# JayKickliter/Multirate.jl

Measured on AMD Instinct MI355X. Metric: Msamples/s in (Float32, 147//160, 24*147 taps) + achieved HBM GB/s vs roofline, higher is better.
Workload: dtype f32

## Files before the change

include/multirate_hip.h:

```cpp
#ifndef MULTIRATE_HIP_H
#define MULTIRATE_HIP_H

#include <stddef.h>
#include <stdint.h>

#ifdef __cplusplus
extern "C" {
#endif

#define MRHIP_ABI_VERSION 1

typedef enum {
    MRHIP_OK = 0,
    MRHIP_ERR_INVALID_ARG = 1,
    MRHIP_ERR_BUFFER_TOO_SMALL = 2,
    MRHIP_ERR_HIP = 3,
    MRHIP_ERR_NO_DEVICE = 4,
    MRHIP_ERR_UNSUPPORTED = 5
} mrhip_status;

typedef enum { MRHIP_F32 = 0, MRHIP_F64 = 1, MRHIP_C64 = 2, MRHIP_C128 = 3 } mrhip_dtype;

typedef enum {
    MRHIP_FIR_STANDARD = 0,
// ... 1 lines not shown
    MRHIP_FIR_INTERPOLATOR = 2,
    MRHIP_FIR_RATIONAL = 3,
    MRHIP_FIR_ARBITRARY = 4,
    MRHIP_FIR_FARROW = 5
} mrhip_kind;

typedef enum { MRHIP_NUMERICS_STRICT = 0, MRHIP_NUMERICS_FUSED = 1 } mrhip_numerics;

typedef struct mrhip_filter mrhip_filter;

typedef struct {
    int32_t kind;
    int32_t tap_dtype;
    int32_t sample_dtype;
    int32_t output_dtype;
    int64_t nchannels;
    int64_t hLen;
    int64_t interpolation;
    int64_t decimation;
    int64_t Nphi;
    int64_t tapsPerPhi;
    int64_t historyLen;
    int64_t phiIdx;
    int64_t inputDeficit;
    int64_t xIdx;
    double rate;
    double phiAccumulator;
    double alpha;
    double delta;
} mrhip_state;

int mrhip_abi_version(void);
const char *mrhip_last_error(void);
int mrhip_device_count(void);

int64_t mrhip_taps2pfb(const void *h, int64_t hLen, int tap_dtype, int64_t Nphi, void *pfb);
int64_t mrhip_nextphase(int64_t currentphase, int64_t interpolation, int64_t decimation);
int64_t mrhip_outputlength_ratio(int64_t inputlength, int64_t interpolation, int64_t decimation,
                                 int64_t initialPhi);
int64_t mrhip_inputlength_ratio(int64_t outputlength, int64_t interpolation, int64_t decimation,
                                int64_t initialPhi);
int mrhip_polyfit(const double *y, int64_t n, int64_t polyorder, double *coef);
int mrhip_output_dtype(int tap_dtype, int sample_dtype);

typedef enum { MRHIP_LOWPASS = 0, MRHIP_BANDPASS = 1, MRHIP_HIGHPASS = 2, MRHIP_BANDSTOP = 3 } mrhip_fir_response;
int mrhip_kaiserlength(double transition, double attenuation, double samplerate, int64_t *numtaps, double *beta);
int mrhip_kaiser(int64_t n, double beta, double *out);
int64_t mrhip_firprototype(int64_t numtaps, const double *F, int nF, int response, double *out);
int64_t mrhip_firdes(int64_t numtaps, const double *cutoff, int ncutoff, int response, double samplerate, double beta,
                     const double *window, double *out);
int64_t mrhip_firdes_kaiser(const double *cutoff, int ncutoff, double transitionwidth, double stopbandAttenuation, int response,
                            double samplerate, double *out);

int mrhip_create_rational(const void *h, int64_t hLen, int tap_dtype, int64_t num, int64_t den,
                          int sample_dtype, int64_t nchannels, int device, mrhip_filter **out);
int mrhip_create_rational_bank(const void *h, int64_t hLen, int tap_dtype, int64_t num, int64_t den,
                               int sample_dtype, int64_t nchannels, int device, mrhip_filter **out);
int mrhip_create_rational_bank_ctaps(const void *h, int64_t hLen, int tap_dtype, int64_t num, int64_t den,
                                     int sample_dtype, int64_t nchannels, int device, mrhip_filter **out);
int mrhip_create_arbitrary(const void *h, int64_t hLen, int tap_dtype, double rate, int64_t Nphi,
                           int sample_dtype, int64_t nchannels, int device, mrhip_filter **out);
int mrhip_create_arbitrary_ctaps(const void *h, int64_t hLen, int tap_dtype, double rate, int64_t Nphi,
                                 int sample_dtype, int64_t nchannels, int device, mrhip_filter **out);
int mrhip_create_farrow(const void *h, int64_t hLen, int tap_dtype, double rate, int64_t Nphi, int64_t polyorder,
                        int sample_dtype, int64_t nchannels, int device, mrhip_filter **out);
int mrhip_create_farrow_pnfb(const double *pnfb, int64_t hLen, int tap_dtype, double rate, int64_t Nphi,
                             int64_t polyorder, int sample_dtype, int64_t nchannels, int device, mrhip_filter **out);
int mrhip_create_farrow_ctaps(const void *h, int64_t hLen, int tap_dtype, double rate, int64_t Nphi, int64_t polyorder,
                              int sample_dtype, int64_t nchannels, int device, mrhip_filter **out);
int mrhip_create_farrow_pnfb_ctaps(const double *pnfb, int64_t hLen, int tap_dtype, double rate, int64_t Nphi,
                                   int64_t polyorder, int sample_dtype, int64_t nchannels, int device, mrhip_filter **out);
int mrhip_get_pnfb(const mrhip_filter *f, double *host_out);
int mrhip_farrow_tapsforphase(const mrhip_filter *f, double phase, void *host_out);
int mrhip_arbitrary_tapsforphase(const mrhip_filter *f, double phase, void *host_out);
void mrhip_destroy(mrhip_filter *f);

int64_t mrhip_outputlength(const mrhip_filter *f, int64_t inputlength);
int64_t mrhip_next_output_count(const mrhip_filter *f, int64_t inputlength);
int64_t mrhip_advance_state(mrhip_filter *f, int64_t inputlength);
int64_t mrhip_inputlength(const mrhip_filter *f, int64_t outputlength);
int mrhip_get_state(const mrhip_filter *f, mrhip_state *st);
int mrhip_set_state(mrhip_filter *f, int64_t phiIdx, int64_t inputDeficit, double phiAccumulator);
int mrhip_get_history(mrhip_filter *f, void *host_out);
int mrhip_set_history(mrhip_filter *f, const void *host_in);
int mrhip_set_history_device(mrhip_filter *f, const void *device_in, void *stream);
int mrhip_reset(mrhip_filter *f);
int mrhip_set_numerics(mrhip_filter *f, int numerics);
int mrhip_set_mod_form(mrhip_filter *f, int form);
int mrhip_get_taps(mrhip_filter *f, int which, void *host_out);

int mrhip_filt_device(mrhip_filter *f, const void *x, int64_t x_len, int64_t x_stride, void *y,
                      int64_t y_capacity, int64_t y_stride, int64_t *n_written, void *stream);
int mrhip_filt_device_async(mrhip_filter *f, const void *x, int64_t x_len, int64_t x_stride, void *y,
                            int64_t y_capacity, int64_t y_stride, int64_t *count_out, void *stream);
int mrhip_filt_device_chained(mrhip_filter *f, const mrhip_filter *prev, const void *x, int64_t x_len_bound, int64_t x_stride,
                              void *y, int64_t y_capacity, int64_t y_stride, int64_t *count_out, void *stream);
int mrhip_filt_device_multi(mrhip_filter *const *filters, int n, const void *const *x, const int64_t *x_len, void *const *y,
                            const int64_t *y_capacity, int64_t *n_written, void *stream);
int64_t mrhip_outputlength_bound(const mrhip_filter *f, int64_t inputlength);
int mrhip_sync_state(mrhip_filter *f, int64_t *last_n_written);
int mrhip_filt_device_chunked(mrhip_filter *f, const void *x, int64_t x_len, int64_t x_stride, int64_t chunk, void *y,
                              int64_t y_capacity, int64_t y_stride, int64_t *n_written, void *stream);
int mrhip_filt_host(mrhip_filter *f, const void *x, int64_t x_len, int64_t x_stride, void *y,
                    int64_t y_capacity, int64_t y_stride, int64_t *n_written);
int mrhip_synchronize(mrhip_filter *f, void *stream);

typedef struct mrhip_cascade mrhip_cascade;
int mrhip_cascade_create(mrhip_filter *const *stages, int nstages, mrhip_cascade **out);
void mrhip_cascade_destroy(mrhip_cascade *c);
int64_t mrhip_cascade_outputlength(const mrhip_cascade *c, int64_t inputlength);
int64_t mrhip_cascade_next_output_count(const mrhip_cascade *c, int64_t inputlength);
int mrhip_cascade_filt_device(mrhip_cascade *c, const void *x, int64_t x_len, int64_t x_stride, void *y, int64_t y_capacity,
                              int64_t y_stride, int64_t *n_written, void *stream);
int mrhip_cascade_filt_device_async(mrhip_cascade *c, const void *x, int64_t x_len, int64_t x_stride, void *y, int64_t y_capacity,
                                    int64_t y_stride, int64_t *count_out, void *stream);
int mrhip_cascade_reset(mrhip_cascade *c);

typedef struct mrhip_ring mrhip_ring;
int mrhip_ring_open(mrhip_filter *f, mrhip_ring **out);
int mrhip_ring_push(mrhip_ring *r, const void *x, int64_t x_len, int64_t x_stride, void *y, int64_t y_capacity, int64_t y_stride,
                    int64_t *n_written, uint64_t *seq);
int mrhip_ring_push_chunks(mrhip_ring *r, const void *x, int64_t x_len, int64_t x_stride, int64_t chunk, void *y, int64_t y_capacity,
                           int64_t y_stride, int64_t *n_written, uint64_t *last_seq);
int mrhip_ring_wait(mrhip_ring *r, uint64_t seq);
int mrhip_ring_drain(mrhip_ring *r);
int mrhip_ring_close(mrhip_ring *r);
int mrhip_ring_info(const mrhip_ring *r, int64_t *info, int n);

typedef struct mrhip_sharded mrhip_sharded;
int mrhip_sharded_create(int ctor, const void *h, int64_t hLen, int tap_dtype, int64_t num, int64_t den, double rate, int64_t Nphi,
                         int64_t polyorder, int sample_dtype, int64_t nchannels, const int *devices, int ndevices, mrhip_sharded **out);
void mrhip_sharded_destroy(mrhip_sharded *s);
int mrhip_sharded_nshards(const mrhip_sharded *s);
int mrhip_sharded_shard(const mrhip_sharded *s, int i, int64_t *start, int64_t *count, int *device, mrhip_filter **filter);
int64_t mrhip_sharded_outputlength(const mrhip_sharded *s, int64_t inputlength);
int64_t mrhip_sharded_next_output_count(const mrhip_sharded *s, int64_t inputlength);
int mrhip_sharded_reset(mrhip_sharded *s);
int mrhip_sharded_filt_device(mrhip_sharded *s, const void *const *x, int64_t x_len, const int64_t *x_stride, void *const *y, int64_t y_capacity,
                              const int64_t *y_stride, int64_t *n_written);
int mrhip_sharded_filt_host(mrhip_sharded *s, const void *x, int64_t x_len, int64_t x_stride, void *y, int64_t y_capacity, int64_t y_stride,
                            int64_t *n_written);
int mrhip_sharded_gather(mrhip_sharded *s, const void *const *y, int64_t n_out, const int64_t *y_stride, void *dst, int64_t dst_stride, int dst_device);
int mrhip_sharded_wait_stream(mrhip_sharded *s, int shard, void *stream);
int mrhip_sharded_signal_stream(mrhip_sharded *s, int shard, void *stream);
int mrhip_sharded_synchronize(mrhip_sharded *s);

int mrhip_filt_once(const void *h, int64_t hLen, int tap_dtype, int64_t num, int64_t den, double rate,
                    int64_t Nphi, const void *x, int64_t x_len, int sample_dtype, void *y,
                    int64_t y_capacity, int64_t *n_written, int device);

int mrhip_set_timing(mrhip_filter *f, int enabled);
int mrhip_timing_read(mrhip_filter *f, int64_t *n_launches, double *total_ms);
const char *mrhip_last_kernel_name(const mrhip_filter *f);
int mrhip_schedule_info(const mrhip_filter *f, int64_t *info, int n);

#ifdef __cplusplus
}
#endif
#endif
```

multirate.jl_amd/csrc/api.hip:

```cpp
#include <algorithm>
#include <cmath>
#include <chrono>
#include <cstdlib>
#include <cstring>
#include <mutex>
#include <numeric>
#include <unordered_map>

#include "mrhip_filter.h"

namespace mrhip {

bool plan_farrow_wave(const FarrowArgs &a);
hipError_t launch_farrow_wave(const TypeKey &tk, bool fused, const FarrowArgs &a, hipStream_t s, const char **kname, int num_cus);

thread_local LaunchEvents g_launch_events;
static thread_local std::string g_last_error;

void set_error(const std::string &msg) { g_last_error = msg; }

namespace {
struct OccKey { const void *fn; int dev; bool operator==(const OccKey &o) const { return fn == o.fn && dev == o.dev; } };
struct OccKeyHash { size_t operator()(const OccKey &k) const { return std::hash<const void *>()(k.fn) ^ (static_cast<size_t>(k.dev) * 0x9e3779b97f4a7c15ull); } };
struct OccEntry { unsigned block = 0; size_t lds = ~static_cast<size_t>(0), attr = 0; int per_cu = 0; };
// ... 137 lines not shown
        } else {
            (void)hipGetLastError();
            MRHIP_CHECK_HIP(device_sync_relaxed());
        }
    }
    f->last_stream = stream;
    f->last_stream_valid = true;
    return MRHIP_OK;
}

int drain_filter(mrhip_filter *f)
{
    if (f->last_stream_valid && hipStreamSynchronize(f->last_stream) != hipSuccess) {
        (void)hipGetLastError();
        MRHIP_CHECK_HIP(device_sync_relaxed());
    }
    return MRHIP_OK;
}

int check_create_args(const void *h, int64_t hLen, int th, int tx, int64_t nch, int device, mrhip_filter **out, bool complex_taps_ok = false)
{
    if (!out) return fail(MRHIP_ERR_INVALID_ARG, "out is NULL");
    *out = nullptr;
    if (!h || hLen < 1) return fail(MRHIP_ERR_INVALID_ARG, "h must hold at least one tap");
    if (th < MRHIP_F32 || th > MRHIP_C128) return fail(MRHIP_ERR_INVALID_ARG, "bad tap dtype");
    if (dtype_is_complex(th) && !complex_taps_ok)
        return fail(MRHIP_ERR_UNSUPPORTED, "complex taps are supported by the rational family only (mrhip_create_rational: FIRStandard, FIRDecimator, "
                                           "FIRInterpolator, FIRRational); FIRArbitrary and FIRFarrow take Float32 or Float64 taps");
    if (tx < MRHIP_F32 || tx > MRHIP_C128) return fail(MRHIP_ERR_INVALID_ARG, "bad sample dtype");
    if (nch < 1) return fail(MRHIP_ERR_INVALID_ARG, "nchannels must be >= 1");
    int ndev = 0;
    if (hipGetDeviceCount(&ndev) != hipSuccess || ndev == 0)
        return fail(MRHIP_ERR_NO_DEVICE, "no HIP device visible; libmultirate_hip has no CPU fallback");
    if (device < 0 || device >= ndev) return fail(MRHIP_ERR_INVALID_ARG, "device ordinal out of range");
    if (!device_is_gfx950(device))
        return fail(MRHIP_ERR_NO_DEVICE, "device is not gfx950 (MI355X); kernels are built for gfx950 only");
    return MRHIP_OK;
}

int multi_staging(mrhip_filter *f, size_t bytes)
{
    if (bytes > f->multi_cap) {
        if (f->multi_in_flight) { MRHIP_CHECK_HIP(hipEventSynchronize(f->multi_ev)); f->multi_in_flight = false; }
        if (int rc = drain_filter(f)) return rc;
        if (f->multi_pin) (void)hipHostFree(f->multi_pin);
        if (f->multi_dev) (void)hipFree(f->multi_dev);
        f->multi_pin = f->multi_dev = nullptr; f->multi_cap = 0;
        MRHIP_CHECK_HIP(hipHostMalloc(&f->multi_pin, bytes * 2, hipHostMallocDefault));
        MRHIP_CHECK_HIP(hipMalloc(&f->multi_dev, bytes * 2));
        f->multi_cap = bytes * 2;
        if (!f->multi_ev) MRHIP_CHECK_HIP(hipEventCreateWithFlags(&f->multi_ev, hipEventDisableTiming));
    }
    if (f->multi_in_flight) { MRHIP_CHECK_HIP(hipEventSynchronize(f->multi_ev)); f->multi_in_flight = false; }
    return MRHIP_OK;
}

hipError_t launch_opair_blocks(mrhip_filter *f, const TypeKey &tk, bool fused, const PolyArgs &a, hipStream_t s, const char **kname, bool *launched)
{
    *launched = false;
    PairArgs pa;
    dim3 block;
    size_t lds = 0;
    int nblocks = 0;
    if (!plan_rational_opair_blocks(tk, fused, a, f->num_cus, &pa, &block, &lds, &nblocks)) return hipSuccess;
    const size_t bytes = static_cast<size_t>(nblocks) * sizeof(MultiDesc);
    if (multi_staging(f, bytes) != MRHIP_OK) return hipErrorOutOfMemory;
    MultiDesc *d = static_cast<MultiDesc *>(f->multi_pin);
    const size_t osz = dtype_scalar_size(f->ty) * static_cast<size_t>(f->nc);
    unsigned steps_max = 0;
    for (int b = 0; b < nblocks; ++b) {
        MultiDesc &m = d[b];
        const long long first = static_cast<long long>(b) * pa.P;
        const long long Pb = std::min<long long>(pa.P, static_cast<long long>(pa.Sout) - first);
        const long long n_rel = a.n_out - first;
        const long long spc = n_rel > 0 ? (n_rel + pa.Sout - 1) / pa.Sout : 0;
        const long long u0b = a.u0 + first * a.M;
        m.x = a.x; m.y = static_cast<unsigned char *>(a.y) + static_cast<size_t>(first) * osz;
        m.hist = a.hist; m.hist_new = a.hist_new; m.taps = a.taps; m.rec = b == 0 ? a.rec : nullptr;
        m.x_stride = a.x_stride; m.y_stride = a.y_stride; m.x_len = a.x_len; m.n_out = std::max<long long>(n_rel, 0);
        m.u0 = u0b; m.d0 = a.d0; m.phi_end = a.phi_end; m.d_end = a.d_end;
        m.steps_per_channel = static_cast<unsigned>(std::max<long long>(spc, 1));
        m.total_steps = static_cast<unsigned>(spc * a.nch);
        m.spc_magic = step_magic(spc);
        m.nch = b == 0 ? a.nch : 0;
        m.P_blk = static_cast<int>(Pb);
        m.q0 = static_cast<int>((u0b / a.L) & ~1LL);
        steps_max = std::max(steps_max, m.total_steps);
    }
    hipError_t e = hipMemcpyAsync(f->multi_dev, f->multi_pin, bytes, hipMemcpyHostToDevice, s);
    if (e != hipSuccess) return e;
    e = hipEventRecord(f->multi_ev, s);
    if (e != hipSuccess) return e;
    f->multi_in_flight = true;
    PolyArgs am = a;
    am.multi = static_cast<const MultiDesc *>(f->multi_dev); am.multi_n = nblocks;
    pa.total_steps = steps_max;
    e = launch_rational_opair(fused, am, pa, block, lds, s, kname, f->num_cus, f->d_counters);
    *launched = e == hipSuccess;
    return e;
}

}
bool try_launch_interp_lane(const TypeKey &tk, bool fused, const PolyArgs &a, unsigned *counters, hipStream_t s, const char **kname, int num_cus, hipError_t *err);
namespace {

hipError_t launch_poly(const mrhip_filter *f, const TypeKey &tk, bool fused, const PolyArgs &a, hipStream_t s,
                       const char **kname, bool *did_shiftin, unsigned *counters, bool *rec_written)
{
    *did_shiftin = false;
    *rec_written = false;
    if (tk.bank && tk.complex_h) {
        *rec_written = true;
        ArbTileArgs bt;
        size_t bl = 0;
        if (!f->force_generic && plan_bank_ctaps_tiled(tk, a, f->num_cus, &bt, &bl))
            return launch_poly_bank_ctaps_tiled(tk, a, bt, bl, s, kname, f->num_cus);
        return launch_poly_bank_ctaps_generic(tk, a, s, kname);
    }
    if (tk.bank) {
        *rec_written = true;
        ArbTileArgs bt;
        size_t bl = 0;
        if (!f->force_generic && plan_bank_tiled(tk, a, f->num_cus, &bt, &bl))
            return launch_poly_bank_tiled(tk, fused, a, bt, bl, s, kname, f->num_cus);
        return launch_poly_bank_generic(tk, fused, a, s, kname);
    }
    if (tk.complex_h) {
        *rec_written = true;
        ArbTileArgs ct;
        size_t cl = 0;
        if (!f->force_generic && plan_ctaps_tiled(tk, a, f->num_cus, &ct, &cl))
            return launch_poly_ctaps_tiled(tk, a, ct, cl, s, kname, f->num_cus);
        return launch_poly_ctaps_generic(tk, a, s, kname);
    }
    if (!f->force_generic) {
        if (a.L == 1) {
            PairArgs spa;
            dim3 sblock;
            size_t slds = 0;
            if (plan_fir_stream(tk, a, f->num_cus, &spa, &sblock, &slds)) {
                *rec_written = true;
                *did_shiftin = a.H > 0;
                return launch_fir_stream(fused, a, spa, sblock, slds, s, kname, f->num_cus, counters);
            }
        }
        {
            hipError_t el = hipSuccess;
            if (try_launch_interp_lane(tk, fused, a, counters, s, kname, f->num_cus, &el)) return el;
        }
        {
            PairArgs pa;
            dim3 block;
            size_t lds = 0;
            if (plan_rational_opair(tk, fused, a, f->num_cus, &pa, &block, &lds)) {
                *rec_written = true;
                *did_shiftin = a.H > 0;
                return launch_rational_opair(fused, a, pa, block, lds, s, kname, f->num_cus, counters);
            }
            bool launched = false;
            const hipError_t eb = launch_opair_blocks(const_cast<mrhip_filter *>(f), tk, fused, a, s, kname, &launched);
            if (eb != hipSuccess) return eb;
            if (launched) { *rec_written = true; *did_shiftin = a.H > 0; return hipSuccess; }
        }
        TileArgs ta;
        dim3 grid, block;
        size_t lds = 0;
        if (plan_phase_stationary(tk, a, f->num_cus, &ta, &grid, &block, &lds))
            return launch_poly_phase_stationary(tk, fused, a, ta, grid, block, lds, s, kname, f->num_cus);
        {
            ArbTileArgs tt;
            size_t tl = 0;
            if (plan_poly_tiled(tk, a, f->num_cus, &tt, &tl))
                return launch_poly_tiled(tk, fused, a, tt, tl, s, kname, f->num_cus);
        }
    }
    *rec_written = true;
    return launch_poly_generic(tk, fused, a, s, kname);
}

}

bool any_capture_active() { return any_capture_active_impl(); }
}

using namespace mrhip;

extern "C" {

int mrhip_abi_version(void) { return MRHIP_ABI_VERSION; }
const char *mrhip_last_error(void) { return g_last_error.c_str(); }

int mrhip_device_count(void)
{
    int n = 0;
    if (hipGetDeviceCount(&n) != hipSuccess) return 0;
    int ok = 0;
    for (int d = 0; d < n; ++d) ok += device_is_gfx950(d) ? 1 : 0;
    return ok;
}

int64_t mrhip_taps2pfb(const void *h, int64_t hLen, int tap_dtype, int64_t Nphi, void *pfb)
{
    if (!h || hLen < 1 || Nphi < 1) return -1;
    return taps2pfb(h, hLen, tap_dtype, Nphi, pfb);
}
int64_t mrhip_nextphase(int64_t p, int64_t L, int64_t M) { return nextphase(p, L, M); }
int64_t mrhip_outputlength_ratio(int64_t n, int64_t L, int64_t M, int64_t phi) { return outputlength_ratio(n, L, M, phi); }
int64_t mrhip_inputlength_ratio(int64_t n, int64_t L, int64_t M, int64_t phi) { return inputlength_ratio(n, L, M, phi); }

int mrhip_output_dtype(int th, int tx)
{
    const bool f64 = dtype_is_f64(th) || dtype_is_f64(tx);
    if (dtype_is_complex(tx) || dtype_is_complex(th)) return f64 ? MRHIP_C128 : MRHIP_C64;
    return f64 ? MRHIP_F64 : MRHIP_F32;
}

static int create_rational_common(const void *h, int64_t hLen, int th, int64_t num, int64_t den, int tx, int64_t nch,
                                  int device, bool bank, mrhip_filter **out)
{
    if (num < 1 || den < 1) return fail(MRHIP_ERR_INVALID_ARG, "ratio must be positive");
    const int64_t g = std::gcd(num, den);
    const int64_t L = num / g, M = den / g;
    if (L > 0x7fffffff || M > 0x7fffffff || hLen > 0x7fffffff)
        return fail(MRHIP_ERR_INVALID_ARG, "L, M and hLen must fit in 31 bits");

    DeviceGuard guard(device);
    if (!guard.ok) return fail(MRHIP_ERR_HIP, "hipSetDevice failed");
    auto *f = new mrhip_filter();
    f->th = th; f->tx = tx; f->ty = mrhip_output_dtype(th, tx);
    f->nc = dtype_is_complex(tx) ? 2 : 1;
    f->r_f64 = dtype_is_f64(f->ty);
    f->nch = nch; f->hLen = hLen; f->L = L; f->M = M; f->device = device;
    f->bank = bank;
    const size_t es = dtype_size(th);
    const size_t rows = bank ? static_cast<size_t>(nch) : 1;

    if (L == 1) {
        f->kind = M == 1 ? MRHIP_FIR_STANDARD : MRHIP_FIR_DECIMATOR;
        f->Nphi = 1; f->T = hLen; f->H = hLen - 1;
    } else {
        f->kind = M == 1 ? MRHIP_FIR_INTERPOLATOR : MRHIP_FIR_RATIONAL;
        f->Nphi = L;
        f->T = taps2pfb(h, hLen, th, L, nullptr);
        f->H = f->T - 1;
    }
    {
        const size_t bank_bytes = static_cast<size_t>(f->T) * static_cast<size_t>(f->Nphi) * es;
        f->h_taps.resize(bank_bytes * rows);
        for (size_t r = 0; r < rows; ++r)
            taps2pfb(static_cast<const unsigned char *>(h) + r * static_cast<size_t>(hLen) * es, hLen, th, f->Nphi, f->h_taps.data() + r * bank_bytes);
    }
    int rc = upload_taps(f, f->h_taps, &f->d_taps, &f->d_taps_alloc);
    if (!rc) rc = alloc_common(f);
    if (rc) { mrhip_destroy(f); return rc; }
    *out = f;
    return MRHIP_OK;
}

int mrhip_create_rational(const void *h, int64_t hLen, int th, int64_t num, int64_t den, int tx, int64_t nch,
                          int device, mrhip_filter **out)
{
    if (int rc = check_create_args(h, hLen, th, tx, nch, device, out, true)) return rc;
    return create_rational_common(h, hLen, th, num, den, tx, nch, device, false, out);
}

int mrhip_create_rational_bank(const void *h, int64_t hLen, int th, int64_t num, int64_t den, int tx, int64_t nch,
                               int device, mrhip_filter **out)
{
    if (out) *out = nullptr;
    if (th == MRHIP_C64 || th == MRHIP_C128)
        return fail(MRHIP_ERR_UNSUPPORTED, "mrhip_create_rational_bank takes Float32 / Float64 taps (complex taps in a bank are not supported)");
    if (int rc = check_create_args(h, hLen, th, tx, nch, device, out)) return rc;
    return create_rational_common(h, hLen, th, num, den, tx, nch, device, true, out);
}

int mrhip_create_rational_bank_ctaps(const void *h, int64_t hLen, int th, int64_t num, int64_t den, int tx, int64_t nch,
                                     int device, mrhip_filter **out)
{
    if (out) *out = nullptr;
    if (th == MRHIP_F32 || th == MRHIP_F64)
        return fail(MRHIP_ERR_INVALID_ARG, "mrhip_create_rational_bank_ctaps takes Complex64 / Complex128 taps; real taps: mrhip_create_rational_bank");
    if (int rc = check_create_args(h, hLen, th, tx, nch, device, out, true)) return rc;
    return create_rational_common(h, hLen, th, num, den, tx, nch, device, true, out);
}

static int create_arbitrary_common(const void *h, int64_t hLen, int th, double rate, int64_t Nphi, int tx, int64_t nch,
                                   int device, mrhip_filter **out)
{
    if (!(rate > 0.0)) return fail(MRHIP_ERR_INVALID_ARG, "rate must be greater than 0");
    if (Nphi < 1 || Nphi > 0x7fffffff || hLen > 0x7fffffff) return fail(MRHIP_ERR_INVALID_ARG, "bad Nphi");

    DeviceGuard guard(device);
    if (!guard.ok) return fail(MRHIP_ERR_HIP, "hipSetDevice failed");
    auto *f = new mrhip_filter();
    f->kind = MRHIP_FIR_ARBITRARY;
    f->th = th; f->tx = tx; f->ty = mrhip_output_dtype(th, tx);
    f->nc = dtype_is_complex(tx) ? 2 : 1;
    f->r_f64 = dtype_is_f64(f->ty);
    f->nch = nch; f->hLen = hLen; f->L = Nphi; f->M = 1; f->Nphi = Nphi; f->device = device;
    f->rate = rate;
    f->delta = static_cast<double>(Nphi) / rate;
    const size_t es = dtype_size(th);

    std::vector<unsigned char> dh(static_cast<size_t>(hLen) * es, 0);
    arbitrary_dh(h, hLen, th, dh.data());
    f->T = taps2pfb(h, hLen, th, Nphi, nullptr);
    f->H = f->T - 1;
// ... 1383 lines not shown
        if (f->d_xbuf[slot]) (void)hipFree(f->d_xbuf[slot]);
        f->d_xbuf[slot] = nullptr; f->d_xcap[slot] = 0;
        MRHIP_CHECK_HIP(hipMalloc(&f->d_xbuf[slot], xbytes));
        f->d_xcap[slot] = xbytes;
    }
    if (ybytes > f->d_ycap[slot]) {
        if (f->d_ybuf[slot]) (void)hipFree(f->d_ybuf[slot]);
        f->d_ybuf[slot] = nullptr; f->d_ycap[slot] = 0;
        MRHIP_CHECK_HIP(hipMalloc(&f->d_ybuf[slot], ybytes));
        f->d_ycap[slot] = ybytes;
    }
    return MRHIP_OK;
}

int mrhip_filt_host(mrhip_filter *f, const void *x, int64_t x_len, int64_t x_stride, void *y, int64_t y_capacity,
                    int64_t y_stride, int64_t *n_written)
{
    if (!f) return fail(MRHIP_ERR_INVALID_ARG, "NULL filter");
    if (n_written) *n_written = 0;
    if (x_len < 0 || y_capacity < 0) return fail(MRHIP_ERR_INVALID_ARG, "negative length");
    if (x_len == 0) return MRHIP_OK;
    if (!x) return fail(MRHIP_ERR_INVALID_ARG, "x is NULL");
    if (f->nch > 1 && x_stride < x_len) return fail(MRHIP_ERR_INVALID_ARG, "x_stride < x_len");
    const int64_t count = mrhip_next_output_count(f, x_len);
    if (count > y_capacity) return fail(MRHIP_ERR_BUFFER_TOO_SMALL, "buffer is too small");
    if (count > 0 && !y) return fail(MRHIP_ERR_INVALID_ARG, "y is NULL");
    if (f->nch > 1 && y_stride < count) return fail(MRHIP_ERR_INVALID_ARG, "y_stride < output count");

    DeviceGuard guard(f->device);
    if (!guard.ok) return fail(MRHIP_ERR_HIP, "hipSetDevice failed");
    const size_t xe = x_elt(f), ye = y_elt(f);
    const int64_t env_kb = MRHIP_ENV_INT("MRHIP_HOST_PIECE_KB", 0);
    const int64_t piece_kb = env_kb > 0 ? env_kb : 64 * 1024;
    int64_t piece = (piece_kb << 10) / static_cast<int64_t>(xe * static_cast<size_t>(f->nch));
    piece = std::max<int64_t>(piece, 256);
    const bool pipelined = x_len > piece + piece / 2;
    if (!pipelined) piece = x_len;
    if (!f->s_in) {
        MRHIP_CHECK_HIP(hipStreamCreateWithFlags(&f->s_in, hipStreamNonBlocking));
        MRHIP_CHECK_HIP(hipStreamCreateWithFlags(&f->s_out, hipStreamNonBlocking));
        for (int i = 0; i < 2; ++i) {
            MRHIP_CHECK_HIP(hipEventCreateWithFlags(&f->ev_in[i], hipEventDisableTiming));
            MRHIP_CHECK_HIP(hipEventCreateWithFlags(&f->ev_k[i], hipEventDisableTiming));
            MRHIP_CHECK_HIP(hipEventCreateWithFlags(&f->ev_out[i], hipEventDisableTiming));
        }
    }
    hipStream_t sk = f->own_stream;
    const int64_t y_piece_cap = pipelined ? std::max<int64_t>(mrhip_outputlength(f, piece), 0) + 8 + 2 * (f->L / std::max<int64_t>(f->M, 1) + 1) : count;
    const int nslots = pipelined ? 2 : 1;
    for (int sl = 0; sl < nslots; ++sl)
        if (int rc = ensure_staging(f, sl, std::max<size_t>(static_cast<size_t>(piece) * xe * f->nch, 16),
                                    std::max<size_t>(static_cast<size_t>(y_piece_cap) * ye * f->nch, 16))) return rc;
    const size_t x_pitch = static_cast<size_t>(f->nch > 1 ? x_stride : x_len) * xe;
    const size_t y_pitch = static_cast<size_t>(f->nch > 1 ? y_stride : count) * ye;
    int64_t k = 0;
    int it = 0;
    bool used[2] = {false, false};
    auto bail = [&](int rc) -> int {
        (void)hipStreamSynchronize(f->s_in); (void)hipStreamSynchronize(sk); (void)hipStreamSynchronize(f->s_out);
        (void)hipGetLastError();
        if (n_written) *n_written = k;
        return rc;
    };
#define MRHIP_HOSTPATH_HIP(expr)                                                                          \
    do {                                                                                                    \
        hipError_t e_ = (expr);                                                                             \
        if (e_ != hipSuccess) return bail(fail(MRHIP_ERR_HIP, std::string(#expr) + ": " + hipGetErrorString(e_))); \
    } while (0)
    for (int64_t a = 0; a < x_len; a += piece, ++it) {
        const int sl = it & 1;
        const int64_t len = std::min<int64_t>(piece, x_len - a);
        const size_t xrow = static_cast<size_t>(len) * xe;
        if (used[sl]) MRHIP_HOSTPATH_HIP(hipStreamWaitEvent(f->s_in, f->ev_k[sl], 0));
        MRHIP_HOSTPATH_HIP(hipMemcpy2DAsync(f->d_xbuf[sl], xrow, static_cast<const unsigned char *>(x) + static_cast<size_t>(a) * xe, x_pitch, xrow,
                                         static_cast<size_t>(f->nch), hipMemcpyHostToDevice, f->s_in));
        MRHIP_HOSTPATH_HIP(hipEventRecord(f->ev_in[sl], f->s_in));
        MRHIP_HOSTPATH_HIP(hipStreamWaitEvent(sk, f->ev_in[sl], 0));
        if (used[sl]) MRHIP_HOSTPATH_HIP(hipStreamWaitEvent(sk, f->ev_out[sl], 0));
        const int64_t cap = std::min<int64_t>(y_piece_cap, count - k);
        int64_t nw = 0;
        if (int rc = filt_device_one(f, f->d_xbuf[sl], len, len, f->d_ybuf[sl], cap, std::max<int64_t>(cap, 1), &nw, sk, a > 0)) {
            return bail(rc);
        }
        MRHIP_HOSTPATH_HIP(hipEventRecord(f->ev_k[sl], sk));
        if (nw > 0) {
            MRHIP_HOSTPATH_HIP(hipStreamWaitEvent(f->s_out, f->ev_k[sl], 0));
            const size_t yrow = static_cast<size_t>(nw) * ye;
            MRHIP_HOSTPATH_HIP(hipMemcpy2DAsync(static_cast<unsigned char *>(y) + static_cast<size_t>(k) * ye, y_pitch, f->d_ybuf[sl],
                                             static_cast<size_t>(std::max<int64_t>(cap, 1)) * ye, yrow, static_cast<size_t>(f->nch), hipMemcpyDeviceToHost, f->s_out));
        }
        MRHIP_HOSTPATH_HIP(hipEventRecord(f->ev_out[sl], f->s_out));
        used[sl] = true;
        k += nw;
    }
#undef MRHIP_HOSTPATH_HIP
    MRHIP_CHECK_HIP(hipStreamSynchronize(f->s_out));
    MRHIP_CHECK_HIP(hipStreamSynchronize(sk));
    if (n_written) *n_written = k;
    return MRHIP_OK;
}

int mrhip_synchronize(mrhip_filter *f, void *stream)
{
    if (!f) return fail(MRHIP_ERR_INVALID_ARG, "NULL filter");
    DeviceGuard guard(f->device);
    MRHIP_CHECK_HIP(hipStreamSynchronize(static_cast<hipStream_t>(stream)));
    return MRHIP_OK;
}

int mrhip_filt_once(const void *h, int64_t hLen, int th, int64_t num, int64_t den, double rate, int64_t Nphi,
                    const void *x, int64_t x_len, int tx, void *y, int64_t y_capacity, int64_t *n_written, int device)
{
    mrhip_filter *f = nullptr;
    int rc = rate > 0.0 ? mrhip_create_arbitrary(h, hLen, th, rate, Nphi, tx, 1, device, &f)
                        : mrhip_create_rational(h, hLen, th, num, den, tx, 1, device, &f);
    if (rc) return rc;
    rc = mrhip_filt_host(f, x, x_len, x_len, y, y_capacity, y_capacity, n_written);
    mrhip_destroy(f);
    return rc;
}

int mrhip_set_timing(mrhip_filter *f, int enabled)
{
    if (!f) return fail(MRHIP_ERR_INVALID_ARG, "NULL filter");
    f->timing = enabled != 0;
    f->timing_stride = enabled > 1 ? enabled : 1;
    f->timing_group = enabled < -1 ? -enabled : 1;
    f->timing_launch = 0; f->timing_open = false; f->ev_skip = false;
    f->ev_used = 0;
    return MRHIP_OK;
}

int mrhip_timing_read(mrhip_filter *f, int64_t *n_launches, double *total_ms)
{
    if (!f || !n_launches || !total_ms) return fail(MRHIP_ERR_INVALID_ARG, "NULL argument");
    DeviceGuard guard(f->device);
    *n_launches = 0;
    *total_ms = 0.0;
    const size_t pairs = f->ev_used / 2;
    for (size_t i = 0; i < pairs; ++i) {
        float ms = 0.f;
        MRHIP_CHECK_HIP(hipEventSynchronize(f->ev_pool[2 * i + 1]));
        MRHIP_CHECK_HIP(hipEventElapsedTime(&ms, f->ev_pool[2 * i], f->ev_pool[2 * i + 1]));
        *total_ms += ms;
    }
    *n_launches = static_cast<int64_t>(pairs) * f->timing_group;
    f->ev_used = 0;
    f->timing_launch = 0; f->timing_open = false;
    return MRHIP_OK;
}

const char *mrhip_last_kernel_name(const mrhip_filter *f) { return f ? f->last_kernel : ""; }

int mrhip_schedule_info(const mrhip_filter *f, int64_t *info, int n)
{
    if (!f || !info || n < 0) return fail(MRHIP_ERR_INVALID_ARG, "NULL argument");
    if (f->kind != MRHIP_FIR_ARBITRARY && f->kind != MRHIP_FIR_FARROW) return fail(MRHIP_ERR_INVALID_ARG, "not a FIRArbitrary / FIRFarrow filter");
    const int64_t v[9] = {f->splan.ok, f->splan.ncand, f->splan.nwin, f->per_valid ? f->per_Q : 0,
                          f->stat_host_steps, f->stat_periodic_steps, f->stat_device_pieces, f->stat_fallback_pieces, f->stat_memo_hits};
    for (int i = 0; i < n && i < 9; ++i) info[i] = v[i];
    return MRHIP_OK;
}

}

#include "ring_api.inc"
```

multirate.jl_amd/csrc/kernels_rational_opair.hip:

```cpp
#include <algorithm>
#include <cstdio>
#include <cstdlib>
#include <vector>

#include "mrhip_internal.h"

namespace mrhip {

hipError_t launch_opair_f32_s0r(bool fused, int T, dim3 block, size_t lds, hipStream_t s, const PolyArgs &a, const PairArgs &pa, int num_cus);
hipError_t launch_opair_f32_s0c(bool fused, int T, dim3 block, size_t lds, hipStream_t s, const PolyArgs &a, const PairArgs &pa, int num_cus);
hipError_t launch_opair_f32_s1r(bool fused, int T, dim3 block, size_t lds, hipStream_t s, const PolyArgs &a, const PairArgs &pa, int num_cus);
hipError_t launch_opair_f32_s1c(bool fused, int T, dim3 block, size_t lds, hipStream_t s, const PolyArgs &a, const PairArgs &pa, int num_cus);
hipError_t launch_opair_f32_s0_long(int nc, bool fused, int T, dim3 block, size_t lds, hipStream_t s, const PolyArgs &a, const PairArgs &pa, int num_cus);
hipError_t launch_opair_f32_s1_long(int nc, bool fused, int T, dim3 block, size_t lds, hipStream_t s, const PolyArgs &a, const PairArgs &pa, int num_cus);
hipError_t launch_opair_f32_s2(int nc, bool fused, int T, dim3 block, size_t lds, hipStream_t s, const PolyArgs &a, const PairArgs &pa, int num_cus);
hipError_t launch_opair_f32_s3(int nc, bool fused, int T, dim3 block, size_t lds, hipStream_t s, const PolyArgs &a, const PairArgs &pa, int num_cus);
hipError_t launch_opair_f32_s4(int nc, bool fused, int T, dim3 block, size_t lds, hipStream_t s, const PolyArgs &a, const PairArgs &pa, int num_cus);
hipError_t launch_opair_f32_s5(int nc, bool fused, int T, dim3 block, size_t lds, hipStream_t s, const PolyArgs &a, const PairArgs &pa, int num_cus);
hipError_t launch_opair_wide_s0(bool x_f64, bool fused, int T, dim3 block, size_t lds, hipStream_t s, const PolyArgs &a, const PairArgs &pa, int num_cus);
hipError_t launch_opair_wide_s1(bool x_f64, bool fused, int T, dim3 block, size_t lds, hipStream_t s, const PolyArgs &a, const PairArgs &pa, int num_cus);
hipError_t launch_opair_cmix_s0(bool x_f64, bool fused, int T, dim3 block, size_t lds, hipStream_t s, const PolyArgs &a, const PairArgs &pa, int num_cus);
hipError_t launch_opair_cmix_s1(bool x_f64, bool fused, int T, dim3 block, size_t lds, hipStream_t s, const PolyArgs &a, const PairArgs &pa, int num_cus);

namespace {
constexpr int kOMaxThreads = 512;
}

bool plan_rational_opair(const TypeKey &tk, bool fused, const PolyArgs &a, int num_cus, PairArgs *out, dim3 *block, size_t *lds, int force_wgpc)
{
    if (!MRHIP_ENV_INT("MRHIP_OPAIR", 1)) return false;
    if (tk.x_f64 && !tk.r_f64) return false;
    const int nc = tk.complex_x ? 2 : 1;
    const long long es = (tk.x_f64 ? 8 : 4) * nc;
#ifdef MRHIP_PS_FAST_BUILD
    if (a.T != 24 && !((a.T == 36 || a.T == 48) && !tk.complex_x) && !(!tk.r_f64 && (a.T == 36 || a.T == 48 || a.T == 56 || a.T == 64))) return false;
#endif
    if (a.T < 1 || a.T > (tk.r_f64 ? (tk.complex_x ? 32 : 48) : 64)) return false;
    if (a.L < 2 || a.M < 1 || a.zero_start_below > 0) return false;
    const int smin = static_cast<int>(a.M / a.L);
    if (smin > 5) return false;
    if (!opair_instantiated(fused, smin, a.T)) return false;
    if (smin >= 2 && (tk.r_f64 || a.T > 32)) return false;
    const int env_c = MRHIP_ENV_INT("MRHIP_OPAIR_C", 0), env_j = MRHIP_ENV_INT("MRHIP_OPAIR_J", 0), env_ns = MRHIP_ENV_INT("MRHIP_OPAIR_NS", 0);
    int best_c = 0;
    double best = -1.0;
    for (int pass = 0; pass < 2 && !best_c; ++pass)
        for (int c = 2; static_cast<long long>(c) * a.L / 2 <= kOMaxThreads && static_cast<long long>(c) * a.L <= 1024; c += 2) {
            const int lanes = static_cast<int>(static_cast<long long>(c) * a.L / 2);
            const int padded = (lanes + 63) / 64 * 64;
            if (pass == 0 && (padded < 192 || padded > 448)) continue;
            const double score = static_cast<double>(lanes) / padded * (padded < 192 ? 0.5 + 0.5 * padded / 192.0 : 1.0);
            if (score > best + 1e-9) { best = score; best_c = c; }
        }
    if (a.n_out * a.nch < (1LL << 22))
        for (int c = 2; static_cast<long long>(c) * a.L / 2 <= kOMaxThreads && static_cast<long long>(c) * a.L <= 1024; c += 2)
            if (static_cast<long long>(c) * a.L / 2 >= 128) { best_c = c; break; }
    if (env_c > 0 && env_c % 2 == 0 && static_cast<long long>(env_c) * a.L / 2 <= kOMaxThreads && static_cast<long long>(env_c) * a.L <= 1024) best_c = env_c;
    if (!best_c) return false;
    if (tk.r_f64 && a.T > 32 && (static_cast<long long>(best_c) * a.L / 2 + 63) / 64 > 7) return false;
    const int c = best_c;
    const long long cM = static_cast<long long>(c) * a.M, cL = static_cast<long long>(c) * a.L;
    const int lanes = static_cast<int>(cL / 2);
    const int padded = (lanes + 63) / 64 * 64;
    const int nwaves = padded / 64;
    const int tail = a.T + smin + 4;
    const int vgpr_est = (2 * a.T + (nc == 2 ? 36 : 30) + 7) / 8 * 8;
    const int waves_per_cu = tk.r_f64 ? 12 : 4 * std::min(8, 512 / vgpr_est);
    int wg_per_cu = std::max(1, std::min(4, waves_per_cu / (nwaves + 1)));
    if (nwaves + 1 == 6 && !tk.r_f64) wg_per_cu = 3;
    if (nwaves + 1 == 6 && tk.r_f64) wg_per_cu = 1;
    if (force_wgpc > 0) wg_per_cu = force_wgpc;
    if (const int env_w = MRHIP_ENV_INT("MRHIP_OPAIR_WGPC", 0); env_w > 0) wg_per_cu = env_w;
    int ns = env_ns >= 2 && env_ns <= 8 ? env_ns : (wg_per_cu == 1 ? 3 : 2);
    auto j_for = [&](int stages) -> long long {
        const long long budget_kib = ((wg_per_cu <= 3 ? 150 : 160) * 1024 / wg_per_cu - 64) / stages / 1024;
        const long long j = ((budget_kib > 1 ? budget_kib : 1) * 1024 / es - tail) / cM;
        return j < 1 ? 1 : j;
    };
    long long J = j_for(ns);
    if (env_j > 0) J = env_j;
    if (J > 64) J = 64;
    if (env_j <= 0) {
        const long long want_tiles = 4LL * num_cus;
        while (J > 2 && ((a.n_out + J * cL - 1) / (J * cL)) * a.nch < want_tiles) J = (J + 1) / 2;
    }
    const long long max_slots = 60 / (ns > 2 ? ns - 2 : 1);
    auto slots_for = [&](long long j) { return (((j * cM + tail + 3) / 4 * 4) * es / 16 + 63) / 64; };
    while (J > 1 && slots_for(J) > max_slots) --J;
    long long tile_len = (J * cM + tail + 3) / 4 * 4;
    const long long nslots = slots_for(J);
    const size_t stage_bytes = static_cast<size_t>(nslots) * 1024;
    if (nslots > max_slots || ns * stage_bytes > 156 * 1024) return false;
    PairArgs pa{};
    pa.c = c; pa.P = static_cast<int>(cL); pa.cM = static_cast<int>(cM);
    pa.Sout = pa.P; pa.lds_step = pa.cM; pa.run_chunks = 0; pa.q0 = 0; pa.run_magic = 0;
    pa.J = static_cast<int>(J);
    pa.tile_len = static_cast<int>(tile_len);
    pa.tail = tail;
    pa.dma_rounds = static_cast<int>(nslots);
    pa.stage_bytes = static_cast<int>(stage_bytes);
    pa.ns = ns;
    pa.nc = nc;
    pa.x_f64 = tk.x_f64 ? 1 : 0; pa.r_f64 = tk.r_f64 ? 1 : 0;
    pa.o0 = a.d0 - a.T;
    pa.tile_in = J * cM;
    pa.tile_out = J * cL;
    pa.tiles_per_channel = (a.n_out + pa.tile_out - 1) / pa.tile_out;
    pa.total_tiles = pa.tiles_per_channel * a.nch;
    if (a.n_out >= (1LL << 31) - pa.tile_out || pa.total_tiles >= (1LL << 31) - 65536) return false;
    const long long spc = (a.n_out + cL - 1) / cL;
    if (spc * a.nch >= (1LL << 31)) return false;
    pa.steps_per_channel = static_cast<unsigned>(spc);
    pa.total_steps = static_cast<unsigned>(spc * a.nch);
    pa.spc_magic = step_magic(spc);
    pa.flags_off = static_cast<int>(ns * stage_bytes);
    {
        const long long pt = (a.T + 4) | 1;
        const bool fits = static_cast<size_t>(a.L * pt * (tk.r_f64 ? 8 : 4)) <= stage_bytes;
        pa.bank_off = (fits && MRHIP_ENV_INT("MRHIP_OPAIR_BANK", 1)) ? static_cast<int>((ns - 1) * stage_bytes) : -1;
    }
    *out = pa;
    *block = dim3(static_cast<unsigned>(padded + 64));
    *lds = ns * stage_bytes + 8 * ns;
    return true;
}

bool plan_rational_opair_blocks(const TypeKey &tk, bool fused, const PolyArgs &a, int num_cus, PairArgs *out, dim3 *block, size_t *lds, int *nblocks_out)
{
    if (!MRHIP_ENV_INT("MRHIP_OPAIR", 1) || !MRHIP_ENV_INT("MRHIP_OPAIR_BLOCKS", 1)) return false;
    if (tk.x_f64 && !tk.r_f64) return false;
    if (a.L <= 512 || a.L > 4096 || a.M < 1 || a.zero_start_below > 0 || a.dyn || a.multi) return false;
    const int smin = static_cast<int>(a.M / a.L);
    if (smin > 1 || !opair_instantiated(fused, smin, a.T)) return false;
    if (a.T < 1 || a.T > (tk.r_f64 ? (tk.complex_x ? 32 : 48) : 64)) return false;
#ifdef MRHIP_PS_FAST_BUILD
    if (a.T != 24) return false;
#endif
    const int nc = tk.complex_x ? 2 : 1;
    const long long es = (tk.x_f64 ? 8 : 4) * nc;
    const int epc = static_cast<int>(16 / es) > 0 ? static_cast<int>(16 / es) : 1;
    const long long Sout = 2LL * a.L, Sin = 2LL * a.M;
    int max_lanes = MRHIP_ENV_INT("MRHIP_OPAIR_BLK_LANES", 0);
    if (max_lanes < 64 || max_lanes > 448) max_lanes = tk.r_f64 ? 320 : 448;
    int nblocks = static_cast<int>((Sout / 2 + max_lanes - 1) / max_lanes);
    if (nblocks < 2) nblocks = 2;
    long long P = (Sout + nblocks - 1) / nblocks;
    P = (P + 1) / 2 * 2;
    nblocks = static_cast<int>((Sout + P - 1) / P);
    const int lanes = static_cast<int>(P / 2), padded = (lanes + 63) / 64 * 64, nwaves = padded / 64;
    if (tk.r_f64 && a.T > 32 && nwaves > 7) return false;
    long long span = ((P - 2) * a.M + a.L - 1) / a.L + 1 + a.T + smin + 2 + 2;
    const long long rc = (span + epc - 1) / epc;
    long long lds_step = rc * epc;
    const int vgpr_est = (2 * a.T + (nc == 2 ? 36 : 30) + 7) / 8 * 8;
    const int waves_per_cu = tk.r_f64 ? 12 : 4 * std::min(8, 512 / vgpr_est);
    int wg_per_cu = std::max(1, std::min(4, waves_per_cu / (nwaves + 1)));
    if (nwaves + 1 == 6 && !tk.r_f64) wg_per_cu = 3;
    const int ns = wg_per_cu == 1 ? 3 : 2;
    const long long budget = ((wg_per_cu <= 3 ? 150 : 160) * 1024 / wg_per_cu - 64) / ns;
    long long J = budget / (lds_step * es);
    if (const int env_j = MRHIP_ENV_INT("MRHIP_OPAIR_J", 0); env_j > 0) J = env_j;
    if (J > 64) J = 64;
    if (J < 1) return false;
    const long long max_slots = 60 / (ns > 2 ? ns - 2 : 1);
    auto slots_for = [&](long long j) { return (j * rc + 63) / 64; };
    while (J > 1 && slots_for(J) > max_slots) --J;
    {
        const long long want_tiles = 4LL * num_cus;
        const long long spc0 = (a.n_out + Sout - 1) / Sout;
        while (J > 2 && ((spc0 + J - 1) / J) * a.nch * nblocks < want_tiles) J = (J + 1) / 2;
    }
    const long long nslots = slots_for(J);
    const size_t stage_bytes = static_cast<size_t>(nslots) * 1024;
    if (nslots > max_slots || ns * stage_bytes > 156 * 1024) return false;
    const long long spc = (a.n_out + Sout - 1) / Sout;
    if (spc * a.nch >= (1LL << 31) || a.n_out >= (1LL << 31) - Sout * J) return false;
    if ((a.u0 + Sout * a.M) >= (1LL << 31)) return false;
    PairArgs pa{};
    pa.c = 2; pa.P = static_cast<int>(P); pa.cM = static_cast<int>(Sin);
    pa.Sout = static_cast<int>(Sout); pa.lds_step = static_cast<int>(lds_step); pa.run_chunks = static_cast<int>(rc); pa.q0 = 0;
    pa.run_magic = static_cast<unsigned>(0xffffffffu / static_cast<unsigned>(rc) + 1u);
    pa.J = static_cast<int>(J);
    pa.tile_len = static_cast<int>(J * lds_step);
    pa.tail = a.T + smin + 4;
    pa.dma_rounds = static_cast<int>(nslots);
    pa.stage_bytes = static_cast<int>(stage_bytes);
    pa.ns = ns; pa.nc = nc;
    pa.x_f64 = tk.x_f64 ? 1 : 0; pa.r_f64 = tk.r_f64 ? 1 : 0;
    pa.o0 = a.d0 - a.T;
    pa.tile_in = J * Sin; pa.tile_out = J * Sout;
    pa.tiles_per_channel = (a.n_out + pa.tile_out - 1) / pa.tile_out;
    pa.total_tiles = pa.tiles_per_channel * a.nch * nblocks;
    pa.steps_per_channel = static_cast<unsigned>(spc);
    pa.total_steps = static_cast<unsigned>(spc * a.nch);
    pa.spc_magic = step_magic(spc);
    pa.flags_off = static_cast<int>(ns * stage_bytes);
    pa.bank_off = -1;
    *out = pa;
    *block = dim3(static_cast<unsigned>(padded + 64));
    *lds = ns * stage_bytes + 8 * ns;
    *nblocks_out = nblocks;
    return true;
}

bool opair_ring_available(const TypeKey &tk, bool fused, const PolyArgs &a)
{
    if (fused || a.L < 2 || a.M < 1 || a.M / a.L > 1) return false;
    if (tk.x_f64 && !tk.r_f64) return false;
#ifdef MRHIP_PS_FAST_BUILD
    return a.T == 24;
#else
    return a.T == 24 || a.T == 32;
#endif
}

#ifdef MRHIP_OPAIR_PROBE
static unsigned long long *opair_probe_buf(long long g)
{
    static unsigned long long *buf = nullptr;
    static long long cap = 0;
    if (!std::getenv("MRHIP_PROBE_OUT")) return nullptr;
    if (g > cap) { if (buf) (void)hipFree(buf); (void)hipMalloc(&buf, static_cast<size_t>(g) * 8 * 4 * 8); cap = g; }
    (void)hipMemset(buf, 0, static_cast<size_t>(g) * 8 * 4 * 8);
    (void)hipDeviceSynchronize();
    return buf;
}
static void opair_probe_dump(unsigned long long *buf, long long g, hipStream_t s)
{
    if (!buf) return;
    (void)hipStreamSynchronize(s);
    std::vector<unsigned long long> h(static_cast<size_t>(g) * 8 * 4);
    (void)hipMemcpy(h.data(), buf, h.size() * 8, hipMemcpyDeviceToHost);
    if (FILE *f = std::fopen(std::getenv("MRHIP_PROBE_OUT"), "wb")) { std::fwrite(h.data(), 8, h.size(), f); std::fclose(f); }
}
#define MRHIP_PROBE_PRE(g) pa.probe = opair_probe_buf(g);
#define MRHIP_PROBE_POST(g) opair_probe_dump(pa.probe, g, s);
#else
#define MRHIP_PROBE_PRE(g)
#define MRHIP_PROBE_POST(g)
#endif

hipError_t launch_opair_kernel(PairKernelFn kfn, const void *key, dim3 block, size_t lds, hipStream_t s, const PolyArgs &a, PairArgs pa, int num_cus)
{
    if (!kfn) return hipErrorNotSupported;
    int per_cu = 0;
    hipError_t eo = occupancy_cached(reinterpret_cast<const void *>(kfn), block.x, lds, &per_cu);
    if (eo != hipSuccess) return eo;
    per_cu = opair_six_wave_cap(per_cu, num_cus, pa.total_steps, pa.J, block.x);
    if (const int bpc = MRHIP_ENV_INT("MRHIP_OPAIR_BPC", 0); bpc > 0) per_cu = bpc;
    const PairGrid pg = pair_grid(per_cu, num_cus, pa.total_steps, pa.J, kPairGroups, a.multi ? a.multi_n : 0, a.ring_dev != nullptr, pa.grid_cap);
    pa.ngroups = pg.ngroups;
    if (!a.ring_dev) pa.steps_per_group = pg.steps_per_group;
    pa.static_grabs = pg.static_grabs;
    const long long g = pg.grid;
    if (int regs; debug_first_launch(key, reinterpret_cast<const void *>(kfn), &regs))
        std::fprintf(stderr, "[mrhip] rational_opair T=%d smin=%d in=%zuB arith=%zuB grid=%lld block=%u lds=%zu occ/CU=%d regs=%d c=%d P=%d cM=%d J=%d ns=%d\n",
                     a.T, static_cast<int>(a.M / a.L), static_cast<size_t>(pa.x_f64 ? 8 : 4) * pa.nc, static_cast<size_t>(pa.r_f64 ? 8 : 4), g, block.x, lds, per_cu,
                     regs, pa.c, pa.P, pa.cM, pa.J, pa.ns);
    MRHIP_PROBE_PRE(g)
    launch_kernel(kfn, dim3(static_cast<unsigned>(g)), block, lds, s, a, pa);
    MRHIP_PROBE_POST(g)
    return hipGetLastError();
}

hipError_t launch_rational_opair(bool fused, const PolyArgs &a, const PairArgs &pa_in, dim3 block, size_t lds, hipStream_t s,
                                 const char **kname, int num_cus, unsigned *counters)
{
    if (!counters) return hipErrorInvalidValue;
    PairArgs pa = pa_in;
    pa.counters = counters;
    *kname = "rational_opair_kernel";
    const int smin = static_cast<int>(a.M / a.L);
    if (pa.r_f64 && pa.nc == 2)
        return smin == 0 ? launch_opair_cmix_s0(pa.x_f64 != 0, fused, a.T, block, lds, s, a, pa, num_cus)
                         : launch_opair_cmix_s1(pa.x_f64 != 0, fused, a.T, block, lds, s, a, pa, num_cus);
    if (pa.r_f64)
        return smin == 0 ? launch_opair_wide_s0(pa.x_f64 != 0, fused, a.T, block, lds, s, a, pa, num_cus)
                         : launch_opair_wide_s1(pa.x_f64 != 0, fused, a.T, block, lds, s, a, pa, num_cus);
    if (a.T > 48)
        return smin == 0 ? launch_opair_f32_s0_long(pa.nc, fused, a.T, block, lds, s, a, pa, num_cus) : launch_opair_f32_s1_long(pa.nc, fused, a.T, block, lds, s, a, pa, num_cus);
    switch (smin) {
    case 0: return pa.nc == 2 ? launch_opair_f32_s0c(fused, a.T, block, lds, s, a, pa, num_cus) : launch_opair_f32_s0r(fused, a.T, block, lds, s, a, pa, num_cus);
    case 1: return pa.nc == 2 ? launch_opair_f32_s1c(fused, a.T, block, lds, s, a, pa, num_cus) : launch_opair_f32_s1r(fused, a.T, block, lds, s, a, pa, num_cus);
    case 2: return launch_opair_f32_s2(pa.nc, fused, a.T, block, lds, s, a, pa, num_cus);
    case 3: return launch_opair_f32_s3(pa.nc, fused, a.T, block, lds, s, a, pa, num_cus);
    case 4: return launch_opair_f32_s4(pa.nc, fused, a.T, block, lds, s, a, pa, num_cus);
    case 5: return launch_opair_f32_s5(pa.nc, fused, a.T, block, lds, s, a, pa, num_cus);
    default: return hipErrorInvalidValue;
    }
}

}
```

multirate.jl_amd/csrc/mrhip_internal.h:

```cpp
#pragma once

#include <hip/hip_runtime.h>
#include <hip/hip_ext.h>

#include <cstdint>
#include <cstdlib>
#include <string>
#include <vector>

#include "multirate_hip.h"

namespace mrhip {

void set_error(const std::string &msg);
int fail(int code, const std::string &msg);

#define MRHIP_CHECK_HIP(expr)                                                                  \
    do {                                                                                       \
        hipError_t _e = (expr);                                                                \
        if (_e != hipSuccess)                                                                  \
            return ::mrhip::fail(MRHIP_ERR_HIP, std::string(#expr) + ": " + hipGetErrorString(_e)); \
    } while (0)

inline bool dtype_is_complex(int dt) { return dt == MRHIP_C64 || dt == MRHIP_C128; }
// ... 203 lines not shown
    unsigned steps_per_channel, total_steps, spc_magic;
    int nch;
    int P_blk, q0;
};

constexpr int kRingDepth = 64;
constexpr int kRingTraceRows = 512, kRingTraceTiles = 32;
constexpr int kRingShards = 32;
struct RingDesc {
    unsigned long long x, y;
    long long x_stride, y_stride, x_len, n_out;
    long long u0, d0;
    unsigned long long tile_base;
    unsigned ngrabs, seq_lo;
    unsigned steps_per_channel, total_steps;
    unsigned spc_magic, flags;
    unsigned long long seq;
    unsigned long long pad[3];
};
static_assert(sizeof(RingDesc) == 128, "RingDesc is 16 quad-words");
constexpr int kRingKeyQword = 8;
struct RingHost {
    unsigned long long head;
    unsigned long long close;
    unsigned long long stopped;
    unsigned long long arrived, grid;
    unsigned long long pad[3];
    unsigned long long done[kRingDepth];
    RingDesc desc[kRingDepth];
};
struct RingDev {
    unsigned long long head;
    unsigned long long closed;
    unsigned long long idle_ticks;
    unsigned long long opts;
    unsigned long long pad[4];
    unsigned long long hist_seq[kRingDepth];
    unsigned chunk_done[kRingDepth];
    unsigned shard_done[kRingDepth][kRingShards][32];
    unsigned long long stats[24];
    unsigned long long arrived;
    unsigned long long grid;
    unsigned long long flush_req;
    unsigned long long flush_pub;
    unsigned long long flush_pad[12];
    unsigned long long flush_ent[kRingDepth][2];
    unsigned long long flush_claim[8][16];
    unsigned long long flush_done[8][16];
    unsigned long long next_ticket[8][16];
    __attribute__((aligned(128))) RingDesc desc[kRingDepth];
    unsigned long long trace[kRingTraceRows][3 * kRingTraceTiles];
};

struct ShiftFold {
    void *hist_new;
    unsigned *done;
};

struct ArbArgs {
    const void *x;
    void *y;
    const void *hist;
    const void *taps;
    const void *dtaps;
    const int *n_idx;
    const double *acc;
    long long x_stride, y_stride;
    long long x_len;
    long long n_out;
    int T, H, Nphi;
    int nch;
    const DevCall *dyn;
    ShiftFold fold;
};

struct FarrowArgs {
    const void *x;
    void *y;
    const void *hist;
    const double *pnfb;
    const int *n_idx;
    const double *acc;
    long long x_stride, y_stride;
    long long x_len;
    long long n_out;
    int T, H, polyorder;
    int tap_f32;
    int nch;
    int seam_below;
    const DevCall *dyn;
    ShiftFold fold;
};

struct HistArgs {
    const void *x;
    const void *hist_old;
    void *hist_new;
    long long x_stride;
    long long x_len;
    int H;
    int nch;
    const DevCall *dyn;
};

struct TileArgs {
    int c;
    int P;
    int J;
    int tile_len;
    int copyB_offset_bytes;
    int stage_bytes;
    int dma_rounds;
    int ablate;
    int x_aligned16;
    int by_position;
    long long tiles_per_channel;
    long long total_tiles;
};

struct PairArgs {
    int c;
    int P;
    int cM;
    int J;
    int tile_len;
    int tail;
    int dma_rounds;
    int stage_bytes;
    int ns;
    int nc;
    int x_f64, r_f64;
    int ablate;
    unsigned steps_per_channel;
    unsigned total_steps;
    unsigned steps_per_group;
    int ngroups;
    int grid_cap;
    int flags_off;
    int pad_every;
    int bank_off;
    int static_grabs;
    int rt;
    int rt_rd;
    unsigned *counters;
    unsigned spc_magic;
    int Sout, lds_step, run_chunks, q0;
    unsigned run_magic;
    long long o0;
    long long tile_in;
    long long tile_out;
    long long tiles_per_channel;
    long long total_tiles;
    unsigned long long *probe;
};

constexpr size_t kCounterBytes = 33 * 256;

struct ArbTileArgs {
    int cpl;
    int tap_pitch;
    int bank_elems;
    int x_offset_bytes;
    int max_span;
    int prefetch;
    int copyb_pad;
    int pipe;
    int row_pitch;
    int dma_slots;
    long long tile_out;
    long long tiles_per_channel;
    long long total_tiles;
    unsigned *counters;
    int run_tiles;
};

__device__ __forceinline__ void tiles_take_dyn(long long &n_out, ArbTileArgs &ta, long long &ngroups, const DevCall *dyn)
{
    ngroups = ta.tiles_per_channel > 0 ? ta.total_tiles / ta.tiles_per_channel : 1;
    if (dyn) {
        n_out = dyn->n_out;
        ta.tiles_per_channel = (n_out + ta.tile_out - 1) / ta.tile_out;
        ta.total_tiles = ta.tiles_per_channel * ngroups;
    }
}

struct LaunchEvents { hipEvent_t start = nullptr, stop = nullptr; };
extern thread_local LaunchEvents g_launch_events;

template <typename F, typename... Args>
inline void launch_kernel(F kfn, dim3 grid, dim3 block, size_t lds, hipStream_t s, Args... args)
{
    const LaunchEvents ev = g_launch_events;
    g_launch_events = LaunchEvents{};
    if (ev.start && ev.stop)
        hipExtLaunchKernelGGL(kfn, grid, block, static_cast<std::uint32_t>(lds), s, ev.start, ev.stop, 0u, args...);
    else
        hipLaunchKernelGGL(kfn, grid, block, lds, s, args...);
}

hipError_t occupancy_cached(const void *kfn, unsigned block, size_t lds, int *per_cu);

inline int env_int_read(const char *name, int dflt)
{
    const char *v = std::getenv(name);
    return v && *v ? std::atoi(v) : dflt;
}
inline bool env_dynamic()
{
    static const bool d = env_int_read("MRHIP_ENV_DYNAMIC", 0) != 0;
    return d;
}
#define MRHIP_ENV_INT(name, dflt) ([]() -> int { static const int v_ = ::mrhip::env_int_read(name, dflt); \
                                                 return ::mrhip::env_dynamic() ? ::mrhip::env_int_read(name, dflt) : v_; }())

struct PersistentGrid { hipError_t err; long long grid; int per_cu; };
inline PersistentGrid persistent_grid(const void *kfn, unsigned threads, size_t lds, int num_cus, long long total_tiles, int bpc = 0,
                                      bool bpc_replaces = false)
{
    PersistentGrid g{hipSuccess, 1, 0};
    g.err = occupancy_cached(kfn, threads, lds, &g.per_cu);
    if (g.err == hipSuccess) g.grid = persistent_grid_size(&g.per_cu, num_cus, total_tiles, bpc, bpc_replaces);
    return g;
}

bool debug_first_launch(const void *key, const void *kfn, int *regs);

struct TypeKey {
    bool x_f64;
    bool r_f64;
    bool complex_x;
    bool complex_h = false;
    bool bank = false;
};

hipError_t launch_poly_generic(const TypeKey &tk, bool fused, const PolyArgs &a, hipStream_t s, const char **kname);
hipError_t launch_arb_generic(const TypeKey &tk, bool fused, const ArbArgs &a, hipStream_t s, const char **kname);
hipError_t launch_farrow(const TypeKey &tk, bool fused, const FarrowArgs &a, hipStream_t s, const char **kname);
bool plan_farrow_tiled(const TypeKey &tk, const FarrowArgs &a, const int32_t *n_idx_host, const int *spans, int num_cus, ArbTileArgs *out, size_t *lds);
hipError_t launch_farrow_tiled(const TypeKey &tk, bool fused, const FarrowArgs &a, const ArbTileArgs &ta, size_t lds, hipStream_t s,
                               const char **kname, int num_cus);
hipError_t launch_shiftin(const TypeKey &tk, const HistArgs &a, hipStream_t s);
bool polyfit_rows(const double *y, int64_t n, int polyorder, double *coef);
bool plan_rational_opair(const TypeKey &tk, bool fused, const PolyArgs &a, int num_cus, PairArgs *out, dim3 *block, size_t *lds, int force_wgpc = 0);
bool plan_rational_opair_blocks(const TypeKey &tk, bool fused, const PolyArgs &a, int num_cus, PairArgs *out, dim3 *block, size_t *lds, int *nblocks);
hipError_t launch_rational_opair(bool fused, const PolyArgs &a, const PairArgs &pa, dim3 block, size_t lds, hipStream_t s,
                                 const char **kname, int num_cus, unsigned *counters);
constexpr bool opair_instantiated(bool fused, int smin, int T) { return !fused || (smin <= 1 && T % 4 == 0); }
using PairKernelFn = void (*)(PolyArgs, PairArgs);
hipError_t launch_opair_kernel(PairKernelFn kfn, const void *key, dim3 block, size_t lds, hipStream_t s, const PolyArgs &a, PairArgs pa, int num_cus);
hipError_t launch_stream_kernel(PairKernelFn kfn, const void *key, dim3 block, size_t lds, hipStream_t s, const PolyArgs &a, PairArgs pa, int num_cus);
bool plan_fir_stream(const TypeKey &tk, const PolyArgs &a, int num_cus, PairArgs *out, dim3 *block, size_t *lds);
hipError_t launch_fir_stream(bool fused, const PolyArgs &a, const PairArgs &pa, dim3 block, size_t lds, hipStream_t s,
                             const char **kname, int num_cus, unsigned *counters);
bool plan_arb_tiled(const TypeKey &tk, const ArbArgs &a, const int32_t *n_idx_host, const int *spans, int num_cus, ArbTileArgs *out, size_t *lds);
bool plan_arb_pipe(const TypeKey &tk, const ArbArgs &a, long long span256, ArbTileArgs *out, size_t *lds);
hipError_t launch_arb_pipe(const TypeKey &tk, bool fused, const ArbArgs &a, const ArbTileArgs &ta, size_t lds, hipStream_t s,
                           const char **kname, int num_cus);
struct ArbLaneArgs {
    int ring;
    int pitch8;
    int stretch;
    int chunk_max;
    int ngroups;
    int y16;
    unsigned *counters;
};
bool arb_lane_eligible(const TypeKey &tk, int T, int H, int64_t nch, double rate, int64_t x_len, int64_t x_stride, int64_t y_stride);
bool plan_arb_lane(const TypeKey &tk, const ArbArgs &a, double rate, ArbLaneArgs *out, size_t *lds);
hipError_t launch_arb_lane(bool fused, const ArbArgs &a, const ArbLaneArgs &la, size_t lds, hipStream_t s, const char **kname, int num_cus);
hipError_t launch_arb_tiled(const TypeKey &tk, bool fused, const ArbArgs &a, const ArbTileArgs &ta, size_t lds, hipStream_t s,
                            const char **kname, int num_cus);
bool plan_poly_tiled(const TypeKey &tk, const PolyArgs &a, int num_cus, ArbTileArgs *out, size_t *lds);
hipError_t launch_poly_tiled(const TypeKey &tk, bool fused, const PolyArgs &a, const ArbTileArgs &ta, size_t lds, hipStream_t s,
                             const char **kname, int num_cus);
hipError_t launch_poly_ctaps_generic(const TypeKey &tk, const PolyArgs &a, hipStream_t s, const char **kname);
bool plan_ctaps_tiled(const TypeKey &tk, const PolyArgs &a, int num_cus, ArbTileArgs *out, size_t *lds);
hipError_t launch_poly_ctaps_tiled(const TypeKey &tk, const PolyArgs &a, const ArbTileArgs &ta, size_t lds, hipStream_t s,
                                   const char **kname, int num_cus);
hipError_t launch_poly_bank_generic(const TypeKey &tk, bool fused, const PolyArgs &a, hipStream_t s, const char **kname);
bool plan_bank_tiled(const TypeKey &tk, const PolyArgs &a, int num_cus, ArbTileArgs *out, size_t *lds);
hipError_t launch_poly_bank_tiled(const TypeKey &tk, bool fused, const PolyArgs &a, const ArbTileArgs &ta, size_t lds, hipStream_t s,
                                  const char **kname, int num_cus);
hipError_t launch_poly_bank_ctaps_generic(const TypeKey &tk, const PolyArgs &a, hipStream_t s, const char **kname);
bool plan_bank_ctaps_tiled(const TypeKey &tk, const PolyArgs &a, int num_cus, ArbTileArgs *out, size_t *lds);
hipError_t launch_poly_bank_ctaps_tiled(const TypeKey &tk, const PolyArgs &a, const ArbTileArgs &ta, size_t lds, hipStream_t s,
                                        const char **kname, int num_cus);
hipError_t launch_arb_ctaps_generic(const TypeKey &tk, const ArbArgs &a, hipStream_t s, const char **kname);
bool plan_ctaps_arb_tiled(const TypeKey &tk, const ArbArgs &a, double rate, int num_cus, ArbTileArgs *out, size_t *lds);
hipError_t launch_arb_ctaps_tiled(const TypeKey &tk, const ArbArgs &a, const ArbTileArgs &ta, size_t lds, hipStream_t s,
                                  const char **kname, int num_cus);
hipError_t launch_farrow_ctaps_generic(const TypeKey &tk, const FarrowArgs &a, hipStream_t s, const char **kname);
bool plan_ctaps_farrow_tiled(const TypeKey &tk, const FarrowArgs &a, double rate, int num_cus, ArbTileArgs *out, size_t *lds);
hipError_t launch_farrow_ctaps_tiled(const TypeKey &tk, const FarrowArgs &a, const ArbTileArgs &ta, size_t lds, hipStream_t s,
                                     const char **kname, int num_cus);
void arbitrary_dh(const void *h, int64_t hLen, int th, void *dh);
bool plan_phase_stationary(const TypeKey &tk, const PolyArgs &a, int num_cus, TileArgs *out, dim3 *grid, dim3 *block,
                           size_t *lds);
hipError_t launch_poly_phase_stationary(const TypeKey &tk, bool fused, const PolyArgs &a, const TileArgs &ta, dim3 grid,
                                        dim3 block, size_t lds, hipStream_t s, const char **kname, int num_cus);

}
```

multirate.jl_amd/csrc/opair_kernel.inc:

```
#include <algorithm>
#include <cstdio>
#include <cstdlib>
#include <type_traits>
#include <vector>

#include "mrhip_internal.h"
#include "pair_device.h"
#include "pair_loader.h"

#pragma clang fp contract(off)

#ifndef MRHIP_OPAIR_WIDE_LONG
#define MRHIP_OPAIR_WIDE_LONG 1
#endif

namespace mrhip {
namespace {

constexpr int kOMaxThreads = 512;

using namespace dev;

__device__ __forceinline__ float fma_r(float a, float b, float c) { return __builtin_fmaf(a, b, c); }
__device__ __forceinline__ double fma_r(double a, double b, double c) { return __builtin_fma(a, b, c); }

template <bool FUSED, bool FIRST, bool COND, typename R>
__device__ __forceinline__ R slot_mac(R tap, R w, R acc, bool used)
{
    if constexpr (FIRST) {
        const R p = tap * w;
        if constexpr (COND) return used ? p : static_cast<R>(-0.0);
        else return p;
    } else if constexpr (FUSED) {
        const R r = fma_r(tap, w, acc);
        if constexpr (COND) return used ? r : acc;
        else return r;
    } else {
        R p = tap * w;
        if constexpr (COND) p = used ? p : static_cast<R>(-0.0);
        return acc + p;
    }
}

template <int T, bool FUSED, int NC, int SMIN, typename TXS, typename R, int MODE = 0>
#ifndef MRHIP_OPAIR_WIDE_WAVES
#define MRHIP_OPAIR_WIDE_WAVES 3
#endif
#ifndef MRHIP_RING_WAVES
#define MRHIP_RING_WAVES 4
#endif
__global__ __launch_bounds__(sizeof(R) == 8 && T > 32 ? kOMaxThreads : kOMaxThreads + 64, sizeof(R) == 8 ? (T > 32 ? 2 : MRHIP_OPAIR_WIDE_WAVES) : (MODE == 2 ? MRHIP_RING_WAVES : 3))
void rational_opair_kernel(PolyArgs a, PairArgs pa)
{
    constexpr unsigned ES = static_cast<unsigned>(sizeof(TXS)) * NC;
    constexpr unsigned OS = static_cast<unsigned>(sizeof(R)) * NC;
    constexpr int NW = static_cast<int>(ES / 4);
    static_assert(NW == 1 || NW == 2 || NW == 4, "sample size");
    using pair_t = std::conditional_t<NW == 1, v2u_t, v4u_t>;
    constexpr int SPRD = NW == 4 ? 1 : 2;
    constexpr int W = T + SMIN + 2;
    constexpr int NPR = (W + SPRD - 1) / SPRD;
    constexpr int NA = T + 1, NB = T + 2;
    constexpr bool TAILM = T >= 3;
    constexpr bool HEADM = T >= 3 && !FUSED;

    extern __shared__ __attribute__((aligned(16))) unsigned char smem[];
    const unsigned lds_base = static_cast<unsigned>(reinterpret_cast<uintptr_t>(smem));
    const int tid = threadIdx.x;
    const int wave = __builtin_amdgcn_readfirstlane(tid >> 6), lane = tid & 63;
    const int ncw = (blockDim.x >> 6) - 1;
    constexpr bool RING = MODE == 2;
    if constexpr (MODE == 0) pair_take_dyn(a, pa);

    if (wave == ncw) {
        if constexpr (RING) pair_ring_loader_wave<NW, static_cast<int>(OS)>(a, pa, smem, lane);
        else pair_loader_wave<NW, MODE != 1>(a, pa, smem, lane);
        return;
    }
    if constexpr (RING) { if (blockIdx.x == 0) return; }
    volatile unsigned *const tile_flag = reinterpret_cast<volatile unsigned *>(smem + pa.flags_off);

    const int Li = static_cast<int>(a.L), Mi = static_cast<int>(a.M);
    int u0 = static_cast<int>(a.u0);
    const bool act = 2 * tid + 1 < pa.P;
    int uA = u0 + (act ? 2 * tid : 0) * Mi, uB = uA + Mi;
    int qA = uA / Li, phA = uA - qA * Li;
    int qB = uB / Li, phB = uB - qB * Li;
    int run0 = qA & ~1;
    int offA = qA - run0;
    int dB = qB - run0 - SMIN;
    R tapA[NA], tapB[NB];
    auto gather_taps = [&]() {
        const R *__restrict__ ca = static_cast<const R *>(a.taps) + static_cast<long long>(phA) * T;
        const R *__restrict__ cb = static_cast<const R *>(a.taps) + static_cast<long long>(phB) * T;
        R colA[T], colB[T];
#pragma unroll
        for (int i = 0; i < T; ++i) { colA[i] = ca[i]; colB[i] = cb[i]; }
#pragma unroll
        for (int j = NA - 1; j >= 0; --j) {
            const R t0 = j < T ? colA[j] : R(0), t1 = j >= 1 ? colA[j - 1] : R(0);
            tapA[j] = act ? (offA == 0 ? t0 : t1) : R(0);
            pin(tapA[j]);
        }
#pragma unroll
        for (int j = NB - 1; j >= 0; --j) {
            const R t0 = j < T ? colB[j] : R(0), t1 = (j >= 1 && j - 1 < T) ? colB[j - 1] : R(0), t2 = j >= 2 ? colB[j - 2] : R(0);
            tapB[j] = act ? (dB == 0 ? t0 : dB == 1 ? t1 : t2) : R(0);
            pin(tapB[j]);
        }
    };
    if constexpr (RING) {
#pragma unroll
        for (int j = 0; j < NA; ++j) tapA[j] = R(0);
#pragma unroll
        for (int j = 0; j < NB; ++j) tapB[j] = R(0);
        u0 = -1;
    } else if (pa.bank_off >= 0) {
        constexpr int PT = (T + 4) | 1;
        R *const bank = reinterpret_cast<R *>(smem + pa.bank_off);
        const R *__restrict__ tg = static_cast<const R *>(a.taps);
        const int ntaps = Li * T;
        for (int idx = tid; idx < ntaps; idx += ncw * 64) {
            const int col = idx / T, i = idx - col * T;
            bank[col * PT + 2 + i] = tg[idx];
        }
        asm volatile("s_waitcnt vmcnt(0) lgkmcnt(0)" ::: "memory");
        __builtin_amdgcn_s_barrier();
        const R *ba = bank + (act ? phA : 0) * PT + 2 - offA;
        const R *bb = bank + (act ? phB : 0) * PT + 2 - (act ? dB : 0);
#pragma unroll
        for (int j = 0; j < NA; ++j) tapA[j] = ba[j];
#pragma unroll
        for (int j = 0; j < NB; ++j) tapB[j] = bb[j];
#pragma unroll
        for (int j = 0; j < NA; ++j) pin(tapA[j]);
#pragma unroll
        for (int j = 0; j < NB; ++j) pin(tapB[j]);
    } else gather_taps();
    bool useA0 = offA == 0, useAT = offA == 1;
    bool useB0 = dB == 0, useB1 = dB <= 1, useBT = dB >= 1, useBT1 = dB == 2;
    auto lanes_of = [](bool b) { return static_cast<unsigned long long>(__builtin_amdgcn_ballot_w64(b)); };
    unsigned long long mA0 = lanes_of(useA0), mAT = lanes_of(useAT);
    unsigned long long mB0 = lanes_of(useB0), mB1 = lanes_of(useB1), mBT = lanes_of(useBT), mBT1 = lanes_of(useBT1);

    const int n_out = static_cast<int>(a.n_out);
#ifdef MRHIP_OPAIR_PROBE
    unsigned long long pr_wait = 0, pr_tiles = 0;
    const unsigned long long pr_t0 = clock64(), pr_w0 = wall_clock64();
#endif
    unsigned ring_opts = 0;
    if constexpr (RING) ring_opts = static_cast<unsigned>(__builtin_amdgcn_readfirstlane(static_cast<int>(ld_sc1(&a.ring_dev->opts))));
    unsigned long long rs_bar = 0, rs_drain = 0;
    const unsigned long long rs_t0 = RING ? wall_clock64() : 0ull;
    bool pend = false;
    int p_stage = 0;
    unsigned p_slot = 0, p_shard = 0, p_cnt = 0, p_nshards = 0, p_seq_lo = 0, p_seq_hi = 0;
    for (int s = 0;; s = (s + 1 == pa.ns ? 0 : s + 1)) {
#ifdef MRHIP_OPAIR_PROBE
        const unsigned long long pr_a = clock64();
#endif
        unsigned long long rs_b0 = 0;
        if constexpr (RING) { if (ring_opts & 256u) rs_b0 = wall_clock64(); }
        __builtin_amdgcn_s_barrier();
        asm volatile("" ::: "memory");
        if constexpr (RING) { if (ring_opts & 256u) rs_bar += wall_clock64() - rs_b0; }
#ifdef MRHIP_OPAIR_PROBE
        pr_wait += clock64() - pr_a;
        ++pr_tiles;
#endif
        int J, remaining;
        R *__restrict__ yc;
        unsigned ring_flags = 0, ring_slot = 0, ring_shard = 0, ring_cnt = 0, ring_nshards = 0, ring_seq_lo = 0, ring_seq_hi = 0;
        if constexpr (RING) {
            auto word = [&](int w) -> unsigned { return static_cast<unsigned>(__builtin_amdgcn_readfirstlane(static_cast<int>(tile_flag[kRingTileWords * s + w]))); };
            const unsigned tj = word(0);
            ring_flags = word(1);
            if (pend) {
                pend = false;
                const unsigned long long rs_d0 = (ring_opts & 256u) ? wall_clock64() : 0ull;
                if (!(ring_opts & 16u)) vm_drain();
                if (ring_opts & 256u) rs_drain += wall_clock64() - rs_d0;
                if (lane == 0) {
                    unsigned *const wg_done = reinterpret_cast<unsigned *>(smem + pa.flags_off) + kRingTileWords * pa.ns;
                    const unsigned prev = __hip_atomic_fetch_add(wg_done + p_stage, 1u, __ATOMIC_RELAXED, __HIP_MEMORY_SCOPE_WORKGROUP);
                    if (prev + 1u == static_cast<unsigned>(ncw)) {
                        __hip_atomic_store(wg_done + p_stage, 0u, __ATOMIC_RELAXED, __HIP_MEMORY_SCOPE_WORKGROUP);
                        ring_grab_done(a.ring_dev, a.ring_host, p_slot, (static_cast<unsigned long long>(p_seq_hi) << 32) | p_seq_lo, p_shard, p_cnt, p_nshards);
                    }
                }
            }
            if (tj == 0u) break;
            if (ring_flags & 2u) continue;
            J = static_cast<int>(tj);
            yc = reinterpret_cast<R *>((static_cast<unsigned long long>(word(3)) << 32) | word(2));
            remaining = static_cast<int>(word(4));
            const int u0_t = static_cast<int>(word(5));
            ring_slot = word(6); ring_shard = word(7); ring_seq_lo = word(8); ring_seq_hi = word(9); ring_cnt = word(10); ring_nshards = word(11);
            if (u0_t != u0) {
                u0 = u0_t;
                uA = u0 + (act ? 2 * tid : 0) * Mi; uB = uA + Mi;
                qA = uA / Li; phA = uA - qA * Li;
                qB = uB / Li; phB = uB - qB * Li;
                run0 = qA & ~1; offA = qA - run0; dB = qB - run0 - SMIN;
                gather_taps();
                useA0 = offA == 0; useAT = offA == 1;
                useB0 = dB == 0; useB1 = dB <= 1; useBT = dB >= 1; useBT1 = dB == 2;
                mA0 = lanes_of(useA0); mAT = lanes_of(useAT);
                mB0 = lanes_of(useB0); mB1 = lanes_of(useB1); mBT = lanes_of(useBT); mBT1 = lanes_of(useBT1);
            }
        } else {
            const unsigned tg = static_cast<unsigned>(__builtin_amdgcn_readfirstlane(static_cast<int>(tile_flag[2 * s])));
            const unsigned tj = static_cast<unsigned>(__builtin_amdgcn_readfirstlane(static_cast<int>(tile_flag[2 * s + 1])));
            if (tj == 0u) break;
            const TileAt ta = pair_tile_at(pa, tg, tj);
            J = ta.jt;
            yc = static_cast<R *>(a.y) + (static_cast<long long>(ta.ch) * a.y_stride + static_cast<long long>(ta.st) * pa.Sout) * NC;
            remaining = n_out - ta.st * pa.Sout;
        }
        const bool full = remaining >= (J - 1) * pa.Sout + pa.P;
        unsigned lane_t;
        asm volatile("v_mbcnt_lo_u32_b32 %0, -1, 0\n\tv_mbcnt_hi_u32_b32 %0, -1, %0" : "=v"(lane_t));
        const unsigned tid_t = static_cast<unsigned>(wave) * 64u + lane_t;
        const unsigned my_out = 2u * tid_t;
        const unsigned uA_t = static_cast<unsigned>(u0) + (2u * tid_t < static_cast<unsigned>(pa.P) ? 2u * tid_t : 0u) * static_cast<unsigned>(Mi);
        const unsigned R_t = (uA_t / static_cast<unsigned>(Li)) & ~1u;
        const unsigned wbase = lds_base + static_cast<unsigned>(s) * pa.stage_bytes + (R_t - static_cast<unsigned>(pa.q0)) * ES;

        auto run_steps = [&](auto full_tag) {
            constexpr bool FULL = decltype(full_tag)::value;
            constexpr int KP = NPR < (NW == 1 ? 5 : 3) ? NPR : (NW == 1 ? 5 : 3);
            constexpr int NPRV = (NPR + KP - 1) / KP * KP;
            constexpr bool PAIRED_WAITS = KP >= 5;
            pair_t pring[KP];
            char *const ybytes = reinterpret_cast<char *>(yc);
            auto read_pair = [&](auto off_tag, unsigned addr) -> pair_t {
                constexpr int OFFP = decltype(off_tag)::value;
                if constexpr (NW == 1) return lds_read_b64<OFFP * 8>(addr);
                else return lds_read_b128<OFFP * 16>(addr);
            };
            static_for<0, KP>([&](auto I) { pring[decltype(I)::value] = read_pair(I, wbase); });
#pragma unroll 1
            for (int j = 0; j < J; ++j) {
                const int jn = j + 1 < J ? j + 1 : j;
                const unsigned wcur = wbase + static_cast<unsigned>(j) * pa.lds_step * ES;
                const unsigned wnext = wbase + static_cast<unsigned>(jn) * pa.lds_step * ES;
                R accA[NC] = {}, accB[NC] = {};
                R headA[NC], headB[NC], sumB[NC];
                static_for<0, NPRV>([&](auto I) {
                    constexpr int r = decltype(I)::value;
                    constexpr int slot = r % KP;
                    if constexpr (r < NPR) {
                        if constexpr (!PAIRED_WAITS) lgkm_wait<ring_younger(r, NPR, KP, 0)>(pring[slot]);
                        else if constexpr (r % 2 == 0) {
                            if constexpr (r + 1 < NPR) lgkm_wait2<ring_younger_pair(r, NPR, KP, 0)>(pring[slot], pring[(r + 1) % KP]);
                            else lgkm_wait<ring_younger(r, NPR, KP, 0)>(pring[slot]);
                        }
                        R wv[2][NC];
                        if constexpr (NW == 4) {
                            wv[0][0] = __hiloint2double(static_cast<int>(pring[slot].y), static_cast<int>(pring[slot].x));
                            wv[0][1] = __hiloint2double(static_cast<int>(pring[slot].w), static_cast<int>(pring[slot].z));
                        } else if constexpr (sizeof(TXS) == 8) {
                            wv[0][0] = __hiloint2double(static_cast<int>(pring[slot].y), static_cast<int>(pring[slot].x));
                            wv[1][0] = __hiloint2double(static_cast<int>(pring[slot].w), static_cast<int>(pring[slot].z));
                        } else if constexpr (NC == 1) {
                            wv[0][0] = static_cast<R>(__uint_as_float(pring[slot].x)); wv[1][0] = static_cast<R>(__uint_as_float(pring[slot].y));
                        } else {
                            wv[0][0] = static_cast<R>(__uint_as_float(pring[slot].x)); wv[0][1] = static_cast<R>(__uint_as_float(pring[slot].y));
                            wv[1][0] = static_cast<R>(__uint_as_float(pring[slot].z)); wv[1][1] = static_cast<R>(__uint_as_float(pring[slot].w));
                        }
                        static_for<0, SPRD>([&](auto H) {
                            constexpr int js = SPRD * r + decltype(H)::value;
                            constexpr int jb = js - SMIN;
                            constexpr bool a_lo = js < 1, a_hi = js > T - 1;
                            constexpr bool b_lo = jb < 2, b_hi = jb > T - 1;
                            constexpr int h = decltype(H)::value;
                            if constexpr (js < NA) {
                                if constexpr (HEADM && js == 0) {
                                    if constexpr (SPRD == 1) masked_mul(headA, tapA[0], wv[h], mA0);
                                } else if constexpr (HEADM && js == 1) {
#pragma unroll
                                    for (int cc = 0; cc < NC; ++cc) accA[cc] = tapA[1] * wv[h][cc];
                                    if constexpr (SPRD == 1) masked_add(accA, headA, mA0);
                                    else masked_mul_add(accA, tapA[0], wv[0], mA0);
                                } else if constexpr (TAILM && a_hi) masked_mac<FUSED>(accA, tapA[js], wv[h], mAT);
                                else {
                                    const bool used = (a_lo ? useA0 : true) && (a_hi ? useAT : true);
#pragma unroll
                                    for (int cc = 0; cc < NC; ++cc) accA[cc] = slot_mac<FUSED, js == 0, a_lo || a_hi, R>(tapA[js], wv[h][cc], accA[cc], used);
                                }
                            }
                            if constexpr (jb >= 0 && jb < NB) {
                                if constexpr (HEADM && jb == 0) masked_mul(headB, tapB[0], wv[h], mB0);
                                else if constexpr (HEADM && jb == 1) masked_mul_then_add(sumB, headB, tapB[1], wv[h], mB1, mB0);
                                else if constexpr (HEADM && jb == 2) {
#pragma unroll
                                    for (int cc = 0; cc < NC; ++cc) accB[cc] = tapB[2] * wv[h][cc];
                                    masked_add(accB, sumB, mB1);
                                } else if constexpr (TAILM && b_hi) masked_mac<FUSED>(accB, tapB[jb], wv[h], jb == T ? mBT : mBT1);
                                else {
                                    const bool used = (b_lo ? (jb == 0 ? useB0 : useB1) : true) && (b_hi ? (jb == T ? useBT : useBT1) : true);
#pragma unroll
                                    for (int cc = 0; cc < NC; ++cc) accB[cc] = slot_mac<FUSED, jb == 0, b_lo || b_hi, R>(tapB[jb], wv[h][cc], accB[cc], used);
                                }
                            }
                        });
                        constexpr int js_l = SPRD * r + SPRD - 1, jb_l = js_l - SMIN;
#pragma unroll
                        for (int cc = 0; cc < NC; ++cc) {
                            if constexpr (HEADM && js_l == 0) pin(headA[cc]); else pin(accA[cc]);
                            if constexpr (HEADM && jb_l == 0) pin(headB[cc]);
                            else if constexpr (HEADM && jb_l == 1) pin(sumB[cc]);
                            else if constexpr (!HEADM || jb_l >= 2) pin(accB[cc]);
                        }
                    }
                    if constexpr (r + KP < NPR) pring[slot] = read_pair(std::integral_constant<int, r + KP>{}, wcur);
                    else if constexpr (r + KP >= NPRV) pring[slot] = read_pair(std::integral_constant<int, r + KP - NPRV>{}, wnext);
                });
                {
                    const unsigned kj = static_cast<unsigned>(j) * static_cast<unsigned>(pa.Sout);
                    char *const dst = ybytes + (kj + my_out) * OS;
                    R v[2 * NC];
#pragma unroll
                    for (int cc = 0; cc < NC; ++cc) { v[cc] = accA[cc]; v[NC + cc] = accB[cc]; }
                    auto put2 = [&]() { if constexpr (RING) { if (ring_nshards >> 31) { store_wt<2 * OS>(dst, v); return; } } __builtin_memcpy(dst, v, 2 * OS); };
                    auto put1 = [&]() { if constexpr (RING) { if (ring_nshards >> 31) { store_wt<OS>(dst, v); return; } } __builtin_memcpy(dst, v, OS); };
                    bool covered = false;
                    if constexpr (RING && 2 * OS == 8) {
                        if (!(ring_nshards >> 31)) {
                            covered = true;
                            const unsigned lim_x = FULL ? static_cast<unsigned>(pa.P) : (static_cast<unsigned>(remaining) > kj ? umin(static_cast<unsigned>(remaining) - kj, static_cast<unsigned>(pa.P)) : 0u);
                            if (my_out + 1 < lim_x) __builtin_memcpy(dst, v, 2 * OS);
                            else if (my_out < lim_x) __builtin_memcpy(dst, v, OS);
                        } else if (ring_opts & 8u) {
                            unsigned q[4];
                            q[0] = __float_as_uint(v[0]); q[1] = __float_as_uint(v[1]);
                            q[2] = static_cast<unsigned>(__builtin_amdgcn_mov_dpp(static_cast<int>(q[0]), 0xF5, 0xF, 0xF, false));
                            q[3] = static_cast<unsigned>(__builtin_amdgcn_mov_dpp(static_cast<int>(q[1]), 0xF5, 0xF, 0xF, false));
                            const unsigned lim_x = FULL ? static_cast<unsigned>(pa.P) : (static_cast<unsigned>(remaining) > kj ? umin(static_cast<unsigned>(remaining) - kj, static_cast<unsigned>(pa.P)) : 0u);
                            const bool even = (lane_t & 1u) == 0u;
                            if (even && my_out + 3 < lim_x) {
                                if (ring_opts & 2048u) {
                                    v4u_t qq; __builtin_memcpy(&qq, q, 16);
                                    asm volatile("global_store_dwordx4 %0, %1, off sc0 sc1" ::"v"(dst), "v"(qq) : "memory");
                                } else store_wt<16>(dst, q);
                                covered = true;
                            }
                            else if (!even && my_out + 1 < lim_x) covered = true;
                        }
                    }
                    if (!covered) {
                    if constexpr (FULL) {
                        if (my_out + 1 < static_cast<unsigned>(pa.P)) put2();
                    } else {
                        const unsigned rem_j = static_cast<unsigned>(remaining) > kj ? static_cast<unsigned>(remaining) - kj : 0u;
                        const unsigned lim = rem_j < static_cast<unsigned>(pa.P) ? rem_j : static_cast<unsigned>(pa.P);
                        if (my_out + 1 < lim) put2();
                        else if (my_out < lim) put1();
                    }
                    }
                }
            }
            lgkm_wait<0>(pring[0]);
            static_for<0, KP>([&](auto I) { pin(pring[decltype(I)::value]); });
        };
        if (full) run_steps(std::true_type{});
        else run_steps(std::false_type{});
        if constexpr (RING) {
            if (ring_flags & 1u) {
                pend = true; p_stage = s;
                p_slot = ring_slot; p_shard = ring_shard; p_cnt = ring_cnt; p_nshards = ring_nshards; p_seq_lo = ring_seq_lo; p_seq_hi = ring_seq_hi;
                if (ring_opts & 2u) {
                    pend = false;
                    vm_drain();
                    if (lane == 0) {
                        unsigned *const wg_done = reinterpret_cast<unsigned *>(smem + pa.flags_off) + kRingTileWords * pa.ns;
                        const unsigned prev = __hip_atomic_fetch_add(wg_done + p_stage, 1u, __ATOMIC_RELAXED, __HIP_MEMORY_SCOPE_WORKGROUP);
                        if (prev + 1u == static_cast<unsigned>(ncw)) {
                            __hip_atomic_store(wg_done + p_stage, 0u, __ATOMIC_RELAXED, __HIP_MEMORY_SCOPE_WORKGROUP);
                            ring_grab_done(a.ring_dev, a.ring_host, p_slot, (static_cast<unsigned long long>(p_seq_hi) << 32) | p_seq_lo, p_shard, p_cnt, p_nshards);
                        }
                    }
                }
            }
        }
    }
    if constexpr (RING) {
        if ((ring_opts & 256u) && lane == 0) {
            atomicAdd(&a.ring_dev->stats[0], wall_clock64() - rs_t0);
            atomicAdd(&a.ring_dev->stats[1], rs_bar);
            atomicAdd(&a.ring_dev->stats[2], rs_drain);
            atomicAdd(&a.ring_dev->stats[3], 1ull);
        }
    }
#ifdef MRHIP_OPAIR_PROBE
    if (pa.probe && lane == 0) {
        unsigned long long *r = pa.probe + (static_cast<unsigned long long>(blockIdx.x) * 8u + static_cast<unsigned>(wave)) * 4u;
        const unsigned hw = __builtin_amdgcn_s_getreg(0xF804), xcc = __builtin_amdgcn_s_getreg(0xF814);
        r[0] = hw | (static_cast<unsigned long long>(xcc) << 32);
        r[1] = clock64() - pr_t0; r[2] = pr_wait; r[3] = pr_tiles | ((wall_clock64() - pr_w0) << 32);
    }
#endif
}

template <typename TXS, typename R>
constexpr bool opair_plain_instantiated(bool fused, int nc, int smin, int T)
{
    return !fused && smin <= 1 && (T == 24 || T == 32) && (nc >= 1) && sizeof(TXS) >= 4 && sizeof(R) >= 4;
}
template <int T, bool FUSED, int NC, int SMIN, typename TXS, typename R>
PairKernelFn opair_select(int mode)
{
    if constexpr (opair_plain_instantiated<TXS, R>(FUSED, NC, SMIN, T)) {
        if (mode == 1) return rational_opair_kernel<T, FUSED, NC, SMIN, TXS, R, 1>;
        if (mode == 2) return rational_opair_kernel<T, FUSED, NC, SMIN, TXS, R, 2>;
        if (mode == 3) return rational_opair_kernel<T, FUSED, NC, SMIN, TXS, R, 3>;
    } else if (mode == 2) return nullptr;
    return rational_opair_kernel<T, FUSED, NC, SMIN, TXS, R>;
}
template <bool FUSED, int NC, int SMIN, typename TXS, typename R>
hipError_t launch_opair_T(int T, dim3 block, size_t lds, hipStream_t s, const PolyArgs &a, PairArgs pa, int num_cus)
{
    const bool plain = !a.ring_dev && !a.dyn && !a.multi && MRHIP_ENV_INT("MRHIP_OPAIR_PLAIN", 1);
    const int mode = a.ring_dev ? 2 : !plain ? 0 : a.n_out * a.nch >= (1LL << 22) ? 1 : 3;
#define MRHIP_CASE(TT) \
    case TT: if constexpr (opair_instantiated(FUSED, SMIN, TT)) return launch_opair_kernel(opair_select<TT, FUSED, NC, SMIN, TXS, R>(mode), \
        reinterpret_cast<const void *>(rational_opair_kernel<TT, FUSED, NC, SMIN, TXS, R>), block, lds, s, a, pa, num_cus); else break;
#ifdef MRHIP_OPAIR_LONG
    switch (T) {
#ifdef MRHIP_PS_FAST_BUILD
        MRHIP_CASE(56) MRHIP_CASE(64)
#else
        MRHIP_CASE(49) MRHIP_CASE(50) MRHIP_CASE(51) MRHIP_CASE(52) MRHIP_CASE(53) MRHIP_CASE(54) MRHIP_CASE(55) MRHIP_CASE(56)
        MRHIP_CASE(57) MRHIP_CASE(58) MRHIP_CASE(59) MRHIP_CASE(60) MRHIP_CASE(61) MRHIP_CASE(62) MRHIP_CASE(63) MRHIP_CASE(64)
#endif
    default: break;
    }
#else
    switch (T) {
#ifdef MRHIP_PS_FAST_BUILD
        MRHIP_CASE(24)
#else
        MRHIP_CASE(1) MRHIP_CASE(2) MRHIP_CASE(3) MRHIP_CASE(4) MRHIP_CASE(5) MRHIP_CASE(6) MRHIP_CASE(7) MRHIP_CASE(8)
        MRHIP_CASE(9) MRHIP_CASE(10) MRHIP_CASE(11) MRHIP_CASE(12) MRHIP_CASE(13) MRHIP_CASE(14) MRHIP_CASE(15) MRHIP_CASE(16)
        MRHIP_CASE(17) MRHIP_CASE(18) MRHIP_CASE(19) MRHIP_CASE(20) MRHIP_CASE(21) MRHIP_CASE(22) MRHIP_CASE(23) MRHIP_CASE(24)
        MRHIP_CASE(25) MRHIP_CASE(26) MRHIP_CASE(27) MRHIP_CASE(28) MRHIP_CASE(29) MRHIP_CASE(30) MRHIP_CASE(31) MRHIP_CASE(32)
#endif
    default: break;
    }
    if constexpr ((sizeof(R) == 4 || (NC == 1 && MRHIP_OPAIR_WIDE_LONG)) && SMIN <= 1) {
        switch (T) {
#ifndef MRHIP_PS_FAST_BUILD
        MRHIP_CASE(33) MRHIP_CASE(34) MRHIP_CASE(35) MRHIP_CASE(36) MRHIP_CASE(37) MRHIP_CASE(38) MRHIP_CASE(39) MRHIP_CASE(40)
        MRHIP_CASE(41) MRHIP_CASE(42) MRHIP_CASE(43) MRHIP_CASE(44) MRHIP_CASE(45) MRHIP_CASE(46) MRHIP_CASE(47) MRHIP_CASE(48)
#else
        MRHIP_CASE(36) MRHIP_CASE(48)
#endif
        default: break;
        }
    }
#endif
    return hipErrorInvalidValue;
#undef MRHIP_CASE
}

}
}
```

multirate.jl_amd/csrc/pair_device.h:

```cpp
#ifndef MRHIP_PAIR_DEVICE_H
#define MRHIP_PAIR_DEVICE_H

#include <hip/hip_runtime.h>
#include <type_traits>

#pragma clang fp contract(off)

namespace mrhip {
namespace dev {

typedef unsigned v2u_t __attribute__((ext_vector_type(2)));

template <int I, int N, typename F>
__device__ __forceinline__ void static_for(F &&f)
{
    if constexpr (I < N) {
        f(std::integral_constant<int, I>{});
        static_for<I + 1, N>(f);
    }
}

template <int OFF>
__device__ __forceinline__ v2u_t lds_read_b64(unsigned byte_addr)
{
    v2u_t v;
    asm volatile("ds_read_b64 %0, %1 offset:%2" : "=v"(v) : "v"(byte_addr), "n"(OFF));
    return v;
}
typedef unsigned v4u_t __attribute__((ext_vector_type(4)));
template <int P0>
__device__ __forceinline__ v4u_t lds_read2_b64(unsigned byte_addr)
{
    v4u_t v;
    asm volatile("ds_read2_b64 %0, %1 offset0:%2 offset1:%3" : "=v"(v) : "v"(byte_addr), "n"(P0), "n"(P0 + 1));
    return v;
}
template <int OFF>
__device__ __forceinline__ v4u_t lds_read_b128(unsigned byte_addr)
{
    v4u_t v;
    asm volatile("ds_read_b128 %0, %1 offset:%2" : "=v"(v) : "v"(byte_addr), "n"(OFF));
    return v;
}
template <int N, typename V>
__device__ __forceinline__ void lgkm_wait(V &reg)
{
    asm volatile("s_waitcnt lgkmcnt(%1)" : "+v"(reg) : "n"(N < 15 ? N : 15));
}

template <int N, typename V>
__device__ __forceinline__ void lgkm_wait2(V &reg_a, V &reg_b)
{
    asm volatile("s_waitcnt lgkmcnt(%2)" : "+v"(reg_a), "+v"(reg_b) : "n"(N < 15 ? N : 15));
}

__device__ __forceinline__ unsigned umin(unsigned a, unsigned b) { return a < b ? a : b; }
template <typename V>
__device__ __forceinline__ void pin(V &reg)
{
    asm volatile("" : "+v"(reg));
}
__device__ __forceinline__ void lds_write_b32(unsigned byte_addr, float v)
{
    asm volatile("ds_write_b32 %0, %1" ::"v"(byte_addr), "v"(v));
}
typedef float v2f_t __attribute__((ext_vector_type(2)));
__device__ __forceinline__ void lds_write_b64(unsigned byte_addr, v2f_t v)
{
    asm volatile("ds_write_b64 %0, %1" ::"v"(byte_addr), "v"(v));
}

__device__ __forceinline__ void dma16(const void *gsrc, void *lds_wave_base)
{
    __builtin_amdgcn_global_load_lds((const __attribute__((address_space(1))) void *)gsrc,
                                     (__attribute__((address_space(3))) void *)lds_wave_base, 16, 0, 0);
}

__device__ __forceinline__ void dma16_sc1(const void *gsrc, void *lds_wave_base)
{
    __builtin_amdgcn_global_load_lds((const __attribute__((address_space(1))) void *)gsrc,
                                     (__attribute__((address_space(3))) void *)lds_wave_base, 16, 0, 16);
}

__device__ __forceinline__ void dma16_nt(const void *gsrc, void *lds_wave_base)
{
    __builtin_amdgcn_global_load_lds((const __attribute__((address_space(1))) void *)gsrc,
                                     (__attribute__((address_space(3))) void *)lds_wave_base, 16, 0, 2);
}

template <typename TX, int NC>
__device__ __forceinline__ void shiftin_by_last_workgroup(const ShiftFold &sf, const void *x, const void *hist, long long x_stride, long long x_len, int H, int nch)
{
    if (!sf.hist_new) return;
    __shared__ int s_last;
    if (!sf.done) {
        if (blockIdx.x + 1u != gridDim.x || blockIdx.y != 0u || blockIdx.z != 0u) return;
        s_last = 1;
    } else {
    __syncthreads();
    if (threadIdx.x == 0) {
        const unsigned total = gridDim.x * gridDim.y * gridDim.z;
        const bool last = __hip_atomic_fetch_add(sf.done, 1u, __ATOMIC_RELAXED, __HIP_MEMORY_SCOPE_AGENT) == total - 1u;
        if (last) __hip_atomic_store(sf.done, 0u, __ATOMIC_RELAXED, __HIP_MEMORY_SCOPE_AGENT);
        s_last = last ? 1 : 0;
    }
    __syncthreads();
    }
    if (!s_last) return;
    const long long total = static_cast<long long>(nch) * H;
    for (long long t = threadIdx.x; t < total; t += blockDim.x) {
        const long long ch = t / H, i = t - ch * H;
        const long long e = i + x_len;
        const TX *src = e < H ? static_cast<const TX *>(hist) + (ch * H + e) * NC : static_cast<const TX *>(x) + (ch * x_stride + (e - H)) * NC;
        TX *dst = static_cast<TX *>(sf.hist_new) + t * NC;
#pragma unroll
        for (int c = 0; c < NC; ++c) dst[c] = src[c];
    }
}

__device__ __forceinline__ v4u_t lds_read16_now(unsigned byte_addr)
{
    v4u_t v;
    asm volatile("ds_read_b128 %0, %1\n\ts_waitcnt lgkmcnt(0)" : "=&v"(v) : "v"(byte_addr) : "memory");
    return v;
}

__device__ __forceinline__ unsigned long long ld_sc1(const unsigned long long *p) { return __hip_atomic_load(p, __ATOMIC_RELAXED, __HIP_MEMORY_SCOPE_AGENT); }
__device__ __forceinline__ unsigned ld_sc1(const unsigned *p) { return __hip_atomic_load(p, __ATOMIC_RELAXED, __HIP_MEMORY_SCOPE_AGENT); }
__device__ __forceinline__ float ld_sc1(const float *p) { return __uint_as_float(__hip_atomic_load(reinterpret_cast<const unsigned *>(p), __ATOMIC_RELAXED, __HIP_MEMORY_SCOPE_AGENT)); }
__device__ __forceinline__ void st_sc1(unsigned long long *p, unsigned long long v) { __hip_atomic_store(p, v, __ATOMIC_RELAXED, __HIP_MEMORY_SCOPE_AGENT); }
__device__ __forceinline__ void st_sc1(unsigned *p, unsigned v) { __hip_atomic_store(p, v, __ATOMIC_RELAXED, __HIP_MEMORY_SCOPE_AGENT); }
__device__ __forceinline__ void st_sc1(float *p, float v) { __hip_atomic_store(reinterpret_cast<unsigned *>(p), __float_as_uint(v), __ATOMIC_RELAXED, __HIP_MEMORY_SCOPE_AGENT); }
__device__ __forceinline__ unsigned long long ld_sys(const unsigned long long *p) { return __hip_atomic_load(p, __ATOMIC_RELAXED, __HIP_MEMORY_SCOPE_SYSTEM); }
__device__ __forceinline__ void st_sys(unsigned long long *p, unsigned long long v) { __hip_atomic_store(p, v, __ATOMIC_RELAXED, __HIP_MEMORY_SCOPE_SYSTEM); }
__device__ __forceinline__ void vm_drain() { asm volatile("s_waitcnt vmcnt(0)" ::: "memory"); }
__device__ __forceinline__ void ld96_sc1(const void *p, v4u_t (&d)[6])
{
    asm volatile("global_load_dwordx4 %0, %6, off sc1\n\t"
                 "global_load_dwordx4 %1, %6, off offset:16 sc1\n\t"
                 "global_load_dwordx4 %2, %6, off offset:32 sc1\n\t"
                 "global_load_dwordx4 %3, %6, off offset:48 sc1\n\t"
                 "global_load_dwordx4 %4, %6, off offset:64 sc1\n\t"
                 "global_load_dwordx4 %5, %6, off offset:80 sc1\n\t"
                 "s_waitcnt vmcnt(0)"
                 : "=&v"(d[0]), "=&v"(d[1]), "=&v"(d[2]), "=&v"(d[3]), "=&v"(d[4]), "=&v"(d[5])
                 : "v"(p)
                 : "memory");
}
__device__ __forceinline__ void ld32_sys(const void *p0, const void *p1, v4u_t &d0, v4u_t &d1)
{
    asm volatile("global_load_dwordx4 %0, %2, off sc0 sc1\n\t"
                 "global_load_dwordx4 %1, %3, off sc0 sc1\n\t"
                 "s_waitcnt vmcnt(0)"
                 : "=&v"(d0), "=&v"(d1)
                 : "v"(p0), "v"(p1)
                 : "memory");
}
template <int N>
__device__ __forceinline__ void store_wt(void *dst, const void *regs)
{
    if constexpr (N == 4) {
        unsigned v; __builtin_memcpy(&v, regs, 4);
        asm volatile("global_store_dword %0, %1, off sc1" ::"v"(dst), "v"(v) : "memory");
    } else if constexpr (N == 8) {
        v2u_t v; __builtin_memcpy(&v, regs, 8);
        asm volatile("global_store_dwordx2 %0, %1, off sc1" ::"v"(dst), "v"(v) : "memory");
    } else if constexpr (N == 16) {
        v4u_t v; __builtin_memcpy(&v, regs, 16);
        asm volatile("global_store_dwordx4 %0, %1, off sc1" ::"v"(dst), "v"(v) : "memory");
    } else {
        static_assert(N == 32, "store_wt");
        v4u_t v0, v1; __builtin_memcpy(&v0, regs, 16); __builtin_memcpy(&v1, static_cast<const char *>(regs) + 16, 16);
        asm volatile("global_store_dwordx4 %0, %1, off sc1\n\tglobal_store_dwordx4 %0, %2, off offset:16 sc1" ::"v"(dst), "v"(v0), "v"(v1) : "memory");
    }
}

__device__ __forceinline__ void wait_vmcnt_le(int n)
{
    switch (n) {
#define MRHIP_W(K) case K: asm volatile("s_waitcnt vmcnt(" #K ")" ::: "memory"); break;
        MRHIP_W(0) MRHIP_W(1) MRHIP_W(2) MRHIP_W(3) MRHIP_W(4) MRHIP_W(5) MRHIP_W(6) MRHIP_W(7) MRHIP_W(8) MRHIP_W(9)
        MRHIP_W(10) MRHIP_W(11) MRHIP_W(12) MRHIP_W(13) MRHIP_W(14) MRHIP_W(15) MRHIP_W(16) MRHIP_W(17) MRHIP_W(18) MRHIP_W(19)
        MRHIP_W(20) MRHIP_W(21) MRHIP_W(22) MRHIP_W(23) MRHIP_W(24) MRHIP_W(25) MRHIP_W(26) MRHIP_W(27) MRHIP_W(28) MRHIP_W(29)
        MRHIP_W(30) MRHIP_W(31) MRHIP_W(32) MRHIP_W(33) MRHIP_W(34) MRHIP_W(35) MRHIP_W(36) MRHIP_W(37) MRHIP_W(38) MRHIP_W(39)
        MRHIP_W(40) MRHIP_W(41) MRHIP_W(42) MRHIP_W(43) MRHIP_W(44) MRHIP_W(45) MRHIP_W(46) MRHIP_W(47) MRHIP_W(48) MRHIP_W(49)
        MRHIP_W(50) MRHIP_W(51) MRHIP_W(52) MRHIP_W(53) MRHIP_W(54) MRHIP_W(55) MRHIP_W(56) MRHIP_W(57) MRHIP_W(58) MRHIP_W(59)
        MRHIP_W(60)
#undef MRHIP_W
    default: asm volatile("s_waitcnt vmcnt(0)" ::: "memory"); break;
    }
}

template <bool FUSED>
__device__ __forceinline__ float macf(float t, float x, float acc)
{
    if constexpr (FUSED) return __builtin_fmaf(t, x, acc);
    else { const float p = t * x; return acc + p; }
}

#define MRHIP_MASKED_SLOT_OPS(R, SFX)                                                                                                     \
                                                                                       \
    template <bool FUSED>                                                                                                                 \
    __device__ __forceinline__ void masked_mac(R (&acc)[1], R tap, const R (&w)[1], unsigned long long m)                                 \
    {                                                                                                                                     \
        unsigned long long sv;                                                                                                            \
        if constexpr (FUSED)                                                                                                              \
            asm("s_and_saveexec_b64 %[sv], %[m]\n\tv_fma_" SFX " %[a0], %[t], %[w0], %[a0]\n\ts_mov_b64 exec, %[sv]"                      \
                : [a0] "+v"(acc[0]), [sv] "=&s"(sv) : [t] "v"(tap), [w0] "v"(w[0]), [m] "s"(m) : "scc");                                  \
        else {                                                                                                                            \
            R p0;                                                                                                                         \
            asm("s_and_saveexec_b64 %[sv], %[m]\n\tv_mul_" SFX " %[p0], %[t], %[w0]\n\tv_add_" SFX " %[a0], %[a0], %[p0]\n\t"             \
                "s_mov_b64 exec, %[sv]"                                                                                                   \
                : [a0] "+v"(acc[0]), [p0] "=&v"(p0), [sv] "=&s"(sv) : [t] "v"(tap), [w0] "v"(w[0]), [m] "s"(m) : "scc");                  \
        }                                                                                                                                 \
    }                                                                                                                                     \
    template <bool FUSED>                                                                                                                 \
    __device__ __forceinline__ void masked_mac(R (&acc)[2], R tap, const R (&w)[2], unsigned long long m)                                 \
    {                                                                                                                                     \
        unsigned long long sv;                                                                                                            \
        if constexpr (FUSED)                                                                                                              \
            asm("s_and_saveexec_b64 %[sv], %[m]\n\tv_fma_" SFX " %[a0], %[t], %[w0], %[a0]\n\tv_fma_" SFX " %[a1], %[t], %[w1], %[a1]\n\t" \
                "s_mov_b64 exec, %[sv]"                                                                                                   \
                : [a0] "+v"(acc[0]), [a1] "+v"(acc[1]), [sv] "=&s"(sv) : [t] "v"(tap), [w0] "v"(w[0]), [w1] "v"(w[1]), [m] "s"(m) : "scc"); \
        else {                                                                                                                            \
            R p0, p1;                                                                                                                     \
            asm("s_and_saveexec_b64 %[sv], %[m]\n\tv_mul_" SFX " %[p0], %[t], %[w0]\n\tv_mul_" SFX " %[p1], %[t], %[w1]\n\t"              \
                "v_add_" SFX " %[a0], %[a0], %[p0]\n\tv_add_" SFX " %[a1], %[a1], %[p1]\n\ts_mov_b64 exec, %[sv]"                         \
                : [a0] "+v"(acc[0]), [a1] "+v"(acc[1]), [p0] "=&v"(p0), [p1] "=&v"(p1), [sv] "=&s"(sv)                                    \
                : [t] "v"(tap), [w0] "v"(w[0]), [w1] "v"(w[1]), [m] "s"(m) : "scc");                                                      \
        }                                                                                                                                 \
    }                                                                                                                                     \
                                                       \
    __device__ __forceinline__ void masked_mul_add(R (&acc)[1], R tap, const R (&w)[1], unsigned long long m)                             \
    {                                                                                                                                     \
        unsigned long long sv;                                                                                                            \
        R p0;                                                                                                                             \
        asm("s_and_saveexec_b64 %[sv], %[m]\n\tv_mul_" SFX " %[p0], %[t], %[w0]\n\tv_add_" SFX " %[a0], %[p0], %[a0]\n\t"                 \
            "s_mov_b64 exec, %[sv]"                                                                                                       \
            : [a0] "+v"(acc[0]), [p0] "=&v"(p0), [sv] "=&s"(sv) : [t] "v"(tap), [w0] "v"(w[0]), [m] "s"(m) : "scc");                      \
    }                                                                                                                                     \
    __device__ __forceinline__ void masked_mul_add(R (&acc)[2], R tap, const R (&w)[2], unsigned long long m)                             \
    {                                                                                                                                     \
        unsigned long long sv;                                                                                                            \
        R p0, p1;                                                                                                                         \
        asm("s_and_saveexec_b64 %[sv], %[m]\n\tv_mul_" SFX " %[p0], %[t], %[w0]\n\tv_mul_" SFX " %[p1], %[t], %[w1]\n\t"                  \
            "v_add_" SFX " %[a0], %[p0], %[a0]\n\tv_add_" SFX " %[a1], %[p1], %[a1]\n\ts_mov_b64 exec, %[sv]"                             \
            : [a0] "+v"(acc[0]), [a1] "+v"(acc[1]), [p0] "=&v"(p0), [p1] "=&v"(p1), [sv] "=&s"(sv)                                        \
            : [t] "v"(tap), [w0] "v"(w[0]), [w1] "v"(w[1]), [m] "s"(m) : "scc");                                                          \
    }                                                                                                                                     \
                                       \
    __device__ __forceinline__ void masked_mul(R (&s)[1], R tap, const R (&w)[1], unsigned long long m)                                   \
    {                                                                                                                                     \
        unsigned long long sv;                                                                                                            \
        asm("s_and_saveexec_b64 %[sv], %[m]\n\tv_mul_" SFX " %[s0], %[t], %[w0]\n\ts_mov_b64 exec, %[sv]"                                 \
            : [s0] "=&v"(s[0]), [sv] "=&s"(sv) : [t] "v"(tap), [w0] "v"(w[0]), [m] "s"(m) : "scc");                                       \
    }                                                                                                                                     \
    __device__ __forceinline__ void masked_mul(R (&s)[2], R tap, const R (&w)[2], unsigned long long m)                                   \
    {                                                                                                                                     \
        unsigned long long sv;                                                                                                            \
        asm("s_and_saveexec_b64 %[sv], %[m]\n\tv_mul_" SFX " %[s0], %[t], %[w0]\n\tv_mul_" SFX " %[s1], %[t], %[w1]\n\t"                  \
            "s_mov_b64 exec, %[sv]"                                                                                                       \
            : [s0] "=&v"(s[0]), [s1] "=&v"(s[1]), [sv] "=&s"(sv) : [t] "v"(tap), [w0] "v"(w[0]), [w1] "v"(w[1]), [m] "s"(m) : "scc");     \
    }                                                                                                                                     \
                                                                                                                       \
    __device__ __forceinline__ void masked_add(R (&acc)[1], const R (&s)[1], unsigned long long m)                                        \
    {                                                                                                                                     \
        unsigned long long sv;                                                                                                            \
        asm("s_and_saveexec_b64 %[sv], %[m]\n\tv_add_" SFX " %[a0], %[s0], %[a0]\n\ts_mov_b64 exec, %[sv]"                                \
            : [a0] "+v"(acc[0]), [sv] "=&s"(sv) : [s0] "v"(s[0]), [m] "s"(m) : "scc");                                                    \
    }                                                                                                                                     \
    __device__ __forceinline__ void masked_add(R (&acc)[2], const R (&s)[2], unsigned long long m)                                        \
    {                                                                                                                                     \
        unsigned long long sv;                                                                                                            \
        asm("s_and_saveexec_b64 %[sv], %[m]\n\tv_add_" SFX " %[a0], %[s0], %[a0]\n\tv_add_" SFX " %[a1], %[s1], %[a1]\n\t"                \
            "s_mov_b64 exec, %[sv]"                                                                                                       \
            : [a0] "+v"(acc[0]), [a1] "+v"(acc[1]), [sv] "=&s"(sv) : [s0] "v"(s[0]), [s1] "v"(s[1]), [m] "s"(m) : "scc");                 \
    }                                                                                                                                     \
// ... 66 lines not shown
```

multirate.jl_amd/csrc/pair_loader.h:

```cpp
#ifndef MRHIP_PAIR_LOADER_H
#define MRHIP_PAIR_LOADER_H

#include "mrhip_internal.h"
#include "pair_device.h"

namespace mrhip {
namespace dev {

struct TileAt { int ch, st, jt; };

__device__ __forceinline__ TileAt pair_tile_at(const PairArgs &pa, unsigned g, unsigned jt)
{
    const unsigned spc = pa.steps_per_channel;
    unsigned q = __umulhi(g, pa.spc_magic);
    unsigned r = g - q * spc;
    if (r >= spc) { ++q; r -= spc; }
    if (r >= spc) { ++q; r -= spc; }
    return TileAt{static_cast<int>(q), static_cast<int>(r), static_cast<int>(umin(jt, spc - r))};
}

__device__ __forceinline__ void pair_take_dyn(PolyArgs &a, PairArgs &pa)
{
#ifdef MRHIP_NO_TAKE_DYN
    return;
#endif
    if (a.multi) {
        const MultiDesc *__restrict__ d = a.multi + (blockIdx.x % static_cast<unsigned>(a.multi_n));
        a.x = d->x; a.y = d->y; a.hist = d->hist; a.hist_new = d->hist_new; a.taps = d->taps; a.rec = d->rec;
        a.x_stride = d->x_stride; a.y_stride = d->y_stride; a.x_len = d->x_len; a.n_out = d->n_out;
        a.u0 = d->u0; a.d0 = d->d0; a.phi_end = d->phi_end; a.d_end = d->d_end; a.nch = d->nch;
        pa.o0 = d->d0 - a.T;
        if (d->P_blk > 0) { pa.P = d->P_blk; pa.q0 = d->q0; pa.o0 += d->q0; }
        pa.steps_per_channel = d->steps_per_channel;
        pa.total_steps = d->total_steps;
        pa.spc_magic = d->spc_magic;
        pa.steps_per_group = d->total_steps;
    }
    if (a.dyn) {
        const DevCall *__restrict__ d = a.dyn;
        a.n_out = d->n_out; a.u0 = d->u0; a.d0 = d->d0;
        a.x_len = d->x_len;
        pa.o0 = d->d0 - a.T;
        pa.steps_per_channel = d->steps_per_channel;
        pa.total_steps = d->total_steps;
        pa.spc_magic = d->spc_magic;
        pa.steps_per_group = (pa.total_steps + static_cast<unsigned>(pa.ngroups) - 1u) / static_cast<unsigned>(pa.ngroups);
    }
}

template <int NC, bool FAST_SEAM = true>
__device__ __forceinline__ void pair_loader_wave(const PolyArgs &a, const PairArgs &pa, unsigned char *smem, int lane)
{
    volatile unsigned *const tile_flag = reinterpret_cast<volatile unsigned *>(smem + pa.flags_off);
    auto tile_at = [&](unsigned g, unsigned jt) -> TileAt { return pair_tile_at(pa, g, jt); };
    const unsigned pad_magic = pa.pad_every > 0 ? 0xffffffffu / static_cast<unsigned>(pa.pad_every + 1) + 1u : 0u;
    auto stage_tile = [&](const TileAt &ta, int stage) -> int {
        const int sch = ta.ch;
        constexpr int EPC = 4 / NC;
        const int rc = pa.run_chunks;
        const int tlen = rc > 0 ? ta.jt * rc * EPC : (ta.jt * pa.cM + pa.tail + EPC - 1) / EPC * EPC;
        const int nchunks = tlen / EPC;
        const int cd = pa.pad_every;
        const int nlds = cd > 0 ? (nchunks + cd - 1) / cd * (cd + 1) : nchunks;
        const int nslots = (nlds + 63) >> 6;
        const float *__restrict__ xc = static_cast<const float *>(a.x) + static_cast<long long>(sch) * a.x_stride * NC;
        const long long o = pa.o0 + static_cast<long long>(ta.st) * pa.cM;
        unsigned char *st = smem + static_cast<size_t>(stage) * pa.stage_bytes;
        const long long o_end = rc > 0 ? o + static_cast<long long>(ta.jt - 1) * pa.cM + rc * EPC : o + tlen;
        const bool interior = o >= 0 && o_end <= a.x_len;
        auto chunk_sample = [&](int c) -> long long {
            if (rc <= 0) return static_cast<long long>(EPC) * c;
            unsigned j = __umulhi(static_cast<unsigned>(c), pa.run_magic);
            int w = c - static_cast<int>(j) * rc;
            if (w < 0) { --j; w += rc; }
            return static_cast<long long>(j) * pa.cM + static_cast<long long>(EPC) * w;
        };
        if (interior) {
            const unsigned char *src = reinterpret_cast<const unsigned char *>(xc + o * NC);
            if (rc > 0) {
                for (int slot = 0; slot < nslots; ++slot) {
                    const int ci = slot * 64 + lane;
                    const int cis = ci < nchunks ? ci : 0;
                    dma16(src + static_cast<size_t>(chunk_sample(cis)) * (NC * 4u), st + static_cast<size_t>(slot) * 1024);
                }
                return nslots;
            }
            for (int slot = 0; slot < nslots; ++slot) {
                const int ci = slot * 64 + lane;
                int d = ci;
                if (cd > 0) { const int g = static_cast<int>(__umulhi(static_cast<unsigned>(ci), pad_magic)), r = ci - g * (cd + 1); d = r == cd ? 0 : g * cd + r; }
                const int cis = d < nchunks ? d : 0;
                dma16(src + static_cast<size_t>(cis) * 16, st + static_cast<size_t>(slot) * 1024);
            }
            return nslots;
        }
        if constexpr (FAST_SEAM) {
            const unsigned char *src = reinterpret_cast<const unsigned char *>(xc + o * NC);
            const unsigned char *dummy = static_cast<const unsigned char *>(a.taps);
            for (int slot = 0; slot < nslots; ++slot) {
                const int ci = slot * 64 + lane;
                int d = ci;
                bool data = ci < nlds;
                if (cd > 0) { const int g = static_cast<int>(__umulhi(static_cast<unsigned>(ci), pad_magic)), r = ci - g * (cd + 1); data = data && r != cd; d = g * cd + r; }
                data = data && d < nchunks;
                const long long smp = data ? chunk_sample(d) : 0;
                const bool inside = data && o + smp >= 0 && o + smp + EPC <= a.x_len;
                dma16(inside ? src + smp * (NC * 4) : dummy, st + static_cast<size_t>(slot) * 1024);
            }
            asm volatile("s_waitcnt vmcnt(0)" ::: "memory");
        }
        const float *__restrict__ hc = static_cast<const float *>(a.hist) + static_cast<long long>(sch) * a.H * NC;
        float *l = reinterpret_cast<float *>(st);
        for (int ci = lane; ci < nchunks; ci += 64) {
            const long long g0 = o + chunk_sample(ci);
            if constexpr (FAST_SEAM) { if (g0 >= 0 && g0 + EPC <= a.x_len) continue; }
            float4 v;
            float *pv = reinterpret_cast<float *>(&v);
#pragma unroll
            for (int e = 0; e < EPC; ++e) {
                const long long gi = g0 + e;
#pragma unroll
                for (int cc = 0; cc < NC; ++cc) {
                    float val = 0.f;
                    if (gi >= 0) { if (gi < a.x_len) val = xc[gi * NC + cc]; }
                    else if (gi >= -static_cast<long long>(a.H)) val = hc[(a.H + gi) * NC + cc];
                    pv[e * NC + cc] = val;
                }
            }
            *reinterpret_cast<float4 *>(l + (cd > 0 ? ci + ci / cd : ci) * 4) = v;
        }
        asm volatile("s_waitcnt vmcnt(0) lgkmcnt(0)" ::: "memory");
        return 0;
    };
    const unsigned grp = blockIdx.x % static_cast<unsigned>(pa.ngroups);
    const unsigned grp_lo = a.multi ? 0u : umin(grp * pa.steps_per_group, pa.total_steps);
    const unsigned grp_hi = umin(grp_lo + pa.steps_per_group, pa.total_steps);
    unsigned *const ctr = pa.counters + grp * 64u;
    unsigned pend = 0;
    unsigned static_next = blockIdx.x / static_cast<unsigned>(pa.ngroups);
    const unsigned static_stride = (gridDim.x + static_cast<unsigned>(pa.ngroups) - 1u - grp) / static_cast<unsigned>(pa.ngroups);
    auto grab_issue = [&]() {
        if (pa.static_grabs) { pend = static_next; static_next += static_stride; }
        else if (lane == 0) pend = atomicAdd(ctr, 1u);
    };
    unsigned ra = 0, rb = 0;
    bool more = true;
    auto grab_take = [&]() {
        const unsigned t = static_cast<unsigned>(__builtin_amdgcn_readfirstlane(static_cast<int>(pend)));
        const unsigned long long lo = static_cast<unsigned long long>(grp_lo) + static_cast<unsigned long long>(t) * pa.J;
        if (lo < grp_hi) { ra = static_cast<unsigned>(lo); rb = umin(ra + pa.J, grp_hi); grab_issue(); }
        else { more = false; ra = rb = 0; }
    };
    unsigned long long hist = 0;
    auto newest_ops = [&](int ntiles) -> int {
        int n = 0;
        for (int k = 0; k < ntiles; ++k) n += static_cast<int>((hist >> (6 * k)) & 63u);
        return n < 60 ? n : 60;
    };
    auto produce = [&](int stage) -> bool {
        if (ra >= rb && more) grab_take();
        if (ra >= rb) {
            if (lane == 0) { tile_flag[2 * stage] = 0u; tile_flag[2 * stage + 1] = 0u; }
            hist <<= 6;
            return false;
        }
        const TileAt ta = tile_at(ra, rb - ra);
        if (lane == 0) { tile_flag[2 * stage] = ra; tile_flag[2 * stage + 1] = static_cast<unsigned>(ta.jt); }
        hist = (hist << 6) | static_cast<unsigned>((pa.ablate & 1) ? 0 : stage_tile(ta, stage));
        ra += static_cast<unsigned>(ta.jt);
        return true;
    };
    grab_issue();
    unsigned pipeline = 0;
    for (int k = 0; k < pa.ns - 1; ++k)
        if (produce(k)) pipeline |= 1u << k;
    if (pa.bank_off >= 0) __builtin_amdgcn_s_barrier();
    wait_vmcnt_le(newest_ops(pa.ns - 2));
    int pstage = pa.ns - 1;
#ifdef MRHIP_OPAIR_PROBE
    unsigned long long pr_bar = 0, pr_vm = 0;
    const unsigned long long pr_t0 = clock64();
#endif
    for (;;) {
        asm volatile("s_waitcnt lgkmcnt(0)" ::: "memory");
#ifdef MRHIP_OPAIR_PROBE
        const unsigned long long pr_a = clock64();
#endif
        __builtin_amdgcn_s_barrier();
#ifdef MRHIP_OPAIR_PROBE
        pr_bar += clock64() - pr_a;
#endif
        if (!(pipeline & 1u)) break;
        pipeline >>= 1;
        if (produce(pstage)) pipeline |= 1u << (pa.ns - 2);
        pstage = pstage + 1 == pa.ns ? 0 : pstage + 1;
#ifdef MRHIP_OPAIR_PROBE
        const unsigned long long pr_b = clock64();
#endif
        wait_vmcnt_le(newest_ops(pa.ns - 2));
#ifdef MRHIP_OPAIR_PROBE
        pr_vm += clock64() - pr_b;
#endif
    }
#ifdef MRHIP_OPAIR_PROBE
    if (pa.probe && lane == 0) {
        unsigned long long *r = pa.probe + (static_cast<unsigned long long>(blockIdx.x) * 8u + 7u) * 4u;
        const unsigned hw = __builtin_amdgcn_s_getreg(0xF804), xcc = __builtin_amdgcn_s_getreg(0xF814);
        r[0] = hw | (static_cast<unsigned long long>(xcc) << 32) | (1ULL << 63);
        r[1] = clock64() - pr_t0; r[2] = pr_bar; r[3] = pr_vm;
    }
#endif
    if (lane == 0 && !pa.static_grabs) {
        unsigned *const done = pa.counters + static_cast<unsigned>(pa.ngroups) * 64u;
        if (atomicAdd(done, 1u) == gridDim.x - 1) {
            for (int k = 0; k < pa.ngroups; ++k) pa.counters[k * 64] = 0u;
            *done = 0u;
        }
    }
    const unsigned wg_in_grp = blockIdx.x / static_cast<unsigned>(pa.ngroups);
    if ((a.multi ? wg_in_grp == 0u : blockIdx.x == 0) && lane == 0 && a.rec && !a.dyn) {
        a.rec->phiIdx = a.phi_end;
        a.rec->inputDeficit = a.d_end;
        a.rec->n_written = a.n_out;
        a.rec->calls += 1;
    }
    if (a.H > 0) {
        const float *__restrict__ xin = static_cast<const float *>(a.x);
        const float *__restrict__ hold = static_cast<const float *>(a.hist);
        float *__restrict__ hnew = static_cast<float *>(a.hist_new);
        const int c_first = a.multi ? static_cast<int>(wg_in_grp) : static_cast<int>(blockIdx.x);
        const int c_step = a.multi ? static_cast<int>(static_stride) : static_cast<int>(gridDim.x);
        for (int c2 = c_first; c2 < a.nch; c2 += c_step)
            for (int i = lane; i < a.H; i += 64) {
                const long long e = static_cast<long long>(i) + a.x_len;
#pragma unroll
                for (int cc = 0; cc < NC; ++cc)
                    hnew[(static_cast<long long>(c2) * a.H + i) * NC + cc] =
                        e < a.H ? hold[(static_cast<long long>(c2) * a.H + e) * NC + cc]
                                : xin[(static_cast<long long>(c2) * a.x_stride + (e - a.H)) * NC + cc];
            }
    }
}


constexpr unsigned kRingTileWords = 16;

__device__ __forceinline__ void ring_grab_done(RingDev *rd, RingHost *rh, unsigned slot, unsigned long long seq, unsigned shard, unsigned cnt, unsigned nshards_wt)
{
    const bool wt = (nshards_wt >> 31) != 0u;
    const unsigned nshards = nshards_wt & 0x7fffffffu;
    const unsigned prev = __hip_atomic_fetch_add(&rd->shard_done[slot][shard][0], 1u, __ATOMIC_RELAXED, __HIP_MEMORY_SCOPE_AGENT);
    if (prev + 1u == cnt) {
        st_sc1(&rd->shard_done[slot][shard][0], 0u);
        vm_drain();
        const unsigned top = __hip_atomic_fetch_add(&rd->chunk_done[slot], 1u, __ATOMIC_RELAXED, __HIP_MEMORY_SCOPE_AGENT);
        if (top + 1u == nshards) {
            st_sc1(&rd->chunk_done[slot], 0u);
            vm_drain();
            if (wt) st_sys(&rh->done[slot], seq + 1ull);
            else {
                const unsigned long long r = __hip_atomic_fetch_add(&rd->flush_req, 1ull, __ATOMIC_RELAXED, __HIP_MEMORY_SCOPE_AGENT) + 1ull;
                const unsigned long long ent[2] = {r, seq};
                store_wt<16>(&rd->flush_ent[r % kRingDepth][0], ent);
                vm_drain();
            }
        }
    }
}
__device__ __forceinline__ unsigned ring_shard_count(unsigned long long tb, unsigned n, unsigned s)
{
    const unsigned long long S = kRingShards;
    auto below = [&](unsigned long long e) -> unsigned long long { return e > s ? (e - s + S - 1ull) / S : 0ull; };
    return static_cast<unsigned>(below(tb + n) - below(tb));
}

__device__ __forceinline__ void ring_feeder(RingDev *rd, RingHost *rh, int lane)
{
    unsigned long long last = 0, t0 = wall_clock64(), code = 0;
    unsigned long long fb = 0, ft = 0, fd = 0;
    const unsigned long long idle = ld_sc1(&rd->idle_ticks);
    const int du = lane & 7, dk = lane >> 3;
    constexpr int KU = kRingKeyQword / 2;
    bool whole = false;
    for (;;) {
        if (!whole) {
            const unsigned long long arr = ld_sc1(&rd->arrived);
            if (lane == 0) { st_sys(&rh->grid, static_cast<unsigned long long>(gridDim.x)); st_sys(&rh->arrived, arr); }
            whole = arr >= gridDim.x;
        }
        const unsigned long long h = ld_sys(&rh->head);
        const unsigned long long tseen = wall_clock64();
        if (h > last) {
            const unsigned nb = h - last < 16ull ? static_cast<unsigned>(h - last) : 16u;
            const unsigned k0 = static_cast<unsigned>(dk), k1 = static_cast<unsigned>(dk) + 8u;
            const bool on0 = k0 < nb && du < 6, on1 = k1 < nb && du < 6;
            const unsigned char *h0 = reinterpret_cast<const unsigned char *>(&rh->desc[(last + (on0 ? k0 : 0u)) % kRingDepth]) + 16 * (du < 6 ? du : 0);
            const unsigned char *h1 = reinterpret_cast<const unsigned char *>(&rh->desc[(last + (on1 ? k1 : 0u)) % kRingDepth]) + 16 * (du < 6 ? du : 0);
            v4u_t u0, u1;
            ld32_sys(h0, h1, u0, u1);
            unsigned char *d0 = reinterpret_cast<unsigned char *>(&rd->desc[(last + k0) % kRingDepth]) + 16 * du;
            unsigned char *d1 = reinterpret_cast<unsigned char *>(&rd->desc[(last + k1) % kRingDepth]) + 16 * du;
            if (on0 && du != KU) store_wt<16>(d0, &u0);
            if (on1 && du != KU) store_wt<16>(d1, &u1);
            vm_drain();
            if (on0 && du == KU) { u0.w = static_cast<unsigned>((last + k0) & 0xffffffffull); store_wt<16>(d0, &u0); }
            if (on1 && du == KU) { u1.w = static_cast<unsigned>((last + k1) & 0xffffffffull); store_wt<16>(d1, &u1); }
            vm_drain();
            last += nb;
            if (lane == 0) st_sc1(&rd->head, last);
            {
                const unsigned long long t1 = wall_clock64();
                if (lane == 0) {
                    if (fb < static_cast<unsigned long long>(kRingTraceTiles)) { rd->trace[0][3 * fb] = tseen; rd->trace[0][3 * fb + 1] = t1; rd->trace[0][3 * fb + 2] = last; }
                    fb += 1; ft += t1 - tseen; fd += nb;
                }
                t0 = t1;
            }
            continue;
        }
        if (ld_sc1(&rd->closed) != 0ull) { code = 3; break; }
        if (ld_sys(&rh->close) != 0ull) {
            if (ld_sys(&rh->head) == last) { code = 1; break; }
            continue;
        }
        if (wall_clock64() - t0 > idle) { code = 2; break; }
        __builtin_amdgcn_s_sleep(8);
    }
    vm_drain();
    if (lane == 0) {
        atomicAdd(&rd->stats[13], fb); atomicAdd(&rd->stats[14], ft); atomicAdd(&rd->stats[15], fd);
        if (code != 3) st_sc1(&rd->closed, code);
        vm_drain();
        st_sys(&rh->stopped, code);
    }
    vm_drain();
}

__device__ __attribute__((noinline)) void ring_flush_duty(RingDev *rd, RingHost *rh, unsigned xcc, unsigned long long req, int lane)
{
    unsigned long long won = 0;
    if (lane == 0) won = __hip_atomic_fetch_max(&rd->flush_claim[xcc][0], req, __ATOMIC_RELAXED, __HIP_MEMORY_SCOPE_AGENT) < req ? 1ull : 0ull;
    if (!__builtin_amdgcn_readfirstlane(static_cast<int>(won))) return;
    __builtin_amdgcn_fence(__ATOMIC_RELEASE, "agent");
    asm volatile("s_waitcnt vmcnt(0)" ::: "memory");
    if (lane != 0) return;
    (void)__hip_atomic_fetch_max(&rd->flush_done[xcc][0], req, __ATOMIC_RELAXED, __HIP_MEMORY_SCOPE_AGENT);
    unsigned long long F = ~0ull;
    for (int x = 0; x < 8; ++x) {
        const unsigned long long d = __hip_atomic_fetch_max(&rd->flush_done[x][0], 0ull, __ATOMIC_RELAXED, __HIP_MEMORY_SCOPE_AGENT);
        F = d < F ? d : F;
    }
    const unsigned long long P = __hip_atomic_fetch_max(&rd->flush_pub, F, __ATOMIC_RELAXED, __HIP_MEMORY_SCOPE_AGENT);
    for (unsigned long long r = P + 1ull; r <= F; ++r) {
        unsigned long long seq;
        for (;;) {
            v4u_t e;
            asm volatile("global_load_dwordx4 %0, %1, off sc1\n\ts_waitcnt vmcnt(0)" : "=&v"(e) : "v"(&rd->flush_ent[r % kRingDepth][0]) : "memory");
            if (((static_cast<unsigned long long>(e.y) << 32) | e.x) == r) { seq = (static_cast<unsigned long long>(e.w) << 32) | e.z; break; }
            __builtin_amdgcn_s_sleep(1);
        }
        st_sys(&rh->done[seq % kRingDepth], seq + 1ull);
    }
}

template <int NC>
__device__ __attribute__((noinline)) void ring_stage_seam(const float *xc, long long o, long long xlen, const float *hc, int H, int nchunks, int cd,
                                                          unsigned char *st, const unsigned char *dummy, int nslots, int lane)
{
    constexpr int EPC = 4 / NC;
    {
        const unsigned char *src = reinterpret_cast<const unsigned char *>(xc + o * NC);
        for (int slot = 0; slot < nslots; ++slot) {
            const int ci = slot * 64 + lane;
            const bool data = ci < nchunks;
            const long long smp = static_cast<long long>(EPC) * (data ? ci : 0);
            const bool inside = data && o + smp >= 0 && o + smp + EPC <= xlen;
            dma16_sc1(inside ? src + smp * (NC * 4) : dummy, st + static_cast<size_t>(slot) * 1024);
        }
        asm volatile("s_waitcnt vmcnt(0)" ::: "memory");
    }
    float *l = reinterpret_cast<float *>(st);
    for (int ci = lane; ci < nchunks; ci += 64) {
        const long long g0 = o + static_cast<long long>(EPC) * ci;
        if (g0 >= 0 && g0 + EPC <= xlen) continue;
        float4 v;
        float *pv = reinterpret_cast<float *>(&v);
#pragma unroll
        for (int e = 0; e < EPC; ++e) {
            const long long gi = g0 + e;
#pragma unroll
            for (int cc = 0; cc < NC; ++cc) {
                float val = 0.f;
                if (gi >= 0) { if (gi < xlen) val = ld_sc1(xc + gi * NC + cc); }
                else if (gi >= -static_cast<long long>(H)) val = ld_sc1(hc + (H + gi) * NC + cc);
// ... 349 lines not shown
```

multirate.jl_amd/host.py:

```python
from __future__ import annotations

import ctypes as C
import os
from fractions import Fraction

import numpy as np

try:
    import torch
except Exception:
    torch = None

_HERE = os.path.dirname(os.path.abspath(__file__))

F32, F64, C64, C128 = 0, 1, 2, 3
STANDARD, DECIMATOR, INTERPOLATOR, RATIONAL, ARBITRARY, FARROW = 0, 1, 2, 3, 4, 5
KIND_NAMES = {STANDARD: "FIRStandard", DECIMATOR: "FIRDecimator", INTERPOLATOR: "FIRInterpolator",
              RATIONAL: "FIRRational", ARBITRARY: "FIRArbitrary", FARROW: "FIRFarrow"}
NUMERICS_STRICT, NUMERICS_FUSED = 0, 1

_NP2DT = {np.dtype(np.float32): F32, np.dtype(np.float64): F64,
          np.dtype(np.complex64): C64, np.dtype(np.complex128): C128}
_DT2NP = {v: k for k, v in _NP2DT.items()}


class MultirateHIPError(RuntimeError):

    def __init__(self, code: int, msg: str):
        super().__init__(f"[mrhip status {code}] {msg}")
        self.code = code


class _State(C.Structure):
    _fields_ = [("kind", C.c_int32), ("tap_dtype", C.c_int32), ("sample_dtype", C.c_int32),
                ("output_dtype", C.c_int32), ("nchannels", C.c_int64), ("hLen", C.c_int64),
                ("interpolation", C.c_int64), ("decimation", C.c_int64), ("Nphi", C.c_int64),
                ("tapsPerPhi", C.c_int64), ("historyLen", C.c_int64), ("phiIdx", C.c_int64),
                ("inputDeficit", C.c_int64), ("xIdx", C.c_int64), ("rate", C.c_double),
                ("phiAccumulator", C.c_double), ("alpha", C.c_double), ("delta", C.c_double)]


_vp, _i64, _i, _d = C.c_void_p, C.c_int64, C.c_int, C.c_double
_pi64 = C.POINTER(C.c_int64)
ABI = [
    ("mrhip_abi_version", _i, []),
    ("mrhip_last_error", C.c_char_p, []),
    ("mrhip_device_count", _i, []),
    ("mrhip_taps2pfb", _i64, [_vp, _i64, _i, _i64, _vp]),
    ("mrhip_nextphase", _i64, [_i64, _i64, _i64]),
    ("mrhip_outputlength_ratio", _i64, [_i64, _i64, _i64, _i64]),
    ("mrhip_inputlength_ratio", _i64, [_i64, _i64, _i64, _i64]),
    ("mrhip_polyfit", _i, [_vp, _i64, _i64, _vp]),
    ("mrhip_output_dtype", _i, [_i, _i]),
    ("mrhip_kaiserlength", _i, [_d, _d, _d, _pi64, C.POINTER(C.c_double)]),
    ("mrhip_kaiser", _i, [_i64, _d, _vp]),
    ("mrhip_firprototype", _i64, [_i64, _vp, _i, _i, _vp]),
    ("mrhip_firdes", _i64, [_i64, _vp, _i, _i, _d, _d, _vp, _vp]),
    ("mrhip_firdes_kaiser", _i64, [_vp, _i, _d, _d, _i, _d, _vp]),
    ("mrhip_create_rational", _i, [_vp, _i64, _i, _i64, _i64, _i, _i64, _i, C.POINTER(_vp)]),
    ("mrhip_create_rational_bank", _i, [_vp, _i64, _i, _i64, _i64, _i, _i64, _i, C.POINTER(_vp)]),
    ("mrhip_create_rational_bank_ctaps", _i, [_vp, _i64, _i, _i64, _i64, _i, _i64, _i, C.POINTER(_vp)]),
    ("mrhip_create_arbitrary", _i, [_vp, _i64, _i, _d, _i64, _i, _i64, _i, C.POINTER(_vp)]),
    ("mrhip_create_arbitrary_ctaps", _i, [_vp, _i64, _i, _d, _i64, _i, _i64, _i, C.POINTER(_vp)]),
    ("mrhip_create_farrow", _i, [_vp, _i64, _i, _d, _i64, _i64, _i, _i64, _i, C.POINTER(_vp)]),
    ("mrhip_create_farrow_pnfb", _i, [_vp, _i64, _i, _d, _i64, _i64, _i, _i64, _i, C.POINTER(_vp)]),
    ("mrhip_create_farrow_ctaps", _i, [_vp, _i64, _i, _d, _i64, _i64, _i, _i64, _i, C.POINTER(_vp)]),
    ("mrhip_create_farrow_pnfb_ctaps", _i, [_vp, _i64, _i, _d, _i64, _i64, _i, _i64, _i, C.POINTER(_vp)]),
    ("mrhip_get_pnfb", _i, [_vp, _vp]),
    ("mrhip_farrow_tapsforphase", _i, [_vp, _d, _vp]),
    ("mrhip_arbitrary_tapsforphase", _i, [_vp, _d, _vp]),
    ("mrhip_destroy", None, [_vp]),
    ("mrhip_outputlength", _i64, [_vp, _i64]),
    ("mrhip_next_output_count", _i64, [_vp, _i64]),
    ("mrhip_advance_state", _i64, [_vp, _i64]),
    ("mrhip_inputlength", _i64, [_vp, _i64]),
    ("mrhip_get_state", _i, [_vp, C.POINTER(_State)]),
    ("mrhip_set_state", _i, [_vp, _i64, _i64, _d]),
    ("mrhip_get_history", _i, [_vp, _vp]),
    ("mrhip_set_history", _i, [_vp, _vp]),
    ("mrhip_reset", _i, [_vp]),
    ("mrhip_set_numerics", _i, [_vp, _i]),
    ("mrhip_set_mod_form", _i, [_vp, _i]),
    ("mrhip_get_taps", _i, [_vp, _i, _vp]),
    ("mrhip_filt_device", _i, [_vp, _vp, _i64, _i64, _vp, _i64, _i64, _pi64, _vp]),
    ("mrhip_filt_device_async", _i, [_vp, _vp, _i64, _i64, _vp, _i64, _i64, _vp, _vp]),
    ("mrhip_filt_device_chained", _i, [_vp, _vp, _vp, _i64, _i64, _vp, _i64, _i64, _vp, _vp]),
    ("mrhip_filt_device_multi", _i, [C.POINTER(_vp), _i, C.POINTER(_vp), _pi64, C.POINTER(_vp), _pi64, _pi64, _vp]),
    ("mrhip_outputlength_bound", _i64, [_vp, _i64]),
    ("mrhip_sync_state", _i, [_vp, _pi64]),
    ("mrhip_set_history_device", _i, [_vp, _vp, _vp]),
    ("mrhip_filt_device_chunked", _i, [_vp, _vp, _i64, _i64, _i64, _vp, _i64, _i64, _pi64, _vp]),
    ("mrhip_filt_host", _i, [_vp, _vp, _i64, _i64, _vp, _i64, _i64, _pi64]),
    ("mrhip_synchronize", _i, [_vp, _vp]),
    ("mrhip_cascade_create", _i, [C.POINTER(_vp), _i, C.POINTER(_vp)]),
    ("mrhip_cascade_destroy", None, [_vp]),
    ("mrhip_cascade_outputlength", _i64, [_vp, _i64]),
    ("mrhip_cascade_next_output_count", _i64, [_vp, _i64]),
    ("mrhip_cascade_filt_device", _i, [_vp, _vp, _i64, _i64, _vp, _i64, _i64, _pi64, _vp]),
    ("mrhip_cascade_filt_device_async", _i, [_vp, _vp, _i64, _i64, _vp, _i64, _i64, _vp, _vp]),
    ("mrhip_cascade_reset", _i, [_vp]),
    ("mrhip_filt_once", _i, [_vp, _i64, _i, _i64, _i64, _d, _i64, _vp, _i64, _i, _vp, _i64, _pi64, _i]),
    ("mrhip_set_timing", _i, [_vp, _i]),
    ("mrhip_timing_read", _i, [_vp, _pi64, C.POINTER(C.c_double)]),
    ("mrhip_last_kernel_name", C.c_char_p, [_vp]),
    ("mrhip_schedule_info", _i, [_vp, _pi64, _i]),
    ("mrhip_sharded_create", _i, [_i, _vp, _i64, _i, _i64, _i64, _d, _i64, _i64, _i, _i64, C.POINTER(_i), _i, C.POINTER(_vp)]),
    ("mrhip_sharded_destroy", None, [_vp]),
    ("mrhip_sharded_nshards", _i, [_vp]),
    ("mrhip_sharded_shard", _i, [_vp, _i, _pi64, _pi64, C.POINTER(_i), C.POINTER(_vp)]),
    ("mrhip_sharded_outputlength", _i64, [_vp, _i64]),
    ("mrhip_sharded_next_output_count", _i64, [_vp, _i64]),
    ("mrhip_sharded_reset", _i, [_vp]),
    ("mrhip_sharded_filt_device", _i, [_vp, C.POINTER(_vp), _i64, _pi64, C.POINTER(_vp), _i64, _pi64, _pi64]),
    ("mrhip_sharded_filt_host", _i, [_vp, _vp, _i64, _i64, _vp, _i64, _i64, _pi64]),
    ("mrhip_sharded_gather", _i, [_vp, C.POINTER(_vp), _i64, _pi64, _vp, _i64, _i]),
    ("mrhip_sharded_wait_stream", _i, [_vp, _i, _vp]),
    ("mrhip_sharded_signal_stream", _i, [_vp, _i, _vp]),
    ("mrhip_sharded_synchronize", _i, [_vp]),
    ("mrhip_ring_open", _i, [_vp, C.POINTER(_vp)]),
    ("mrhip_ring_push", _i, [_vp, _vp, _i64, _i64, _vp, _i64, _i64, _pi64, C.POINTER(C.c_uint64)]),
    ("mrhip_ring_push_chunks", _i, [_vp, _vp, _i64, _i64, _i64, _vp, _i64, _i64, _pi64, C.POINTER(C.c_uint64)]),
    ("mrhip_ring_wait", _i, [_vp, C.c_uint64]),
    ("mrhip_ring_drain", _i, [_vp]),
    ("mrhip_ring_close", _i, [_vp]),
    ("mrhip_ring_info", _i, [_vp, _pi64, _i]),
]

_lib = None


def library_path() -> str:
    return os.environ.get("MRHIP_LIB_PATH") or os.path.join(_HERE, "libmultirate_hip.so")


def load_library():
    global _lib
    if _lib is None:
        path = library_path()
        if not os.path.exists(path):
            raise MultirateHIPError(-1, f"{path} not found: build it with `make -C multirate.jl_amd/csrc` "
                                        "(or __graft_entry__.build()); there is no CPU fallback")
        lib = C.CDLL(path)
        for name, res, args in ABI:
            fn = getattr(lib, name)
            fn.restype = res
            fn.argtypes = args
        if lib.mrhip_abi_version() != 1:
            raise MultirateHIPError(-1, "ABI version mismatch")
        _lib = lib
    return _lib


def _check(rc: int):
    if rc != 0:
        raise MultirateHIPError(rc, load_library().mrhip_last_error().decode("utf-8", "replace"))


def _ptr(a: np.ndarray):
    return a.ctypes.data_as(C.c_void_p)


def _as_taps(h, allow_complex: bool = False) -> np.ndarray:
    h = np.ascontiguousarray(h)
    if h.dtype == np.float32 or h.dtype == np.float64:
        return h
    if np.issubdtype(h.dtype, np.integer) or h.dtype == np.float16:
        return h.astype(np.float64)
    if h.dtype == np.complex64 or h.dtype == np.complex128:
        if allow_complex:
            return h
        raise MultirateHIPError(5, f"tap dtype {h.dtype}: complex taps are built with FIRFilter.complex_taps(h, ratio) "
                                   "(the rational family only); this constructor takes Float32/Float64 taps")
    raise MultirateHIPError(5, f"unsupported tap dtype {h.dtype} (taps must be Float32/Float64, or Complex64/Complex128 "
                               "through FIRFilter.complex_taps)")


def _is_torch(x) -> bool:
    return torch is not None and isinstance(x, torch.Tensor)


def _torch_np_dtype(t):
    return {torch.float32: np.dtype(np.float32), torch.float64: np.dtype(np.float64),
            torch.complex64: np.dtype(np.complex64), torch.complex128: np.dtype(np.complex128)}[t]


def _np_torch_dtype(d):
    return {np.dtype(np.float32): torch.float32, np.dtype(np.float64): torch.float64,
            np.dtype(np.complex64): torch.complex64, np.dtype(np.complex128): torch.complex128}[np.dtype(d)]


def taps2pfb(h, Nphi: int) -> np.ndarray:
    h = _as_taps(h, allow_complex=True)
    lib = load_library()
    T = lib.mrhip_taps2pfb(_ptr(h), len(h), _NP2DT[h.dtype], Nphi, None)
    if T < 0:
        raise MultirateHIPError(1, "bad taps2pfb arguments")
    out = np.empty(T * Nphi, dtype=h.dtype)
    lib.mrhip_taps2pfb(_ptr(h), len(h), _NP2DT[h.dtype], Nphi, _ptr(out))
    return out.reshape(Nphi, T).T.copy()


def polyfit(y, polyorder: int) -> np.ndarray:
    y = np.ascontiguousarray(y, dtype=np.float64)
    out = np.zeros(polyorder + 1, dtype=np.float64)
    _check(load_library().mrhip_polyfit(_ptr(y), len(y), polyorder, _ptr(out)))
    return out


def nextphase(currentphase: int, ratio) -> int:
    r = Fraction(ratio)
    return load_library().mrhip_nextphase(currentphase, r.numerator, r.denominator)


class FIRFilter:

    def __init__(self, h, ratio=Fraction(1, 1), Nphi: int = 32, polyorder=None, *, device: int = 0,
                 numerics: int = NUMERICS_STRICT, pnfb=None, _complex_taps: bool = False):
        self._lib = load_library()
        self.h = _as_taps(h, allow_complex=_complex_taps).copy()
        if len(self.h) < 1:
            raise MultirateHIPError(1, "h must hold at least one tap")
        self.device = int(device)
        self.numerics = int(numerics)
        self._handle = None
        self._tx = None
        self._nch = None
        self.polyorder = None
        self._pnfb_in = None
        self._bank = None
        if isinstance(ratio, (float, np.floating)):
            if not ratio > 0.0:
                raise MultirateHIPError(1, "rate must be greater than 0")
            self.rate = float(ratio)
            self.ratio = None
            self.Nphi = int(Nphi)
            self.kind = ARBITRARY if polyorder is None else FARROW
            self.polyorder = None if polyorder is None else int(polyorder)
            self._pnfb_in = None if pnfb is None else np.ascontiguousarray(pnfb, dtype=np.complex128 if self.h.dtype.kind == "c" else np.float64)
            self.interpolation, self.decimation = self.Nphi, 1
            self.tapsPerPhi = -(-len(self.h) // self.Nphi)
            self.historyLen = self.tapsPerPhi - 1
        else:
            if isinstance(ratio, tuple):
                ratio = Fraction(*ratio)
            self.ratio = Fraction(ratio)
            if self.ratio <= 0:
                raise MultirateHIPError(1, "ratio must be positive")
            self.rate = None
            L, M = self.ratio.numerator, self.ratio.denominator
            self.interpolation, self.decimation = L, M
            if L == 1 and M == 1:
                self.kind = STANDARD
            elif L == 1:
                self.kind = DECIMATOR
            elif M == 1:
                self.kind = INTERPOLATOR
            else:
# ... 81 lines not shown
        elif self._bank is not None:
            rc = self._lib.mrhip_create_rational_bank(_ptr(self._bank), self._bank.shape[1], _NP2DT[self._bank.dtype],
                                                      self.ratio.numerator, self.ratio.denominator, _NP2DT[tx], nch,
                                                      self.device, C.byref(out))
        elif self.kind == FARROW and self.h.dtype.kind == "c":
            if self._pnfb_in is not None:
                rc = self._lib.mrhip_create_farrow_pnfb_ctaps(_ptr(self._pnfb_in), len(self.h), _NP2DT[self.h.dtype], self.rate,
                                                              self.Nphi, self.polyorder, _NP2DT[tx], nch, self.device, C.byref(out))
            else:
                rc = self._lib.mrhip_create_farrow_ctaps(_ptr(self.h), len(self.h), _NP2DT[self.h.dtype], self.rate, self.Nphi,
                                                         self.polyorder, _NP2DT[tx], nch, self.device, C.byref(out))
        elif self.kind == FARROW and self._pnfb_in is not None:
            rc = self._lib.mrhip_create_farrow_pnfb(_ptr(self._pnfb_in), len(self.h), _NP2DT[self.h.dtype], self.rate,
                                                    self.Nphi, self.polyorder, _NP2DT[tx], nch, self.device, C.byref(out))
        elif self.kind == FARROW:
            rc = self._lib.mrhip_create_farrow(_ptr(self.h), len(self.h), _NP2DT[self.h.dtype], self.rate, self.Nphi,
                                               self.polyorder, _NP2DT[tx], nch, self.device, C.byref(out))
        elif self.kind == ARBITRARY and self.h.dtype.kind == "c":
            rc = self._lib.mrhip_create_arbitrary_ctaps(_ptr(self.h), len(self.h), _NP2DT[self.h.dtype], self.rate,
                                                        self.Nphi, _NP2DT[tx], nch, self.device, C.byref(out))
        elif self.kind == ARBITRARY:
            rc = self._lib.mrhip_create_arbitrary(_ptr(self.h), len(self.h), _NP2DT[self.h.dtype], self.rate,
                                                  self.Nphi, _NP2DT[tx], nch, self.device, C.byref(out))
        else:
            rc = self._lib.mrhip_create_rational(_ptr(self.h), len(self.h), _NP2DT[self.h.dtype],
                                                 self.ratio.numerator, self.ratio.denominator, _NP2DT[tx], nch,
                                                 self.device, C.byref(out))
        _check(rc)
        self._handle, self._tx, self._nch = out, tx, nch
        if self.numerics != NUMERICS_STRICT:
            _check(self._lib.mrhip_set_numerics(self._handle, self.numerics))

    def close(self):
        if getattr(self, "_handle", None):
            self._lib.mrhip_destroy(self._handle)
            self._handle = None

    def __del__(self):
        try:
            self.close()
        except Exception:
            pass

    @property
    def kernel_name(self) -> str:
        return KIND_NAMES[self.kind]

    @property
    def output_dtype(self):
        if self._tx is None:
            return None
        return _DT2NP[self._lib.mrhip_output_dtype(_NP2DT[self.h.dtype], _NP2DT[self._tx])]

    @property
    def state(self) -> _State:
        st = _State()
        if self._handle is None:
            st.kind = self.kind
            st.phiIdx, st.inputDeficit, st.xIdx = 1, 1, 1
            st.phiAccumulator, st.alpha = 1.0, 0.0
            st.Nphi, st.tapsPerPhi, st.historyLen = self.Nphi, self.tapsPerPhi, self.historyLen
            st.interpolation, st.decimation, st.hLen = self.interpolation, self.decimation, len(self.h)
            st.rate = self.rate or 0.0
            st.delta = self.Nphi / self.rate if self.rate else 0.0
            return st
        _check(self._lib.mrhip_get_state(self._handle, C.byref(st)))
        return st

    def set_state(self, phiIdx: int = 1, inputDeficit: int = 1, phiAccumulator: float = 1.0):
        if self._handle is None:
            raise MultirateHIPError(1, "set_state needs a bound filter (call filt once, or bind())")
        _check(self._lib.mrhip_set_state(self._handle, phiIdx, inputDeficit, phiAccumulator))

    def bind(self, dtype, nchannels: int = 1):
        self._ensure(np.dtype(dtype), int(nchannels))
        return self

    @property
    def history(self) -> np.ndarray:
        if self._handle is None:
            return np.zeros(self.historyLen)
        out = np.zeros((self._nch, self.historyLen), dtype=self._tx)
        _check(self._lib.mrhip_get_history(self._handle, _ptr(out)))
        return out[0] if self._nch == 1 else out

    def set_history(self, hist):
        hist = np.ascontiguousarray(hist, dtype=self._tx).reshape(self._nch, self.historyLen)
        _check(self._lib.mrhip_set_history(self._handle, _ptr(hist)))

    def taps(self, which: int = 0) -> np.ndarray:
        if self._handle is None:
            raise MultirateHIPError(1, "taps() needs a bound filter")
        if self._bank is not None:
            out = np.zeros((self._nch, self.Nphi, self.tapsPerPhi), dtype=self.h.dtype)
            _check(self._lib.mrhip_get_taps(self._handle, which, _ptr(out)))
            return out.transpose(0, 2, 1).copy()
        out = np.zeros(self.tapsPerPhi * self.Nphi, dtype=self.h.dtype)
        _check(self._lib.mrhip_get_taps(self._handle, which, _ptr(out)))
        return out.reshape(self.Nphi, self.tapsPerPhi).T.copy()

    def pnfb(self) -> np.ndarray:
        if self._handle is None or self.kind != FARROW:
            raise MultirateHIPError(1, "pnfb() needs a bound FIRFarrow filter")
        out = np.zeros((self.tapsPerPhi, self.polyorder + 1), dtype=np.complex128 if self.h.dtype.kind == "c" else np.float64)
        _check(self._lib.mrhip_get_pnfb(self._handle, _ptr(out)))
        return out

    def tapsforphase(self, phase: float) -> np.ndarray:
        if self._handle is None or self.kind not in (ARBITRARY, FARROW):
            raise MultirateHIPError(1, "tapsforphase() needs a bound FIRArbitrary or FIRFarrow filter")
        out = np.zeros(self.tapsPerPhi, dtype=self.h.dtype)
        fn = self._lib.mrhip_farrow_tapsforphase if self.kind == FARROW else self._lib.mrhip_arbitrary_tapsforphase
        _check(fn(self._handle, float(phase), _ptr(out)))
        return out

    def setphase(self, phi: float):
        if not 0.0 <= phi <= 1.0:
            raise MultirateHIPError(1, "phase must be in [0, 1]")
        if self._handle is None:
            raise MultirateHIPError(1, "setphase needs a bound filter (call filt once, or bind())")
        st = self.state
        if self.kind in (INTERPOLATOR, RATIONAL):
            idx = min(int(phi * self.Nphi) + 1, self.Nphi)
            self.set_state(idx, st.inputDeficit, 1.0)
            return idx
        if self.kind == ARBITRARY:
            import math
            alpha, idx = math.modf(phi * self.Nphi)
            acc = min(max(idx + alpha, 1.0), math.nextafter(self.Nphi + 1.0, 0.0))
            self.set_state(1, st.inputDeficit, acc)
            return idx, alpha
        if self.kind == FARROW:
            acc = phi * (self.Nphi - 1) + 1
            self.set_state(1, st.inputDeficit, acc)
            return acc
        raise MultirateHIPError(5, f"setphase is not defined for {self.kernel_name}")

    def set_mod_form(self, julia03: bool):
        if self._handle is None:
            raise MultirateHIPError(1, "set_mod_form needs a bound filter (call filt once, or bind())")
        _check(self._lib.mrhip_set_mod_form(self._handle, 1 if julia03 else 0))

    def set_timing(self, enabled=True):
        _check(self._lib.mrhip_set_timing(self._handle, int(enabled)))

    def timing_read(self):
        n, ms = C.c_int64(0), C.c_double(0.0)
        _check(self._lib.mrhip_timing_read(self._handle, C.byref(n), C.byref(ms)))
        return int(n.value), float(ms.value)

    def last_kernel_name(self) -> str:
        return self._lib.mrhip_last_kernel_name(self._handle).decode()

    def schedule_info(self) -> dict:
        v = (C.c_int64 * 8)()
        _check(self._lib.mrhip_schedule_info(self._handle, v, 8))
        keys = ("device_ok", "ncand", "nwin", "period", "host_steps", "periodic_steps", "device_pieces", "fallback_pieces")
        return dict(zip(keys, (int(a) for a in v)))

    def outputlength(self, inputlength: int) -> int:
        if self._handle is None:
            self_state = self.state
            if self.kind == STANDARD:
                return inputlength
            if self.kind == INTERPOLATOR:
                return self.interpolation * inputlength
            if self.kind in (ARBITRARY, FARROW):
                import math
                return int(math.ceil((inputlength - self_state.inputDeficit + 1) * self.rate))
            return self._lib.mrhip_outputlength_ratio(inputlength, self.interpolation, self.decimation, 1)
        return self._lib.mrhip_outputlength(self._handle, inputlength)

    def inputlength(self, outputlength: int) -> int:
        if self._handle is None:
            if self.kind in (ARBITRARY, FARROW):
                raise MultirateHIPError(5, "inputlength is not defined for FIRArbitrary in the reference")
            return self._lib.mrhip_inputlength_ratio(outputlength, self.interpolation, self.decimation, 1)
        n = self._lib.mrhip_inputlength(self._handle, outputlength)
        if n < 0:
            raise MultirateHIPError(5, "inputlength is not defined for FIRArbitrary in the reference")
        return n

    def advance_state(self, inputlength: int) -> int:
        if self._handle is None:
            raise MultirateHIPError(1, "advance_state needs a bound filter (call filt once, or bind())")
        n = self._lib.mrhip_advance_state(self._handle, int(inputlength))
        if n < 0:
            raise MultirateHIPError(1, self._lib.mrhip_last_error().decode("utf-8", "replace"))
        return n

    def next_output_count(self, inputlength: int) -> int:
        if self._handle is None:
            raise MultirateHIPError(1, "next_output_count needs a bound filter")
        return self._lib.mrhip_next_output_count(self._handle, inputlength)

    def reset(self):
        if self._handle is not None:
            _check(self._lib.mrhip_reset(self._handle))
        return self

    def _shape(self, x):
        if x.ndim == 1:
            return 1, x.shape[0], True
        if x.ndim == 2:
            return x.shape[0], x.shape[1], False
        raise MultirateHIPError(1, "x must be (n,) or (nchannels, n)")

    def filt_into(self, buffer, x) -> int:
        nw = C.c_int64(0)
        if _is_torch(x):
            if not x.is_cuda:
                raise MultirateHIPError(1, "torch input must live on the GPU (use numpy for host data)")
            if x.stride(-1) != 1 or buffer.stride(-1) != 1:
                raise MultirateHIPError(1, "x and buffer must be contiguous along time (planar channels)")
            nch, n, _ = self._shape(x)
            self._ensure(_torch_np_dtype(x.dtype), nch)
            if _torch_np_dtype(buffer.dtype) != self.output_dtype:
                raise MultirateHIPError(1, f"buffer dtype must be {self.output_dtype}")
            if x.device.index != self.device or buffer.device != x.device:
                raise MultirateHIPError(1, "x / buffer are not on the filter's device")
            cap = buffer.shape[-1]
            xs = x.stride(0) if x.ndim == 2 and nch > 1 else n
            ys = buffer.stride(0) if buffer.ndim == 2 and nch > 1 else cap
            if buffer.ndim != x.ndim or (x.ndim == 2 and buffer.shape[0] != nch):
                raise MultirateHIPError(1, "buffer must have one row per channel")
            stream = torch.cuda.current_stream(x.device).cuda_stream
            _check(self._lib.mrhip_filt_device(self._handle, C.c_void_p(x.data_ptr()), n, xs,
                                               C.c_void_p(buffer.data_ptr()), cap, ys, C.byref(nw),
                                               C.c_void_p(stream)))
            return nw.value
        x = np.asarray(x)
        if not x.flags.c_contiguous:
            x = np.ascontiguousarray(x)
        nch, n, _ = self._shape(x)
        self._ensure(x.dtype, nch)
        if not isinstance(buffer, np.ndarray) or buffer.dtype != self.output_dtype or not buffer.flags.c_contiguous:
            raise MultirateHIPError(1, f"buffer must be a C-contiguous numpy array of {self.output_dtype}")
        cap = buffer.shape[-1]
        _check(self._lib.mrhip_filt_host(self._handle, _ptr(x), n, n, _ptr(buffer), cap, cap, C.byref(nw)))
        return nw.value

    def outputlength_bound(self, inputlength: int) -> int:
        if self._handle is None:
            raise MultirateHIPError(1, "outputlength_bound needs a bound filter (call filt once, or bind())")
        return self._lib.mrhip_outputlength_bound(self._handle, int(inputlength))

    def filt_into_async(self, buffer, x, count=None, after: "FIRFilter" = None) -> None:
        if not _is_torch(x) or not x.is_cuda:
            raise MultirateHIPError(1, "filt_into_async takes torch device tensors")
        if x.stride(-1) != 1 or buffer.stride(-1) != 1:
            raise MultirateHIPError(1, "x and buffer must be contiguous along time (planar channels)")
        nch, n, _ = self._shape(x)
        self._ensure(_torch_np_dtype(x.dtype), nch)
        if _torch_np_dtype(buffer.dtype) != self.output_dtype:
            raise MultirateHIPError(1, f"buffer dtype must be {self.output_dtype}")
        if buffer.ndim != x.ndim or (x.ndim == 2 and buffer.shape[0] != nch):
            raise MultirateHIPError(1, "buffer must have one row per channel")
        cap = buffer.shape[-1]
        xs = x.stride(0) if x.ndim == 2 and nch > 1 else n
        ys = buffer.stride(0) if buffer.ndim == 2 and nch > 1 else cap
        cptr = None
        if count is not None:
            if not (_is_torch(count) and count.is_cuda and count.dtype == torch.int64 and count.numel() >= 1):
                raise MultirateHIPError(1, "count must be an int64 CUDA tensor")
            cptr = C.c_void_p(count.data_ptr())
        stream = torch.cuda.current_stream(x.device).cuda_stream
        if after is not None:
            if after._handle is None:
                raise MultirateHIPError(1, "after= needs a bound filter")
            _check(self._lib.mrhip_filt_device_chained(self._handle, after._handle, C.c_void_p(x.data_ptr()), n, xs, C.c_void_p(buffer.data_ptr()),
                                                       cap, ys, cptr, C.c_void_p(stream)))
            return
        _check(self._lib.mrhip_filt_device_async(self._handle, C.c_void_p(x.data_ptr()), n, xs, C.c_void_p(buffer.data_ptr()),
                                                 cap, ys, cptr, C.c_void_p(stream)))

    def sync_state(self) -> int:
        nw = C.c_int64(0)
        _check(self._lib.mrhip_sync_state(self._handle, C.byref(nw)))
        return nw.value

    def set_history_device(self, hist) -> None:
        if not _is_torch(hist) or not hist.is_cuda or not hist.is_contiguous():
            raise MultirateHIPError(1, "set_history_device takes a contiguous torch CUDA tensor")
        if _torch_np_dtype(hist.dtype) != self._tx or hist.numel() != self._nch * self.historyLen:
            raise MultirateHIPError(1, f"history must hold {self._nch} x {self.historyLen} samples of {self._tx}")
        stream = torch.cuda.current_stream(hist.device).cuda_stream
        _check(self._lib.mrhip_set_history_device(self._handle, C.c_void_p(hist.data_ptr()), C.c_void_p(stream)))

    def filt_into_chunked(self, buffer, x, chunk: int) -> int:
        if not _is_torch(x) or not x.is_cuda:
            raise MultirateHIPError(1, "filt_into_chunked takes torch device tensors")
        if x.stride(-1) != 1 or buffer.stride(-1) != 1:
            raise MultirateHIPError(1, "x and buffer must be contiguous along time (planar channels)")
        nch, n, _ = self._shape(x)
        self._ensure(_torch_np_dtype(x.dtype), nch)
        if _torch_np_dtype(buffer.dtype) != self.output_dtype:
            raise MultirateHIPError(1, f"buffer dtype must be {self.output_dtype}")
        cap = buffer.shape[-1]
        xs = x.stride(0) if x.ndim == 2 and nch > 1 else n
        ys = buffer.stride(0) if buffer.ndim == 2 and nch > 1 else cap
        nw = C.c_int64(0)
        stream = torch.cuda.current_stream(x.device).cuda_stream
        _check(self._lib.mrhip_filt_device_chunked(self._handle, C.c_void_p(x.data_ptr()), n, xs, int(chunk),
                                                   C.c_void_p(buffer.data_ptr()), cap, ys, C.byref(nw), C.c_void_p(stream)))
        return nw.value

# ... 438 lines not shown
```

Before: 666,900.

## Add balanced opair kernel mode with all waves computing and cooperative tile staging

Adds a balanced MODE 4 variant of the rational output-pair kernel for the f32 M/L in (1,2), T=24 case. It drops the dedicated loader wave: every wave stages the next tile cooperatively, and wave 0 handles the work handout through LDS flag slots. Block size is chosen so lanes fill 8 or 12 whole waves, with a two-stage pipeline and wg_per_cu = 24/nwaves. The aim is to stop leaving a wave idle on loading and to raise occupancy. The trade-off is more synchronous staging inside the compute loop and more complex handout logic.

```diff
diff --git a/include/multirate_hip.h b/include/multirate_hip.h
--- a/include/multirate_hip.h
+++ b/include/multirate_hip.h
@@ -177,6 +177,7 @@
 int mrhip_set_timing(mrhip_filter *f, int enabled);
 int mrhip_timing_read(mrhip_filter *f, int64_t *n_launches, double *total_ms);
 const char *mrhip_last_kernel_name(const mrhip_filter *f);
+int mrhip_opair_plan_info(int64_t *info, int n);
 int mrhip_schedule_info(const mrhip_filter *f, int64_t *info, int n);
 
 #ifdef __cplusplus
diff --git a/multirate.jl_amd/csrc/api.hip b/multirate.jl_amd/csrc/api.hip
--- a/multirate.jl_amd/csrc/api.hip
+++ b/multirate.jl_amd/csrc/api.hip
@@ -313,7 +313,7 @@
             PairArgs pa;
             dim3 block;
             size_t lds = 0;
-            if (plan_rational_opair(tk, fused, a, f->num_cus, &pa, &block, &lds)) {
+            if (plan_rational_opair(tk, fused, a, f->num_cus, &pa, &block, &lds, 0, true)) {
                 *rec_written = true;
                 *did_shiftin = a.H > 0;
                 return launch_rational_opair(fused, a, pa, block, lds, s, kname, f->num_cus, counters);
@@ -2003,6 +2003,13 @@
 
 const char *mrhip_last_kernel_name(const mrhip_filter *f) { return f ? f->last_kernel : ""; }
 
+int mrhip_opair_plan_info(int64_t *info, int n)
+{
+    if (!info || n < 0) return fail(MRHIP_ERR_INVALID_ARG, "mrhip_opair_plan_info: no buffer");
+    opair_last_plan(info, n);
+    return MRHIP_OK;
+}
+
 int mrhip_schedule_info(const mrhip_filter *f, int64_t *info, int n)
 {
     if (!f || !info || n < 0) return fail(MRHIP_ERR_INVALID_ARG, "NULL argument");
diff --git a/multirate.jl_amd/csrc/kernels_rational_opair.hip b/multirate.jl_amd/csrc/kernels_rational_opair.hip
--- a/multirate.jl_amd/csrc/kernels_rational_opair.hip
+++ b/multirate.jl_amd/csrc/kernels_rational_opair.hip
@@ -11,6 +11,7 @@
 hipError_t launch_opair_f32_s0c(bool fused, int T, dim3 block, size_t lds, hipStream_t s, const PolyArgs &a, const PairArgs &pa, int num_cus);
 hipError_t launch_opair_f32_s1r(bool fused, int T, dim3 block, size_t lds, hipStream_t s, const PolyArgs &a, const PairArgs &pa, int num_cus);
 hipError_t launch_opair_f32_s1c(bool fused, int T, dim3 block, size_t lds, hipStream_t s, const PolyArgs &a, const PairArgs &pa, int num_cus);
+hipError_t launch_opair_f32_s1b(int T, dim3 block, size_t lds, hipStream_t s, const PolyArgs &a, const PairArgs &pa, int num_cus);
 hipError_t launch_opair_f32_s0_long(int nc, bool fused, int T, dim3 block, size_t lds, hipStream_t s, const PolyArgs &a, const PairArgs &pa, int num_cus);
 hipError_t launch_opair_f32_s1_long(int nc, bool fused, int T, dim3 block, size_t lds, hipStream_t s, const PolyArgs &a, const PairArgs &pa, int num_cus);
 hipError_t launch_opair_f32_s2(int nc, bool fused, int T, dim3 block, size_t lds, hipStream_t s, const PolyArgs &a, const PairArgs &pa, int num_cus);
@@ -24,9 +25,43 @@
 
 namespace {
 constexpr int kOMaxThreads = 512;
-}
-
-bool plan_rational_opair(const TypeKey &tk, bool fused, const PolyArgs &a, int num_cus, PairArgs *out, dim3 *block, size_t *lds, int force_wgpc)
+constexpr int kOBalThreads = 768;
+thread_local int64_t g_last_plan[10] = {};
+
+int balanced_c(const PolyArgs &a)
+{
+    int best_c = 0;
+    double best = 0.95 - 1e-9;
+    for (int c = 2; static_cast<long long>(c) * a.L / 2 <= kOBalThreads; c += 2) {
+        const int lanes = static_cast<int>(static_cast<long long>(c) * a.L / 2);
+        const int nwaves = (lanes + 63) / 64;
+        if (nwaves != 8 && nwaves != 12) continue;
+        const double fill = static_cast<double>(lanes) / (64.0 * nwaves);
+        if (fill >= best) { best = fill; best_c = c; }
+    }
+    return best_c;
+}
+}
+
+void opair_last_plan(int64_t *info, int n)
+{
+    for (int i = 0; i < n; ++i) info[i] = i < 10 ? g_last_plan[i] : 0;
+}
+
+static bool plan_opair_geometry(const TypeKey &tk, bool fused, const PolyArgs &a, int num_cus, PairArgs *out, dim3 *block, size_t *lds, int force_wgpc, int bal_c);
+
+bool plan_rational_opair(const TypeKey &tk, bool fused, const PolyArgs &a, int num_cus, PairArgs *out, dim3 *block, size_t *lds, int force_wgpc, bool one_filter)
+{
+    const int env_b = MRHIP_ENV_INT("MRHIP_OPAIR_BALANCED", 1);
+    if (env_b > 0 && one_filter && force_wgpc == 0 && !a.dyn && !a.multi && !a.ring_dev && a.L >= 2 && a.M > a.L &&
+        opair_balanced_instantiated(tk, fused, static_cast<int>(a.M / a.L), a.T) && (env_b >= 2 || a.n_out * a.nch >= (1LL << 22)) &&
+        !MRHIP_ENV_INT("MRHIP_OPAIR_C", 0) && !MRHIP_ENV_INT("MRHIP_OPAIR_NS", 0) && !MRHIP_ENV_INT("MRHIP_OPAIR_WGPC", 0)) {
+        if (const int bc = balanced_c(a); bc > 0 && plan_opair_geometry(tk, fused, a, num_cus, out, block, lds, 0, bc)) return true;
+    }
+    return plan_opair_geometry(tk, fused, a, num_cus, out, block, lds, force_wgpc, 0);
+}
+
+static bool plan_opair_geometry(const TypeKey &tk, bool fused, const PolyArgs &a, int num_cus, PairArgs *out, dim3 *block, size_t *lds, int force_wgpc, int bal_c)
 {
     if (!MRHIP_ENV_INT("MRHIP_OPAIR", 1)) return false;
     if (tk.x_f64 && !tk.r_f64) return false;
@@ -56,6 +91,7 @@
         for (int c = 2; static_cast<long long>(c) * a.L / 2 <= kOMaxThreads && static_cast<long long>(c) * a.L <= 1024; c += 2)
             if (static_cast<long long>(c) * a.L / 2 >= 128) { best_c = c; break; }
     if (env_c > 0 && env_c % 2 == 0 && static_cast<long long>(env_c) * a.L / 2 <= kOMaxThreads && static_cast<long long>(env_c) * a.L <= 1024) best_c = env_c;
+    if (bal_c > 0) best_c = bal_c;
     if (!best_c) return false;
     if (tk.r_f64 && a.T > 32 && (static_cast<long long>(best_c) * a.L / 2 + 63) / 64 > 7) return false;
     const int c = best_c;
@@ -69,9 +105,11 @@
     int wg_per_cu = std::max(1, std::min(4, waves_per_cu / (nwaves + 1)));
     if (nwaves + 1 == 6 && !tk.r_f64) wg_per_cu = 3;
     if (nwaves + 1 == 6 && tk.r_f64) wg_per_cu = 1;
+    if (bal_c > 0) wg_per_cu = 24 / nwaves;
     if (force_wgpc > 0) wg_per_cu = force_wgpc;
     if (const int env_w = MRHIP_ENV_INT("MRHIP_OPAIR_WGPC", 0); env_w > 0) wg_per_cu = env_w;
     int ns = env_ns >= 2 && env_ns <= 8 ? env_ns : (wg_per_cu == 1 ? 3 : 2);
+    if (bal_c > 0) ns = 2;
     auto j_for = [&](int stages) -> long long {
         const long long budget_kib = ((wg_per_cu <= 3 ? 150 : 160) * 1024 / wg_per_cu - 64) / stages / 1024;
         const long long j = ((budget_kib > 1 ? budget_kib : 1) * 1024 / es - tail) / cM;
@@ -118,6 +156,14 @@
         const long long pt = (a.T + 4) | 1;
         const bool fits = static_cast<size_t>(a.L * pt * (tk.r_f64 ? 8 : 4)) <= stage_bytes;
         pa.bank_off = (fits && MRHIP_ENV_INT("MRHIP_OPAIR_BANK", 1)) ? static_cast<int>((ns - 1) * stage_bytes) : -1;
+    }
+    if (bal_c > 0) {
+        if (padded > kOBalThreads) return false;
+        pa.balanced = 1;
+        *out = pa;
+        *block = dim3(static_cast<unsigned>(padded));
+        *lds = ns * stage_bytes + 8 * ns;
+        return true;
     }
     *out = pa;
     *block = dim3(static_cast<unsigned>(padded + 64));
@@ -257,6 +303,10 @@
         std::fprintf(stderr, "[mrhip] rational_opair T=%d smin=%d in=%zuB arith=%zuB grid=%lld block=%u lds=%zu occ/CU=%d regs=%d c=%d P=%d cM=%d J=%d ns=%d\n",
                      a.T, static_cast<int>(a.M / a.L), static_cast<size_t>(pa.x_f64 ? 8 : 4) * pa.nc, static_cast<size_t>(pa.r_f64 ? 8 : 4), g, block.x, lds, per_cu,
                      regs, pa.c, pa.P, pa.cM, pa.J, pa.ns);
+    {
+        const int64_t lp[10] = {pa.balanced, pa.c, pa.P, pa.cM, pa.J, pa.ns, block.x, static_cast<int64_t>(lds), per_cu, g};
+        for (int i = 0; i < 10; ++i) g_last_plan[i] = lp[i];
+    }
     MRHIP_PROBE_PRE(g)
     launch_kernel(kfn, dim3(static_cast<unsigned>(g)), block, lds, s, a, pa);
     MRHIP_PROBE_POST(g)
@@ -271,6 +321,7 @@
     pa.counters = counters;
     *kname = "rational_opair_kernel";
     const int smin = static_cast<int>(a.M / a.L);
+    if (pa.balanced) return launch_opair_f32_s1b(a.T, block, lds, s, a, pa, num_cus);
     if (pa.r_f64 && pa.nc == 2)
         return smin == 0 ? launch_opair_cmix_s0(pa.x_f64 != 0, fused, a.T, block, lds, s, a, pa, num_cus)
                          : launch_opair_cmix_s1(pa.x_f64 != 0, fused, a.T, block, lds, s, a, pa, num_cus);
diff --git a/multirate.jl_amd/csrc/kernels_rational_opair_f32_s1b.hip b/multirate.jl_amd/csrc/kernels_rational_opair_f32_s1b.hip
--- /dev/null
+++ b/multirate.jl_amd/csrc/kernels_rational_opair_f32_s1b.hip
@@ -0,0 +1,13 @@
+#include "opair_kernel.inc"
+
+namespace mrhip {
+
+hipError_t launch_opair_f32_s1b(int T, dim3 block, size_t lds, hipStream_t s, const PolyArgs &a, const PairArgs &pa, int num_cus)
+{
+    if (T != 24 || !pa.balanced || pa.ns != 2 || block.x > static_cast<unsigned>(kOBalThreads) || a.ring_dev || a.dyn || a.multi)
+        return hipErrorInvalidValue;
+    const PairKernelFn kfn = rational_opair_kernel<24, false, 1, 1, float, float, 4>;
+    return launch_opair_kernel(kfn, reinterpret_cast<const void *>(kfn), block, lds, s, a, pa, num_cus);
+}
+
+}
diff --git a/multirate.jl_amd/csrc/mrhip_internal.h b/multirate.jl_amd/csrc/mrhip_internal.h
--- a/multirate.jl_amd/csrc/mrhip_internal.h
+++ b/multirate.jl_amd/csrc/mrhip_internal.h
@@ -379,6 +379,7 @@
     long long tiles_per_channel;
     long long total_tiles;
     unsigned long long *probe;
+    int balanced;
 };
 
 constexpr size_t kCounterBytes = 33 * 256;
@@ -468,7 +469,13 @@
                                const char **kname, int num_cus);
 hipError_t launch_shiftin(const TypeKey &tk, const HistArgs &a, hipStream_t s);
 bool polyfit_rows(const double *y, int64_t n, int polyorder, double *coef);
-bool plan_rational_opair(const TypeKey &tk, bool fused, const PolyArgs &a, int num_cus, PairArgs *out, dim3 *block, size_t *lds, int force_wgpc = 0);
+bool plan_rational_opair(const TypeKey &tk, bool fused, const PolyArgs &a, int num_cus, PairArgs *out, dim3 *block, size_t *lds, int force_wgpc = 0,
+                         bool one_filter = false);
+constexpr bool opair_balanced_instantiated(const TypeKey &tk, bool fused, int smin, int T)
+{
+    return !fused && !tk.x_f64 && !tk.r_f64 && !tk.complex_x && smin == 1 && T == 24;
+}
+void opair_last_plan(int64_t *info, int n);
 bool plan_rational_opair_blocks(const TypeKey &tk, bool fused, const PolyArgs &a, int num_cus, PairArgs *out, dim3 *block, size_t *lds, int *nblocks);
 hipError_t launch_rational_opair(bool fused, const PolyArgs &a, const PairArgs &pa, dim3 block, size_t lds, hipStream_t s,
                                  const char **kname, int num_cus, unsigned *counters);
diff --git a/multirate.jl_amd/csrc/opair_kernel.inc b/multirate.jl_amd/csrc/opair_kernel.inc
--- a/multirate.jl_amd/csrc/opair_kernel.inc
+++ b/multirate.jl_amd/csrc/opair_kernel.inc
@@ -18,6 +18,7 @@
 namespace {
 
 constexpr int kOMaxThreads = 512;
+constexpr int kOBalThreads = 768;
 
 using namespace dev;
 
@@ -49,7 +50,8 @@
 #ifndef MRHIP_RING_WAVES
 #define MRHIP_RING_WAVES 4
 #endif
-__global__ __launch_bounds__(sizeof(R) == 8 && T > 32 ? kOMaxThreads : kOMaxThreads + 64, sizeof(R) == 8 ? (T > 32 ? 2 : MRHIP_OPAIR_WIDE_WAVES) : (MODE == 2 ? MRHIP_RING_WAVES : 3))
+__global__ __launch_bounds__(MODE == 4 ? kOBalThreads : sizeof(R) == 8 && T > 32 ? kOMaxThreads : kOMaxThreads + 64,
+                             MODE == 4 ? 6 : sizeof(R) == 8 ? (T > 32 ? 2 : MRHIP_OPAIR_WIDE_WAVES) : (MODE == 2 ? MRHIP_RING_WAVES : 3))
 void rational_opair_kernel(PolyArgs a, PairArgs pa)
 {
     constexpr unsigned ES = static_cast<unsigned>(sizeof(TXS)) * NC;
@@ -68,17 +70,46 @@
     const unsigned lds_base = static_cast<unsigned>(reinterpret_cast<uintptr_t>(smem));
     const int tid = threadIdx.x;
     const int wave = __builtin_amdgcn_readfirstlane(tid >> 6), lane = tid & 63;
-    const int ncw = (blockDim.x >> 6) - 1;
     constexpr bool RING = MODE == 2;
+    constexpr bool BAL = MODE == 4;
+    const int ncw = (blockDim.x >> 6) - (BAL ? 0 : 1);
     if constexpr (MODE == 0) pair_take_dyn(a, pa);
 
-    if (wave == ncw) {
-        if constexpr (RING) pair_ring_loader_wave<NW, static_cast<int>(OS)>(a, pa, smem, lane);
-        else pair_loader_wave<NW, MODE != 1>(a, pa, smem, lane);
-        return;
+    if constexpr (!BAL) {
+        if (wave == ncw) {
+            if constexpr (RING) pair_ring_loader_wave<NW, static_cast<int>(OS)>(a, pa, smem, lane);
+            else pair_loader_wave<NW, MODE != 1>(a, pa, smem, lane);
+            return;
+        }
     }
     if constexpr (RING) { if (blockIdx.x == 0) return; }
     volatile unsigned *const tile_flag = reinterpret_cast<volatile unsigned *>(smem + pa.flags_off);
+    const unsigned flag_base = lds_base + static_cast<unsigned>(pa.flags_off);
+    [[maybe_unused]] PairHandoutT<true> ho;
+    [[maybe_unused]] unsigned cur_g = 0, cur_j = 0;
+    auto fresh_lane = []() -> int {
+        unsigned l;
+        asm volatile("v_mbcnt_lo_u32_b32 %0, -1, 0\n\tv_mbcnt_hi_u32_b32 %0, -1, %0" : "=v"(l));
+        return static_cast<int>(l);
+    };
+    auto bal_publish = [&](int slot) {
+        unsigned g = 0;
+        TileAt ta{0, 0, 0};
+        v2u_t d;
+        if (ho.next_tile(pa, lane, &g, &ta)) { d.x = g; d.y = static_cast<unsigned>(ta.jt); }
+        else { d.x = 0u; d.y = 0u; }
+        lds_write8_now(flag_base + 8u * static_cast<unsigned>(slot), d);
+    };
+    if constexpr (BAL) {
+        ho.init(a, pa);
+        if (wave == 0) {
+            ho.grab_issue(pa, lane);
+            if (ho.want_draw) ho.draw_now();
+            bal_publish(0);
+            if (ho.want_draw) ho.draw_now();
+            bal_publish(1);
+        }
+    }
 
     const int Li = static_cast<int>(a.L), Mi = static_cast<int>(a.M);
     int u0 = static_cast<int>(a.u0);
@@ -136,7 +167,17 @@
         for (int j = 0; j < NA; ++j) pin(tapA[j]);
 #pragma unroll
         for (int j = 0; j < NB; ++j) pin(tapB[j]);
-    } else gather_taps();
+    } else {
+        gather_taps();
+        if constexpr (BAL) __builtin_amdgcn_s_barrier();
+    }
+    if constexpr (BAL) {
+        const v2u_t d0 = lds_read8_now(flag_base);
+        cur_g = static_cast<unsigned>(__builtin_amdgcn_readfirstlane(static_cast<int>(d0.x)));
+        cur_j = static_cast<unsigned>(__builtin_amdgcn_readfirstlane(static_cast<int>(d0.y)));
+        if (cur_j != 0u) (void)pair_stage_tile<NW, false>(a, pa, smem, fresh_lane(), pair_pad_magic(pa), pair_tile_at(pa, cur_g, cur_j), 0, wave, ncw);
+        asm volatile("s_waitcnt vmcnt(0)" ::: "memory");
+    }
     bool useA0 = offA == 0, useAT = offA == 1;
     bool useB0 = dB == 0, useB1 = dB <= 1, useBT = dB >= 1, useBT1 = dB == 2;
     auto lanes_of = [](bool b) { return static_cast<unsigned long long>(__builtin_amdgcn_ballot_w64(b)); };
@@ -209,9 +250,21 @@
                 mB0 = lanes_of(useB0); mB1 = lanes_of(useB1); mBT = lanes_of(useBT); mBT1 = lanes_of(useBT1);
             }
         } else {
-            const unsigned tg = static_cast<unsigned>(__builtin_amdgcn_readfirstlane(static_cast<int>(tile_flag[2 * s])));
-            const unsigned tj = static_cast<unsigned>(__builtin_amdgcn_readfirstlane(static_cast<int>(tile_flag[2 * s + 1])));
-            if (tj == 0u) break;
+            unsigned tg, tj;
+            if constexpr (BAL) {
+                tg = cur_g; tj = cur_j;
+                if (tj == 0u) break;
+                const int sn = s + 1 == pa.ns ? 0 : s + 1;
+                const v2u_t dn = lds_read8_now(flag_base + 8u * static_cast<unsigned>(sn));
+                cur_g = static_cast<unsigned>(__builtin_amdgcn_readfirstlane(static_cast<int>(dn.x)));
+                cur_j = static_cast<unsigned>(__builtin_amdgcn_readfirstlane(static_cast<int>(dn.y)));
+                if (wave == 0) bal_publish(s);
+                if (cur_j != 0u) (void)pair_stage_tile<NW, false>(a, pa, smem, fresh_lane(), pair_pad_magic(pa), pair_tile_at(pa, cur_g, cur_j), sn, wave, ncw);
+            } else {
+                tg = static_cast<unsigned>(__builtin_amdgcn_readfirstlane(static_cast<int>(tile_flag[2 * s])));
+                tj = static_cast<unsigned>(__builtin_amdgcn_readfirstlane(static_cast<int>(tile_flag[2 * s + 1])));
+                if (tj == 0u) break;
+            }
             const TileAt ta = pair_tile_at(pa, tg, tj);
             J = ta.jt;
             yc = static_cast<R *>(a.y) + (static_cast<long long>(ta.ch) * a.y_stride + static_cast<long long>(ta.st) * pa.Sout) * NC;
@@ -241,6 +294,18 @@
             static_for<0, KP>([&](auto I) { pring[decltype(I)::value] = read_pair(I, wbase); });
 #pragma unroll 1
             for (int j = 0; j < J; ++j) {
+                [[maybe_unused]] bool drawn = false;
+                [[maybe_unused]] unsigned tkt;
+                if constexpr (BAL) {
+                    drawn = j + 1 == J && ho.want_draw;
+                    if (drawn) {
+                        unsigned z;
+                        unsigned long long sv;
+                        asm volatile("s_mov_b64 %[sv], exec\n\ts_mov_b64 exec, 1\n\tv_mov_b32 %[t], 1\n\tv_mov_b32 %[z], 0\n\t"
+                                     "global_atomic_add %[t], %[z], %[t], %[base] sc0\n\ts_mov_b64 exec, %[sv]"
+                                     : [t] "=&v"(tkt), [z] "=&v"(z), [sv] "=&s"(sv) : [base] "s"(ho.ctr) : "memory");
+                    }
+                }
                 const int jn = j + 1 < J ? j + 1 : j;
                 const unsigned wcur = wbase + static_cast<unsigned>(j) * pa.lds_step * ES;
                 const unsigned wnext = wbase + static_cast<unsigned>(jn) * pa.lds_step * ES;
@@ -317,6 +382,13 @@
                     else if constexpr (r + KP >= NPRV) pring[slot] = read_pair(std::integral_constant<int, r + KP - NPRV>{}, wnext);
                 });
                 {
+                    if constexpr (BAL) {
+                        if (drawn) {
+                            asm volatile("s_waitcnt vmcnt(0)" : "+v"(tkt) : : "memory");
+                            ho.pend = static_cast<unsigned>(__builtin_amdgcn_readfirstlane(static_cast<int>(tkt)));
+                            ho.want_draw = false;
+                        } else if (j + 1 == J) asm volatile("s_waitcnt vmcnt(0)" ::: "memory");
+                    }
                     const unsigned kj = static_cast<unsigned>(j) * static_cast<unsigned>(pa.Sout);
                     char *const dst = ybytes + (kj + my_out) * OS;
                     R v[2 * NC];
@@ -392,8 +464,9 @@
             atomicAdd(&a.ring_dev->stats[3], 1ull);
         }
     }
+    if constexpr (BAL) { if (wave == 0) pair_loader_finish<NW>(a, pa, fresh_lane(), ho.static_stride); }
 #ifdef MRHIP_OPAIR_PROBE
-    if (pa.probe && lane == 0) {
+    if (pa.probe && lane == 0 && (!BAL || wave < 8)) {
         unsigned long long *r = pa.probe + (static_cast<unsigned long long>(blockIdx.x) * 8u + static_cast<unsigned>(wave)) * 4u;
         const unsigned hw = __builtin_amdgcn_s_getreg(0xF804), xcc = __builtin_amdgcn_s_getreg(0xF814);
         r[0] = hw | (static_cast<unsigned long long>(xcc) << 32);
diff --git a/multirate.jl_amd/csrc/pair_device.h b/multirate.jl_amd/csrc/pair_device.h
--- a/multirate.jl_amd/csrc/pair_device.h
+++ b/multirate.jl_amd/csrc/pair_device.h
@@ -123,6 +123,17 @@
     v4u_t v;
     asm volatile("ds_read_b128 %0, %1\n\ts_waitcnt lgkmcnt(0)" : "=&v"(v) : "v"(byte_addr) : "memory");
     return v;
+}
+
+__device__ __forceinline__ v2u_t lds_read8_now(unsigned byte_addr)
+{
+    v2u_t v;
+    asm volatile("ds_read_b64 %0, %1\n\ts_waitcnt lgkmcnt(0)" : "=&v"(v) : "v"(byte_addr) : "memory");
+    return v;
+}
+__device__ __forceinline__ void lds_write8_now(unsigned byte_addr, v2u_t v)
+{
+    asm volatile("ds_write_b64 %0, %1\n\ts_waitcnt lgkmcnt(0)" ::"v"(byte_addr), "v"(v) : "memory");
 }
 
 __device__ __forceinline__ unsigned long long ld_sc1(const unsigned long long *p) { return __hip_atomic_load(p, __ATOMIC_RELAXED, __HIP_MEMORY_SCOPE_AGENT); }
diff --git a/multirate.jl_amd/csrc/pair_loader.h b/multirate.jl_amd/csrc/pair_loader.h
--- a/multirate.jl_amd/csrc/pair_loader.h
+++ b/multirate.jl_amd/csrc/pair_loader.h
@@ -48,109 +48,193 @@
     }
 }
 
+template <bool DEFER>
+struct PairHandoutT {
+    bool want_draw;
+    unsigned grp_lo, grp_hi;
+    unsigned *ctr;
+    unsigned pend;
+    unsigned static_next, static_stride;
+    unsigned ra, rb;
+    bool more;
+    __device__ __forceinline__ void init(const PolyArgs &a, const PairArgs &pa)
+    {
+        const unsigned grp = blockIdx.x % static_cast<unsigned>(pa.ngroups);
+        grp_lo = a.multi ? 0u : umin(grp * pa.steps_per_group, pa.total_steps);
+        grp_hi = umin(grp_lo + pa.steps_per_group, pa.total_steps);
+        ctr = pa.counters + grp * 64u;
+        pend = 0;
+        static_next = blockIdx.x / static_cast<unsigned>(pa.ngroups);
+        static_stride = (gridDim.x + static_cast<unsigned>(pa.ngroups) - 1u - grp) / static_cast<unsigned>(pa.ngroups);
+        ra = rb = 0;
+        more = true;
+        want_draw = false;
+    }
+    __device__ __forceinline__ void draw_now()
+    {
+        unsigned t = 1u, z = 0u;
+        unsigned long long sv;
+        asm volatile("s_mov_b64 %[sv], exec\n\ts_mov_b64 exec, 1\n\tglobal_atomic_add %[t], %[z], %[t], %[base] sc0\n\ts_waitcnt vmcnt(0)\n\ts_mov_b64 exec, %[sv]"
+                     : [t] "+v"(t), [sv] "=&s"(sv) : [z] "v"(z), [base] "s"(ctr) : "memory");
+        pend = static_cast<unsigned>(__builtin_amdgcn_readfirstlane(static_cast<int>(t)));
+        want_draw = false;
+    }
+    __device__ __forceinline__ void grab_issue(const PairArgs &pa, int lane)
+    {
+        if (pa.static_grabs) { pend = static_next; static_next += static_stride; }
+        else if constexpr (DEFER) want_draw = true;
+        else if (lane == 0) pend = atomicAdd(ctr, 1u);
+    }
+    __device__ __forceinline__ void grab_take(const PairArgs &pa, int lane)
+    {
+        const unsigned t = static_cast<unsigned>(__builtin_amdgcn_readfirstlane(static_cast<int>(pend)));
+        const unsigned long long lo = static_cast<unsigned long long>(grp_lo) + static_cast<unsigned long long>(t) * pa.J;
+        if (lo < grp_hi) { ra = static_cast<unsigned>(lo); rb = umin(ra + pa.J, grp_hi); grab_issue(pa, lane); }
+        else { more = false; ra = rb = 0; }
+    }
+    __device__ __forceinline__ bool next_tile(const PairArgs &pa, int lane, unsigned *g, TileAt *ta)
+    {
+        if (ra >= rb && more) grab_take(pa, lane);
+        if (ra >= rb) return false;
+        *ta = pair_tile_at(pa, ra, rb - ra);
+        *g = ra;
+        ra += static_cast<unsigned>(ta->jt);
+        return true;
+    }
+};
+using PairHandout = PairHandoutT<false>;
+
+__device__ __forceinline__ unsigned pair_pad_magic(const PairArgs &pa)
+{
+    return pa.pad_every > 0 ? 0xffffffffu / static_cast<unsigned>(pa.pad_every + 1) + 1u : 0u;
+}
+
+template <int NC, bool FAST_SEAM>
+__device__ __forceinline__ int pair_stage_tile(const PolyArgs &a, const PairArgs &pa, unsigned char *smem, int lane, unsigned pad_magic,
+                                               const TileAt &ta, int stage, int slot0, int slot_step)
+{
+    const int sch = ta.ch;
+    constexpr int EPC = 4 / NC;
+    const int rc = pa.run_chunks;
+    const int tlen = rc > 0 ? ta.jt * rc * EPC : (ta.jt * pa.cM + pa.tail + EPC - 1) / EPC * EPC;
+    const int nchunks = tlen / EPC;
+    const int cd = pa.pad_every;
+    const int nlds = cd > 0 ? (nchunks + cd - 1) / cd * (cd + 1) : nchunks;
+    const int nslots = (nlds + 63) >> 6;
+    const float *__restrict__ xc = static_cast<const float *>(a.x) + static_cast<long long>(sch) * a.x_stride * NC;
+    const long long o = pa.o0 + static_cast<long long>(ta.st) * pa.cM;
+    unsigned char *st = smem + static_cast<size_t>(stage) * pa.stage_bytes;
+    const long long o_end = rc > 0 ? o + static_cast<long long>(ta.jt - 1) * pa.cM + rc * EPC : o + tlen;
+    const bool interior = o >= 0 && o_end <= a.x_len;
+    auto chunk_sample = [&](int c) -> long long {
+        if (rc <= 0) return static_cast<long long>(EPC) * c;
+        unsigned j = __umulhi(static_cast<unsigned>(c), pa.run_magic);
+        int w = c - static_cast<int>(j) * rc;
+        if (w < 0) { --j; w += rc; }
+        return static_cast<long long>(j) * pa.cM + static_cast<long long>(EPC) * w;
+    };
+    if (interior) {
+        const unsigned char *src = reinterpret_cast<const unsigned char *>(xc + o * NC);
+        int issued = 0;
+        if (rc > 0) {
+            for (int slot = slot0; slot < nslots; slot += slot_step, ++issued) {
+                const int ci = slot * 64 + lane;
+                const int cis = ci < nchunks ? ci : 0;
+                dma16(src + static_cast<size_t>(chunk_sample(cis)) * (NC * 4u), st + static_cast<size_t>(slot) * 1024);
+            }
+            return issued;
+        }
+        for (int slot = slot0; slot < nslots; slot += slot_step, ++issued) {
+            const int ci = slot * 64 + lane;
+            int d = ci;
+            if (cd > 0) { const int g = static_cast<int>(__umulhi(static_cast<unsigned>(ci), pad_magic)), r = ci - g * (cd + 1); d = r == cd ? 0 : g * cd + r; }
+            const int cis = d < nchunks ? d : 0;
+            dma16(src + static_cast<size_t>(cis) * 16, st + static_cast<size_t>(slot) * 1024);
+        }
+        return issued;
+    }
+    if (slot0 != 0) return 0;
+    if constexpr (FAST_SEAM) {
+        const unsigned char *src = reinterpret_cast<const unsigned char *>(xc + o * NC);
+        const unsigned char *dummy = static_cast<const unsigned char *>(a.taps);
+        for (int slot = 0; slot < nslots; ++slot) {
+            const int ci = slot * 64 + lane;
+            int d = ci;
+            bool data = ci < nlds;
+            if (cd > 0) { const int g = static_cast<int>(__umulhi(static_cast<unsigned>(ci), pad_magic)), r = ci - g * (cd + 1); data = data && r != cd; d = g * cd + r; }
+            data = data && d < nchunks;
+            const long long smp = data ? chunk_sample(d) : 0;
+            const bool inside = data && o + smp >= 0 && o + smp + EPC <= a.x_len;
+            dma16(inside ? src + smp * (NC * 4) : dummy, st + static_cast<size_t>(slot) * 1024);
+        }
+        asm volatile("s_waitcnt vmcnt(0)" ::: "memory");
+    }
+    const float *__restrict__ hc = static_cast<const float *>(a.hist) + static_cast<long long>(sch) * a.H * NC;
+    float *l = reinterpret_cast<float *>(st);
+    for (int ci = lane; ci < nchunks; ci += 64) {
+        const long long g0 = o + chunk_sample(ci);
+        if constexpr (FAST_SEAM) { if (g0 >= 0 && g0 + EPC <= a.x_len) continue; }
+        float4 v;
+        float *pv = reinterpret_cast<float *>(&v);
+#pragma unroll
+        for (int e = 0; e < EPC; ++e) {
+            const long long gi = g0 + e;
+#pragma unroll
+            for (int cc = 0; cc < NC; ++cc) {
+                float val = 0.f;
+                if (gi >= 0) { if (gi < a.x_len) val = xc[gi * NC + cc]; }
+                else if (gi >= -static_cast<long long>(a.H)) val = hc[(a.H + gi) * NC + cc];
+                pv[e * NC + cc] = val;
+            }
+        }
+        *reinterpret_cast<float4 *>(l + (cd > 0 ? ci + ci / cd : ci) * 4) = v;
+    }
+    asm volatile("s_waitcnt vmcnt(0) lgkmcnt(0)" ::: "memory");
+    return 0;
+}
+
+template <int NC>
+__device__ __forceinline__ void pair_loader_finish(const PolyArgs &a, const PairArgs &pa, int lane, unsigned static_stride)
+{
+    if (lane == 0 && !pa.static_grabs) {
+        unsigned *const done = pa.counters + static_cast<unsigned>(pa.ngroups) * 64u;
+        if (atomicAdd(done, 1u) == gridDim.x - 1) {
+            for (int k = 0; k < pa.ngroups; ++k) pa.counters[k * 64] = 0u;
+            *done = 0u;
+        }
+    }
+    const unsigned wg_in_grp = blockIdx.x / static_cast<unsigned>(pa.ngroups);
+    if ((a.multi ? wg_in_grp == 0u : blockIdx.x == 0) && lane == 0 && a.rec && !a.dyn) {
+        a.rec->phiIdx = a.phi_end;
+        a.rec->inputDeficit = a.d_end;
+        a.rec->n_written = a.n_out;
+        a.rec->calls += 1;
+    }
+    if (a.H > 0) {
+        const float *__restrict__ xin = static_cast<const float *>(a.x);
+        const float *__restrict__ hold = static_cast<const float *>(a.hist);
+        float *__restrict__ hnew = static_cast<float *>(a.hist_new);
+        const int c_first = a.multi ? static_cast<int>(wg_in_grp) : static_cast<int>(blockIdx.x);
+        const int c_step = a.multi ? static_cast<int>(static_stride) : static_cast<int>(gridDim.x);
+        for (int c2 = c_first; c2 < a.nch; c2 += c_step)
+            for (int i = lane; i < a.H; i += 64) {
+                const long long e = static_cast<long long>(i) + a.x_len;
+#pragma unroll
+                for (int cc = 0; cc < NC; ++cc)
+                    hnew[(static_cast<long long>(c2) * a.H + i) * NC + cc] =
+                        e < a.H ? hold[(static_cast<long long>(c2) * a.H + e) * NC + cc]
+                                : xin[(static_cast<long long>(c2) * a.x_stride + (e - a.H)) * NC + cc];
+            }
+    }
+}
+
 template <int NC, bool FAST_SEAM = true>
 __device__ __forceinline__ void pair_loader_wave(const PolyArgs &a, const PairArgs &pa, unsigned char *smem, int lane)
 {
     volatile unsigned *const tile_flag = reinterpret_cast<volatile unsigned *>(smem + pa.flags_off);
-    auto tile_at = [&](unsigned g, unsigned jt) -> TileAt { return pair_tile_at(pa, g, jt); };
-    const unsigned pad_magic = pa.pad_every > 0 ? 0xffffffffu / static_cast<unsigned>(pa.pad_every + 1) + 1u : 0u;
-    auto stage_tile = [&](const TileAt &ta, int stage) -> int {
-        const int sch = ta.ch;
-        constexpr int EPC = 4 / NC;
-        const int rc = pa.run_chunks;
-        const int tlen = rc > 0 ? ta.jt * rc * EPC : (ta.jt * pa.cM + pa.tail + EPC - 1) / EPC * EPC;
-        const int nchunks = tlen / EPC;
-        const int cd = pa.pad_every;
-        const int nlds = cd > 0 ? (nchunks + cd - 1) / cd * (cd + 1) : nchunks;
-        const int nslots = (nlds + 63) >> 6;
-        const float *__restrict__ xc = static_cast<const float *>(a.x) + static_cast<long long>(sch) * a.x_stride * NC;
-        const long long o = pa.o0 + static_cast<long long>(ta.st) * pa.cM;
-        unsigned char *st = smem + static_cast<size_t>(stage) * pa.stage_bytes;
-        const long long o_end = rc > 0 ? o + static_cast<long long>(ta.jt - 1) * pa.cM + rc * EPC : o + tlen;
-        const bool interior = o >= 0 && o_end <= a.x_len;
-        auto chunk_sample = [&](int c) -> long long {
-            if (rc <= 0) return static_cast<long long>(EPC) * c;
-            unsigned j = __umulhi(static_cast<unsigned>(c), pa.run_magic);
-            int w = c - static_cast<int>(j) * rc;
-            if (w < 0) { --j; w += rc; }
-            return static_cast<long long>(j) * pa.cM + static_cast<long long>(EPC) * w;
-        };
-        if (interior) {
-            const unsigned char *src = reinterpret_cast<const unsigned char *>(xc + o * NC);
-            if (rc > 0) {
-                for (int slot = 0; slot < nslots; ++slot) {
-                    const int ci = slot * 64 + lane;
-                    const int cis = ci < nchunks ? ci : 0;
-                    dma16(src + static_cast<size_t>(chunk_sample(cis)) * (NC * 4u), st + static_cast<size_t>(slot) * 1024);
-                }
-                return nslots;
-            }
-            for (int slot = 0; slot < nslots; ++slot) {
-                const int ci = slot * 64 + lane;
-                int d = ci;
-                if (cd > 0) { const int g = static_cast<int>(__umulhi(static_cast<unsigned>(ci), pad_magic)), r = ci - g * (cd + 1); d = r == cd ? 0 : g * cd + r; }
-                const int cis = d < nchunks ? d : 0;
-                dma16(src + static_cast<size_t>(cis) * 16, st + static_cast<size_t>(slot) * 1024);
-            }
-            return nslots;
-        }
-        if constexpr (FAST_SEAM) {
-            const unsigned char *src = reinterpret_cast<const unsigned char *>(xc + o * NC);
-            const unsigned char *dummy = static_cast<const unsigned char *>(a.taps);
-            for (int slot = 0; slot < nslots; ++slot) {
-                const int ci = slot * 64 + lane;
-                int d = ci;
-                bool data = ci < nlds;
-                if (cd > 0) { const int g = static_cast<int>(__umulhi(static_cast<unsigned>(ci), pad_magic)), r = ci - g * (cd + 1); data = data && r != cd; d = g * cd + r; }
-                data = data && d < nchunks;
-                const long long smp = data ? chunk_sample(d) : 0;
-                const bool inside = data && o + smp >= 0 && o + smp + EPC <= a.x_len;
-                dma16(inside ? src + smp * (NC * 4) : dummy, st + static_cast<size_t>(slot) * 1024);
-            }
-            asm volatile("s_waitcnt vmcnt(0)" ::: "memory");
-        }
-        const float *__restrict__ hc = static_cast<const float *>(a.hist) + static_cast<long long>(sch) * a.H * NC;
-        float *l = reinterpret_cast<float *>(st);
-        for (int ci = lane; ci < nchunks; ci += 64) {
-            const long long g0 = o + chunk_sample(ci);
-            if constexpr (FAST_SEAM) { if (g0 >= 0 && g0 + EPC <= a.x_len) continue; }
-            float4 v;
-            float *pv = reinterpret_cast<float *>(&v);
-#pragma unroll
-            for (int e = 0; e < EPC; ++e) {
-                const long long gi = g0 + e;
-#pragma unroll
-                for (int cc = 0; cc < NC; ++cc) {
-                    float val = 0.f;
-                    if (gi >= 0) { if (gi < a.x_len) val = xc[gi * NC + cc]; }
-                    else if (gi >= -static_cast<long long>(a.H)) val = hc[(a.H + gi) * NC + cc];
-                    pv[e * NC + cc] = val;
-                }
-            }
-            *reinterpret_cast<float4 *>(l + (cd > 0 ? ci + ci / cd : ci) * 4) = v;
-        }
-        asm volatile("s_waitcnt vmcnt(0) lgkmcnt(0)" ::: "memory");
-        return 0;
-    };
-    const unsigned grp = blockIdx.x % static_cast<unsigned>(pa.ngroups);
-    const unsigned grp_lo = a.multi ? 0u : umin(grp * pa.steps_per_group, pa.total_steps);
-    const unsigned grp_hi = umin(grp_lo + pa.steps_per_group, pa.total_steps);
-    unsigned *const ctr = pa.counters + grp * 64u;
-    unsigned pend = 0;
-    unsigned static_next = blockIdx.x / static_cast<unsigned>(pa.ngroups);
-    const unsigned static_stride = (gridDim.x + static_cast<unsigned>(pa.ngroups) - 1u - grp) / static_cast<unsigned>(pa.ngroups);
-    auto grab_issue = [&]() {
-        if (pa.static_grabs) { pend = static_next; static_next += static_stride; }
-        else if (lane == 0) pend = atomicAdd(ctr, 1u);
-    };
-    unsigned ra = 0, rb = 0;
-    bool more = true;
-    auto grab_take = [&]() {
-        const unsigned t = static_cast<unsigned>(__builtin_amdgcn_readfirstlane(static_cast<int>(pend)));
-        const unsigned long long lo = static_cast<unsigned long long>(grp_lo) + static_cast<unsigned long long>(t) * pa.J;
-        if (lo < grp_hi) { ra = static_cast<unsigned>(lo); rb = umin(ra + pa.J, grp_hi); grab_issue(); }
-        else { more = false; ra = rb = 0; }
-    };
+    const unsigned pad_magic = pair_pad_magic(pa);
+    PairHandout ho;
+    ho.init(a, pa);
     unsigned long long hist = 0;
     auto newest_ops = [&](int ntiles) -> int {
         int n = 0;
@@ -158,19 +242,18 @@
         return n < 60 ? n : 60;
     };
     auto produce = [&](int stage) -> bool {
-        if (ra >= rb && more) grab_take();
-        if (ra >= rb) {
+        unsigned g;
+        TileAt ta;
+        if (!ho.next_tile(pa, lane, &g, &ta)) {
             if (lane == 0) { tile_flag[2 * stage] = 0u; tile_flag[2 * stage + 1] = 0u; }
             hist <<= 6;
             return false;
         }
-        const TileAt ta = tile_at(ra, rb - ra);
-        if (lane == 0) { tile_flag[2 * stage] = ra; tile_flag[2 * stage + 1] = static_cast<unsigned>(ta.jt); }
-        hist = (hist << 6) | static_cast<unsigned>((pa.ablate & 1) ? 0 : stage_tile(ta, stage));
-        ra += static_cast<unsigned>(ta.jt);
+        if (lane == 0) { tile_flag[2 * stage] = g; tile_flag[2 * stage + 1] = static_cast<unsigned>(ta.jt); }
+        hist = (hist << 6) | static_cast<unsigned>((pa.ablate & 1) ? 0 : pair_stage_tile<NC, FAST_SEAM>(a, pa, smem, lane, pad_magic, ta, stage, 0, 1));
         return true;
     };
-    grab_issue();
+    ho.grab_issue(pa, lane);
     unsigned pipeline = 0;
     for (int k = 0; k < pa.ns - 1; ++k)
         if (produce(k)) pipeline |= 1u << k;
@@ -210,36 +293,7 @@
         r[1] = clock64() - pr_t0; r[2] = pr_bar; r[3] = pr_vm;
     }
 #endif
-    if (lane == 0 && !pa.static_grabs) {
-        unsigned *const done = pa.counters + static_cast<unsigned>(pa.ngroups) * 64u;
-        if (atomicAdd(done, 1u) == gridDim.x - 1) {
-            for (int k = 0; k < pa.ngroups; ++k) pa.counters[k * 64] = 0u;
-            *done = 0u;
-        }
-    }
-    const unsigned wg_in_grp = blockIdx.x / static_cast<unsigned>(pa.ngroups);
-    if ((a.multi ? wg_in_grp == 0u : blockIdx.x == 0) && lane == 0 && a.rec && !a.dyn) {
-        a.rec->phiIdx = a.phi_end;
-        a.rec->inputDeficit = a.d_end;
-        a.rec->n_written = a.n_out;
-        a.rec->calls += 1;
-    }
-    if (a.H > 0) {
-        const float *__restrict__ xin = static_cast<const float *>(a.x);
-        const float *__restrict__ hold = static_cast<const float *>(a.hist);
-        float *__restrict__ hnew = static_cast<float *>(a.hist_new);
-        const int c_first = a.multi ? static_cast<int>(wg_in_grp) : static_cast<int>(blockIdx.x);
-        const int c_step = a.multi ? static_cast<int>(static_stride) : static_cast<int>(gridDim.x);
-        for (int c2 = c_first; c2 < a.nch; c2 += c_step)
-            for (int i = lane; i < a.H; i += 64) {
-                const long long e = static_cast<long long>(i) + a.x_len;
-#pragma unroll
-                for (int cc = 0; cc < NC; ++cc)
-                    hnew[(static_cast<long long>(c2) * a.H + i) * NC + cc] =
-                        e < a.H ? hold[(static_cast<long long>(c2) * a.H + e) * NC + cc]
-                                : xin[(static_cast<long long>(c2) * a.x_stride + (e - a.H)) * NC + cc];
-            }
-    }
+    pair_loader_finish<NC>(a, pa, lane, ho.static_stride);
 }
 
 
diff --git a/multirate.jl_amd/host.py b/multirate.jl_amd/host.py
--- a/multirate.jl_amd/host.py
+++ b/multirate.jl_amd/host.py
@@ -103,6 +103,7 @@
     ("mrhip_set_timing", _i, [_vp, _i]),
     ("mrhip_timing_read", _i, [_vp, _pi64, C.POINTER(C.c_double)]),
     ("mrhip_last_kernel_name", C.c_char_p, [_vp]),
+    ("mrhip_opair_plan_info", _i, [_pi64, _i]),
     ("mrhip_schedule_info", _i, [_vp, _pi64, _i]),
     ("mrhip_sharded_create", _i, [_i, _vp, _i64, _i, _i64, _i64, _d, _i64, _i64, _i, _i64, C.POINTER(_i), _i, C.POINTER(_vp)]),
     ("mrhip_sharded_destroy", None, [_vp]),
@@ -490,6 +491,12 @@
     def last_kernel_name(self) -> str:
         return self._lib.mrhip_last_kernel_name(self._handle).decode()
 
+    def opair_plan_info(self) -> dict:
+        v = (C.c_int64 * 10)()
+        _check(self._lib.mrhip_opair_plan_info(v, 10))
+        keys = ("balanced", "c", "P", "cM", "J", "ns", "block", "lds", "wg_per_cu", "grid")
+        return dict(zip(keys, (int(a) for a in v)))
+
     def schedule_info(self) -> dict:
         v = (C.c_int64 * 8)()
         _check(self._lib.mrhip_schedule_info(self._handle, v, 8))
```

New measurement: 597,600. 10.4% lower.
